# GStreamer/gst-plugins-rs

Hardware: AMD Instinct MI355X
Metric: 4K RGBA frames/sec through hsvfilter+colorlut at 1 GPU; % HBM roofline (higher is better)
Workload: dtype u8

## Files before the change

gst-plugins-rs_amd/csrc/colorlut_kernels.hip:

```cpp
#include "internal.hpp"
#include "hsv_device.hpp"
#include "exact_math.hpp"

#include <cmath>
#include <cstring>
#include <map>
#include <memory>
#include <mutex>
#include <vector>

namespace mi355 {

struct LutK {
  float scale[3];
  float offset[3];
  int size;
};


__device__ __forceinline__ uint32_t floor_idx(float x, uint32_t max_idx) {
  const float f = floorf(x);
  uint32_t i = (f > 0.0f) ? ((f >= 4294967040.0f) ? 0xffffffffu : (uint32_t)f) : 0u;
  return i < max_idx ? i : max_idx;
}
// ... 1337 lines not shown
  }
#undef MI355_ROWS
  return check_hip(ctx, hipGetLastError(), "colorlut rows kernel launch");
}


struct Rgba8Geom {
  size_t n_vec = 0;
  unsigned sw4 = 0, dw4 = 0;
  bool packed = false;
};
static bool rgba8_geom(const uint8_t *d_src, size_t src_pitch, int src_stride, const uint8_t *d_dst, size_t dst_pitch, int dst_stride, int n_frames,
                       int width, int height, Rgba8Geom *g) {
  const size_t row_bytes = (size_t)width * 4;
  if (((uintptr_t)d_src % 16 != 0) || ((uintptr_t)d_dst % 16 != 0)) return false;
  const bool packed = (size_t)src_stride == row_bytes && (size_t)dst_stride == row_bytes &&
                      (n_frames == 1 || (src_pitch == row_bytes * (size_t)height && dst_pitch == row_bytes * (size_t)height));
  const size_t total_bytes = row_bytes * (size_t)height * (size_t)n_frames;
  if (packed) {
    if (total_bytes % 16 != 0) return false;
    g->n_vec = total_bytes / 16;
    g->sw4 = g->dw4 = (unsigned)(row_bytes / 16);
    g->packed = true;
    return true;
  }
  if (width % 4 != 0 || width < 128 || (size_t)src_stride < row_bytes || (size_t)dst_stride < row_bytes || src_stride % 16 != 0 || dst_stride % 16 != 0) return false;
  if (n_frames != 1 && (src_pitch != (size_t)src_stride * (size_t)height || dst_pitch != (size_t)dst_stride * (size_t)height)) return false;
  g->n_vec = total_bytes / 16;
  g->sw4 = (unsigned)src_stride / 16;
  g->dw4 = (unsigned)dst_stride / 16;
  g->packed = false;
  return true;
}

static bool same_hs(const mi355_hsv_settings &a, const mi355_hsv_settings &b) { return std::memcmp(&a, &b, sizeof(a)) == 0; }

struct SharedTable {
  uint32_t *d = nullptr;
  hipEvent_t ready = nullptr;
  std::vector<hipEvent_t> released;
  int device = 0;
  ~SharedTable() {
    int cur = 0;
    (void)hipGetDevice(&cur);
    (void)hipSetDevice(device);
    if (ready) { (void)hipEventSynchronize(ready); (void)hipEventDestroy(ready); }
    for (hipEvent_t e : released) (void)hipEventDestroy(e);
    if (d) (void)hipFree(d);
    (void)hipSetDevice(cur);
  }
};
static std::mutex g_tables_mu;
static std::map<std::string, std::weak_ptr<SharedTable>> g_tables;

static void shared_table_release_locked(mi355_ctx *ctx, std::shared_ptr<void> *ref) {
  if (!*ref) return;
  if (ref->use_count() > 1) {
    SharedTable *sp = static_cast<SharedTable *>(ref->get());
    hipEvent_t e = nullptr;
    if (hipEventCreateWithFlags(&e, hipEventDisableTiming) == hipSuccess) {
      if (hipEventRecord(e, ctx->stream) == hipSuccess) sp->released.push_back(e);
      else { (void)hipEventDestroy(e); (void)hipStreamSynchronize(ctx->stream); }
    } else {
      (void)hipStreamSynchronize(ctx->stream);
    }
    (void)hipGetLastError();
  }
  ref->reset();
}
void shared_table_release(mi355_ctx *ctx, std::shared_ptr<void> *ref) {
  std::shared_ptr<void> last;
  {
    std::lock_guard<std::mutex> g(g_tables_mu);
    if (*ref && ref->use_count() == 1) last = std::move(*ref);
    else shared_table_release_locked(ctx, ref);
  }
}

template <class Build>
static int shared_table_acquire(mi355_ctx *ctx, const std::string &key, std::shared_ptr<void> *ref, uint32_t **out, Build &&build) {
  std::lock_guard<std::mutex> g(g_tables_mu);
  for (auto it = g_tables.begin(); it != g_tables.end();) it = it->second.expired() ? g_tables.erase(it) : std::next(it);
  const std::string full = std::string((const char *)&ctx->device, sizeof(ctx->device)) + key;
  if (auto sp = g_tables[full].lock()) {
    int rc = check_hip(ctx, hipStreamWaitEvent(ctx->stream, sp->ready, 0), "hipStreamWaitEvent(shared table)");
    if (rc) return rc;
    if (ref->get() != sp.get()) shared_table_release_locked(ctx, ref);
    *out = sp->d;
    *ref = sp;
    return MI355_OK;
  }
  std::shared_ptr<SharedTable> sp;
  if (*ref && ref->use_count() == 1) {
    sp = std::static_pointer_cast<SharedTable>(*ref);
    for (hipEvent_t e : sp->released) {
      int rc = check_hip(ctx, hipStreamWaitEvent(ctx->stream, e, 0), "hipStreamWaitEvent(released table)");
      if (rc) return rc;
    }
    for (hipEvent_t e : sp->released) (void)hipEventDestroy(e);
    sp->released.clear();
    for (auto it = g_tables.begin(); it != g_tables.end();) it = it->second.lock() == sp ? g_tables.erase(it) : std::next(it);
  } else {
    shared_table_release_locked(ctx, ref);
    sp = std::make_shared<SharedTable>();
    sp->device = ctx->device;
    int rc = check_hip(ctx, hipMalloc((void **)&sp->d, (size_t)kTableEntries * 4), "hipMalloc(memoised table)");
    if (rc) return rc;
    if ((rc = check_hip(ctx, hipEventCreateWithFlags(&sp->ready, hipEventDisableTiming), "hipEventCreate(shared table)"))) return rc;
  }
  int rc = build(sp->d);
  if (rc) { ref->reset(); return rc; }
  if ((rc = check_hip(ctx, hipEventRecord(sp->ready, ctx->stream), "hipEventRecord(shared table)"))) { ref->reset(); return rc; }
  g_tables[full] = sp;
  *out = sp->d;
  *ref = sp;
  return MI355_OK;
}

extern "C" int mi355_shared_table_count(void) {
  std::lock_guard<std::mutex> g(g_tables_mu);
  int n = 0;
  for (auto &kv : g_tables) n += kv.second.expired() ? 0 : 1;
  return n;
}

static int table_ensure(mi355_ctx *ctx, int which, int morton, const mi355_hsv_settings *hs) {
  LutDevice &L = ctx->lut;
  std::string key(which ? "F" : "L");
  key.push_back((char)('0' + morton));
  key += L.digest;
  if (which) key.append((const char *)hs, sizeof(*hs));
  if (L.table_ref[which] && L.table_key[which] == key) return MI355_OK;
  L.d_table[which] = nullptr;
  L.table_morton[which] = -1;
  L.table_key[which].clear();
  int rc = shared_table_acquire(ctx, key, &L.table_ref[which], &L.d_table[which], [&](uint32_t *tab) {
    uint8_t *t = (uint8_t *)tab;
    hipLaunchKernelGGL(table_domain_kernel, dim3(kTableEntries / 256), dim3(256), 0, ctx->stream, tab, morton);
    L.building_table = true;
    const char *serving = L.last_kernel;
    const int r = which == 0 ? launch_colorlut_compute(ctx, t, 0, 4096 * 4, t, 0, 4096 * 4, 1, 4096, 4096, MI355_FMT_RGBA)
                             : launch_hsv_colorlut_compute(ctx, t, 0, 4096 * 4, t, 0, 4096 * 4, 1, 4096, 4096, *hs, true);
    L.building_table = false;
    L.last_kernel = serving;
    return r;
  });
  if (rc) { L.table_ref[which].reset(); L.d_table[which] = nullptr; return rc; }
  L.table_key[which] = key;
  L.table_morton[which] = morton;
  if (which == 1) L.table_hs = *hs;
  return MI355_OK;
}

enum TableKernel { kTableGather = 0, kTableWindow = 1, kTableEither = 2 };
template <class Compute, class Ensure, class Table>
static int auto_launch(mi355_ctx *ctx, AutoPick &A, size_t n_vec, Compute &&compute, Ensure &&ensure, Table &&table);
static int launch_table_gather(mi355_ctx *ctx, const uint32_t *t, const uint8_t *d_src, uint8_t *d_dst, const Rgba8Geom &geo, int width, size_t rows, int morton);
static int launch_table_raw(mi355_ctx *ctx, const uint32_t *t, const uint8_t *d_src, uint8_t *d_dst, const Rgba8Geom &geo, int width, size_t rows, int morton,
                            TableKernel sub = kTableGather, int *last_sub = nullptr);
static int launch_table(mi355_ctx *ctx, int which, const uint8_t *d_src, uint8_t *d_dst, const Rgba8Geom &geo, int width, size_t rows, int morton,
                        const mi355_hsv_settings *hs, TableKernel sub = kTableGather) {
  int rc = table_ensure(ctx, which, morton, hs);
  if (rc) return rc;
  return launch_table_raw(ctx, ctx->lut.d_table[which], d_src, d_dst, geo, width, rows, morton, sub, &ctx->lut.last_sub[which]);
}

static int launch_table_raw(mi355_ctx *ctx, const uint32_t *t, const uint8_t *d_src, uint8_t *d_dst, const Rgba8Geom &geo, int width, size_t rows, int morton,
                            TableKernel sub, int *last_sub) {
  const bool window_ok = morton && sub != kTableGather && width % 4 == 0 && window_applicable(ctx, (unsigned)width / 4, geo.dw4, rows);
  const size_t src_bytes = (size_t)geo.sw4 * 16 * rows;
  const bool window = window_ok && (sub == kTableWindow || !recently_written(ctx->device, d_src, src_bytes));
  if (last_sub) *last_sub = window ? 1 : 0;
  int rc;
  if (window) {
    ctx->lut.last_kernel = "colorlut_window_kernel";
    rc = launch_window_table(ctx, t, d_src, d_dst, (unsigned)width / 4, geo.sw4, geo.dw4, rows);
  } else {
    rc = launch_table_gather(ctx, t, d_src, d_dst, geo, width, rows, morton);
  }
  return rc;
}

static int launch_table_gather(mi355_ctx *ctx, const uint32_t *t, const uint8_t *d_src, uint8_t *d_dst, const Rgba8Geom &geo, int width, size_t rows, int morton) {
  const size_t n_vec = geo.n_vec;
  ctx->lut.last_kernel = "colorlut_table_tiled_kernel";
  if (width % 4 == 0 && width >= 128 && rows < (1u << 30)) {
    const unsigned w4 = (unsigned)width / 4;
    const unsigned pad64 = (w4 + 63) / 64 * 64 - w4, pad32 = (w4 + 31) / 32 * 32 - w4;
    const unsigned tw4 = pad64 <= pad32 ? 64 : 32;
    const unsigned n_cols = (w4 + tw4 - 1) / tw4, rpb = 8 * (64 / tw4);
    const size_t n_tiles = (size_t)n_cols * ((rows + rpb - 1) / rpb);
    if (n_tiles < (1u << 31)) {
      const size_t grid = n_tiles;
#define MI355_LT(M, T) hipLaunchKernelGGL((colorlut_table_tiled_kernel<M, T>), dim3((unsigned)grid), dim3(256), 0, ctx->stream, (const uint4 *)d_src, \
                                          (uint4 *)d_dst, w4, geo.sw4, geo.dw4, (unsigned)rows, n_cols, t)
      if (morton && tw4 == 64) MI355_LT(true, 64);
      else if (morton) MI355_LT(true, 32);
      else if (tw4 == 64) MI355_LT(false, 64);
      else MI355_LT(false, 32);
#undef MI355_LT
      return check_hip(ctx, hipGetLastError(), "colorlut table kernel launch");
    }
  }
  if (!geo.packed) return set_error(ctx, MI355_ERR_INVALID_ARG, "colorlut: table kernel geometry");
  ctx->lut.last_kernel = "colorlut_table_kernel";
  size_t grid = (size_t)ctx->n_cu * 16;
  const size_t max_blocks = n_vec / 512 + 1;
  if (grid > max_blocks) grid = max_blocks;
  if (morton) hipLaunchKernelGGL((colorlut_table_kernel<true>), dim3((unsigned)grid), dim3(256), 0, ctx->stream, (const uint4 *)d_src, (uint4 *)d_dst, n_vec, t);
  else hipLaunchKernelGGL((colorlut_table_kernel<false>), dim3((unsigned)grid), dim3(256), 0, ctx->stream, (const uint4 *)d_src, (uint4 *)d_dst, n_vec, t);
  return check_hip(ctx, hipGetLastError(), "colorlut table kernel launch");
}

static void auto_harvest(AutoPick &A) {
  if (A.pending_kind < 0) return;
  if (hipEventQuery(A.ev1) != hipSuccess) {
    (void)hipGetLastError();
    return;
  }
  float ms = 0.0f;
  if (hipEventElapsedTime(&ms, A.ev0, A.ev1) != hipSuccess) { (void)hipGetLastError(); ms = 0.0f; }
  auto_complete(A, (double)ms);
}

template <class Compute, class Ensure, class Table>
static int auto_launch(mi355_ctx *ctx, AutoPick &A, size_t n_vec, Compute &&compute, Ensure &&ensure, Table &&table) {
  int rc;
  if (A.table_unavailable) return compute();
  if (!A.ev0) {
    if ((rc = check_hip(ctx, hipEventCreate(&A.ev0), "hipEventCreate"))) return rc;
    if ((rc = check_hip(ctx, hipEventCreate(&A.ev1), "hipEventCreate"))) return rc;
  }
  auto_harvest(A);
  const AutoDecision D = auto_decide(A, n_vec);
  if (D.kind == 1 && (rc = ensure())) {
    auto_give_up_table(A);
    (void)hipGetLastError();
    return compute();
  }
  if (D.measure && (rc = check_hip(ctx, hipEventRecord(A.ev0, ctx->stream), "hipEventRecord"))) return rc;
  if ((rc = D.kind ? table() : compute())) return rc;
  if (D.measure) {
    if ((rc = check_hip(ctx, hipEventRecord(A.ev1, ctx->stream), "hipEventRecord"))) return rc;
    auto_sampled(A, D, n_vec);
  }
  return MI355_OK;
}

constexpr size_t kAutoMinVec = 16384;
static bool table_variant(int v) { return v == 4 || v == 5 || v == 8 || v == 9; }
static TableKernel table_variant_kernel(int v) { return v == 8 ? kTableWindow : (v == 9 ? kTableEither : kTableGather); }

int launch_colorlut(mi355_ctx *ctx, const uint8_t *d_src, size_t src_pitch, int src_stride, uint8_t *d_dst,
                    size_t dst_pitch, int dst_stride, int n_frames, int width, int height, int format) {
  LutDevice &L = ctx->lut;
  if (!L.loaded) return set_error(ctx, MI355_ERR_NOT_CONFIGURED, "No LUT configured");
  if (n_frames <= 0 || width <= 0 || height <= 0) return MI355_OK;
  Rgba8Geom geo;
  const bool table_ok = format == MI355_FMT_RGBA && !ctx->force_generic &&
                        rgba8_geom(d_src, src_pitch, src_stride, d_dst, dst_pitch, dst_stride, n_frames, width, height, &geo);
  const size_t n_vec = geo.n_vec;
  const int v = ctx->lut_variant;
  auto compute = [&]() { return launch_colorlut_compute(ctx, d_src, src_pitch, src_stride, d_dst, dst_pitch, dst_stride, n_frames, width, height, format); };
  if (table_ok && table_variant(v))
    return launch_table(ctx, 0, d_src, d_dst, geo, width, (size_t)n_frames * height, v == 4 ? 0 : 1, nullptr, table_variant_kernel(v));
  if (!table_ok || v != 0 || n_vec < kAutoMinVec) return compute();
  return auto_launch(ctx, L.pick[0], n_vec, compute, [&]() { return table_ensure(ctx, 0, 1, nullptr); },
                     [&]() { return launch_table(ctx, 0, d_src, d_dst, geo, width, (size_t)n_frames * height, 1, nullptr, kTableEither); });
}

constexpr unsigned kStableCalls = 8;
int launch_hsv_colorlut(mi355_ctx *ctx, const uint8_t *d_src, size_t src_pitch, int src_stride, uint8_t *d_dst,
                        size_t dst_pitch, int dst_stride, int n_frames, int width, int height,
                        const mi355_hsv_settings &hs) {
  LutDevice &L = ctx->lut;
  if (!L.loaded) return set_error(ctx, MI355_ERR_NOT_CONFIGURED, "No LUT configured");
  if (n_frames <= 0 || width <= 0 || height <= 0) return MI355_OK;
  Rgba8Geom geo;
  const bool table_ok = !ctx->force_generic && rgba8_geom(d_src, src_pitch, src_stride, d_dst, dst_pitch, dst_stride, n_frames, width, height, &geo);
  const size_t n_vec = geo.n_vec;
  const int v = ctx->lut_variant;
  auto compute = [&]() { return launch_hsv_colorlut_compute(ctx, d_src, src_pitch, src_stride, d_dst, dst_pitch, dst_stride, n_frames, width, height, hs, false); };
  if (table_ok && table_variant(v))
    return launch_table(ctx, 1, d_src, d_dst, geo, width, (size_t)n_frames * height, v == 4 ? 0 : 1, &hs, table_variant_kernel(v));
  if (!table_ok || v != 0 || n_vec < kAutoMinVec) return compute();
  if (same_hs(hs, L.seen_hs)) { if (L.seen_stable < kStableCalls) L.seen_stable++; }
  else { L.seen_hs = hs; L.seen_stable = 0; }
  const bool have = L.table_ref[1] && L.table_morton[1] == 1 && same_hs(L.table_hs, hs);
  if (!have && L.seen_stable < kStableCalls) return compute();
  if (!have && L.pick[1].learn > 2) {
    L.pick[1].t_table = 0.0;
    L.pick[1].learn = 2;
  }
  return auto_launch(ctx, L.pick[1], n_vec, compute, [&]() { return table_ensure(ctx, 1, 1, &hs); },
                     [&]() { return launch_table(ctx, 1, d_src, d_dst, geo, width, (size_t)n_frames * height, 1, &hs, kTableEither); });
}

int colorlut_multi_table(mi355_ctx *ctx, const uint32_t **table_out) {
  LutDevice &L = ctx->lut;
  if (!L.loaded) return set_error(ctx, MI355_ERR_NOT_CONFIGURED, "No LUT configured");
  int rc = table_ensure(ctx, 0, 1, nullptr);
  if (rc) return rc;
  *table_out = L.d_table[0];
  return MI355_OK;
}

int colorlut_multi_fused_table(mi355_ctx *ctx, const mi355_hsv_settings *hs, const uint32_t **table_out) {
  LutDevice &L = ctx->lut;
  if (!L.loaded) return set_error(ctx, MI355_ERR_NOT_CONFIGURED, "No LUT configured");
  if (!hs) return set_error(ctx, MI355_ERR_INVALID_ARG, "null settings");
  int rc = table_ensure(ctx, 1, 1, hs);
  if (rc) return rc;
  *table_out = L.d_table[1];
  return MI355_OK;
}
int launch_colorlut_multi(mi355_ctx *ctx, hipStream_t stream, const uint32_t *table, uint8_t *const *srcs, uint8_t *const *dsts, int n_frames, int width,
                          int height, bool from_hbm) {
  if (n_frames < 1 || n_frames > kMultiFrames || width % 4 != 0 || width < 128 || height <= 0) return MI355_ERR_UNSUPPORTED;
  MultiFramePtrs s{}, d{};
  for (int f = 0; f < n_frames; f++) {
    if (!srcs[f] || !dsts[f] || (uintptr_t)srcs[f] % 16 != 0 || (uintptr_t)dsts[f] % 16 != 0) return MI355_ERR_UNSUPPORTED;
    s.p[f] = srcs[f];
    d.p[f] = dsts[f];
  }
  const unsigned w4 = (unsigned)width / 4;
  if (from_hbm && ctx->lut_variant == 0 && window_multi_applicable(ctx, w4, (size_t)height, n_frames)) {
    ctx->lut.last_kernel = "colorlut_window_kernel";
    return launch_window_table_multi(ctx, stream, table, srcs, dsts, n_frames, w4, (size_t)height);
  }
  ctx->lut.last_kernel = "colorlut_table_tiled_multi_kernel";
  const unsigned pad64 = (w4 + 63) / 64 * 64 - w4, pad32 = (w4 + 31) / 32 * 32 - w4;
  const unsigned tw4 = pad64 <= pad32 ? 64 : 32;
  const unsigned n_cols = (w4 + tw4 - 1) / tw4, rpb = 8 * (64 / tw4);
  const size_t tiles_per_frame = (size_t)n_cols * (((size_t)height + rpb - 1) / rpb);
  const size_t grid = tiles_per_frame * (size_t)n_frames;
  if (grid >= (1u << 31)) return MI355_ERR_UNSUPPORTED;
  if (tw4 == 64) hipLaunchKernelGGL((colorlut_table_tiled_multi_kernel<64>), dim3((unsigned)grid), dim3(256), 0, stream, s, d, w4, (unsigned)height, n_cols, (unsigned)tiles_per_frame, table);
  else hipLaunchKernelGGL((colorlut_table_tiled_multi_kernel<32>), dim3((unsigned)grid), dim3(256), 0, stream, s, d, w4, (unsigned)height, n_cols, (unsigned)tiles_per_frame, table);
  return check_hip(ctx, hipGetLastError(), "colorlut multi-frame table kernel launch");
}

void hsv_table_release(mi355_ctx *ctx) {
  HsvTable &T = ctx->hsv_table;
  shared_table_release(ctx, &T.table_ref);
  if (T.pick.ev0) (void)hipEventDestroy(T.pick.ev0);
  if (T.pick.ev1) (void)hipEventDestroy(T.pick.ev1);
  T = HsvTable{};
}

static int hsv_table_ensure(mi355_ctx *ctx, const PixFmt &fmt, const mi355_hsv_settings &hs) {
  HsvTable &T = ctx->hsv_table;
  if (T.valid && T.bgr == fmt.bgr && same_hs(T.hs, hs)) return MI355_OK;
  T.valid = false;
  T.d_table = nullptr;
  std::string key("H");
  key.push_back((char)('0' + fmt.bgr));
  key.append((const char *)&hs, sizeof(hs));
  int rc = shared_table_acquire(ctx, key, &T.table_ref, &T.d_table, [&](uint32_t *tab) {
    hipLaunchKernelGGL(table_domain_kernel, dim3(kTableEntries / 256), dim3(256), 0, ctx->stream, tab, 1);
    return launch_hsvfilter_compute(ctx, (uint8_t *)tab, 1, 0, 4096, 4096, 4096 * 4, fmt, hs);
  });
  if (rc) { T.table_ref.reset(); T.d_table = nullptr; return rc; }
  T.valid = true;
  T.bgr = fmt.bgr;
  T.hs = hs;
  return MI355_OK;
}

int launch_hsvfilter(mi355_ctx *ctx, uint8_t *d_data, int n_frames, size_t frame_pitch, int width, int height, int stride, const PixFmt &fmt,
                     const mi355_hsv_settings &hs) {
  if (n_frames <= 0 || width <= 0 || height <= 0) return MI355_OK;
  HsvTable &T = ctx->hsv_table;
  auto compute = [&]() { return launch_hsvfilter_compute(ctx, d_data, n_frames, frame_pitch, width, height, stride, fmt, hs); };
  Rgba8Geom geo;
  const bool candidate = ctx->hsv_table_mode == 1 || ctx->hsv_table_mode == 2 || (ctx->hsv_table_mode == 0 && hsv_variant_for(hs, false, true) < 0);
  const bool table_ok = candidate && !ctx->force_generic && fmt.pixel_stride == 4 && fmt.first == 0 &&
                        rgba8_geom(d_data, frame_pitch, stride, d_data, frame_pitch, stride, n_frames, width, height, &geo);
  const size_t n_vec = geo.n_vec;
  T.last_table = false;
  if (!table_ok) return compute();
  const size_t rows = (size_t)n_frames * height;
  if (ctx->hsv_table_mode == 2) {
    int rc = hsv_table_ensure(ctx, fmt, hs);
    T.last_table = true;
    return rc ? rc : launch_table_raw(ctx, T.d_table, d_data, d_data, geo, width, rows, 1, kTableEither, nullptr);
  }
  if (n_vec < kAutoMinVec) return compute();
  if (same_hs(hs, T.seen_hs) && fmt.bgr == T.seen_bgr) { if (T.seen_stable < kStableCalls) T.seen_stable++; }
  else { T.seen_hs = hs; T.seen_bgr = fmt.bgr; T.seen_stable = 0; }
  const bool have = T.valid && T.bgr == fmt.bgr && same_hs(T.hs, hs);
  if (!have && T.seen_stable < kStableCalls) return compute();
  if (!have && T.pick.learn > 2) {
    T.pick.t_table = 0.0;
    T.pick.learn = 2;
  }
  return auto_launch(ctx, T.pick, n_vec, compute, [&]() { return hsv_table_ensure(ctx, fmt, hs); },
                     [&]() { T.last_table = true; return launch_table_raw(ctx, T.d_table, d_data, d_data, geo, width, rows, 1, kTableEither, nullptr); });
}

}

extern "C" int mi355_selftest_brickwatch(int n_calls, const double *miss0, const double *slow0, const double *miss1, const double *slow1, int lag,
                                         int *level_out) {
  if (n_calls < 0 || !miss0 || !slow0 || !miss1 || !slow1 || !level_out || lag < 0) return MI355_ERR_INVALID_ARG;
  const bool shared1 = (lag >> 16) & 1;
  const int min_level = (lag >> 17) & 3;
  lag &= 0xffff;
  mi355::BrickWatch W;
  int level_since = -1, launches_since = 0, pend_level = -1, pend_ready = 0;
  double acc_m = 0, acc_s = 0, pend_m = 0, pend_s = 0;
  for (int i = 0; i < n_calls; i++) {
    if (pend_level >= 0 && i >= pend_ready) { const int l = pend_level; pend_level = -1; mi355::watch_snapshot(W, l, pend_m, pend_s, shared1); }
    const int level = mi355::watch_level(W, pend_level < 0, min_level);
    level_out[i] = level;
    if (level == 2) { level_since = 2; continue; }
    if (level != level_since) { level_since = level; launches_since = 0; acc_m = acc_s = 0; }
    acc_m += level ? miss1[i] : miss0[i];
    acc_s += level ? slow1[i] : slow0[i];
    launches_since++;
    if (pend_level < 0 && launches_since >= (W.probing == level ? 1 : (int)mi355::kWatchSnapEvery)) {
      pend_level = level; pend_m = acc_m / launches_since; pend_s = acc_s / launches_since; pend_ready = i + 1 + lag;
      launches_since = 0; acc_m = acc_s = 0;
    }
  }
  return MI355_OK;
}

extern "C" int mi355_selftest_autopick(int n_calls, const uint64_t *n_vec, const double *ms_compute, const double *ms_table, int lag,
                                       int *kind_out, int *measured_out) {
  if (n_calls < 0 || !n_vec || !ms_compute || !ms_table || !kind_out || lag < 0) return MI355_ERR_INVALID_ARG;
  mi355::AutoPolicy A;
  double pending_ms = 0.0;
  for (int i = 0; i < n_calls; i++) {
    const size_t nv = (size_t)n_vec[i];
    if (A.pending_kind >= 0 && A.calls - A.pending_call >= (unsigned)lag) mi355::auto_complete(A, pending_ms);
    const mi355::AutoDecision D = mi355::auto_decide(A, nv);
    kind_out[i] = D.kind;
    if (measured_out) measured_out[i] = D.measure ? 1 : 0;
    if (D.measure) {
      mi355::auto_sampled(A, D, nv);
      pending_ms = D.kind ? ms_table[i] : ms_compute[i];
    }
  }
  return MI355_OK;
}
```

gst-plugins-rs_amd/csrc/ctx.hip:

```cpp
#include "internal.hpp"
#include <mutex>

#include <cstdio>
#include <cstring>

namespace mi355 {

bool pixfmt_of(int format, PixFmt *out) {
  switch (format) {
    case MI355_FMT_RGBX: *out = {4, 0, 0, 0}; return true;
    case MI355_FMT_RGBA: *out = {4, 0, 0, 1}; return true;
    case MI355_FMT_XRGB: *out = {4, 1, 0, 0}; return true;
    case MI355_FMT_ARGB: *out = {4, 1, 0, 1}; return true;
    case MI355_FMT_BGRX: *out = {4, 0, 1, 0}; return true;
    case MI355_FMT_BGRA: *out = {4, 0, 1, 1}; return true;
    case MI355_FMT_XBGR: *out = {4, 1, 1, 0}; return true;
    case MI355_FMT_ABGR: *out = {4, 1, 1, 1}; return true;
    case MI355_FMT_RGB: *out = {3, 0, 0, 0}; return true;
    case MI355_FMT_BGR: *out = {3, 0, 1, 0}; return true;
    default: return false;
  }
}

int set_error(mi355_ctx *ctx, int status, const std::string &msg) {
// ... 1 lines not shown
  return status;
}

int check_hip(mi355_ctx *ctx, hipError_t e, const char *what) {
  if (e == hipSuccess) return MI355_OK;
  std::string msg = std::string(what) + ": " + hipGetErrorString(e);
  const int st = (e == hipErrorOutOfMemory) ? MI355_ERR_OUT_OF_MEMORY : MI355_ERR_HIP;
  return set_error(ctx, st, msg);
}

static int ensure_stage(mi355_ctx *ctx, int slot, size_t bytes) {
  if (ctx->d_stage_bytes[slot] >= bytes && ctx->d_stage[slot]) return MI355_OK;
  if (ctx->d_stage[slot]) (void)hipFree(ctx->d_stage[slot]);
  ctx->d_stage[slot] = nullptr;
  ctx->d_stage_bytes[slot] = 0;
  int rc = check_hip(ctx, hipMalloc(&ctx->d_stage[slot], bytes ? bytes : 16), "hipMalloc(staging)");
  if (rc) return rc;
  ctx->d_stage_bytes[slot] = bytes ? bytes : 16;
  return MI355_OK;
}

}

using namespace mi355;

template <typename F>
static int time_launches(mi355_ctx *ctx, int iters, float *ms_per_launch, F &&launch) {
  if (iters <= 0 || !ms_per_launch) return set_error(ctx, MI355_ERR_INVALID_ARG, "timing: bad iters/output");
  hipEvent_t e0, e1;
  int rc = check_hip(ctx, hipEventCreate(&e0), "hipEventCreate");
  if (rc) return rc;
  rc = check_hip(ctx, hipEventCreate(&e1), "hipEventCreate");
  if (rc) { (void)hipEventDestroy(e0); return rc; }
  rc = check_hip(ctx, hipEventRecord(e0, ctx->stream), "hipEventRecord");
  for (int i = 0; i < iters && rc == MI355_OK; i++) rc = launch();
  if (rc == MI355_OK) rc = check_hip(ctx, hipEventRecord(e1, ctx->stream), "hipEventRecord");
  if (rc == MI355_OK) rc = check_hip(ctx, hipEventSynchronize(e1), "hipEventSynchronize");
  float ms = 0.0f;
  if (rc == MI355_OK) rc = check_hip(ctx, hipEventElapsedTime(&ms, e0, e1), "hipEventElapsedTime");
  (void)hipEventDestroy(e0);
  (void)hipEventDestroy(e1);
  if (rc == MI355_OK) *ms_per_launch = ms / (float)iters;
  return rc;
}


#define REQUIRE_CTX(ctx) \
  do { if (!(ctx)) return MI355_ERR_INVALID_ARG; } while (0)
#define BIND_DEVICE(ctx)                                                                  \
  do { int rc__ = check_hip((ctx), hipSetDevice((ctx)->device), "hipSetDevice");          \
       if (rc__) return rc__; } while (0)

extern "C" {

int mi355_abi_version(void) { return MI355FX_ABI_VERSION; }

int mi355_device_count(void) {
  int n = 0;
  if (hipGetDeviceCount(&n) != hipSuccess) return 0;
  return n;
}

const char *mi355_status_string(int status) {
  switch (status) {
    case MI355_OK: return "ok";
    case MI355_ERR_INVALID_ARG: return "invalid argument";
    case MI355_ERR_NO_DEVICE: return "no usable gfx950 device";
    case MI355_ERR_HIP: return "HIP runtime error";
    case MI355_ERR_NOT_CONFIGURED: return "element not configured";
    case MI355_ERR_OUT_OF_MEMORY: return "out of device memory";
    case MI355_ERR_UNSUPPORTED: return "unsupported";
    case MI355_ERR_TIMEOUT: return "timeout";
    default: return "unknown status";
  }
}

}

namespace mi355 {
namespace {
struct Written { uintptr_t lo = 0, hi = 0; };
std::mutex g_written_mu;
Written g_written[16][2];
constexpr size_t kOnDieBytes = (size_t)320 << 20;
}

void note_written(int device, const void *p, size_t bytes) {
  if (device < 0 || device >= 16 || !p || !bytes) return;
  std::lock_guard<std::mutex> lk(g_written_mu);
  g_written[device][1] = g_written[device][0];
  g_written[device][0].lo = (uintptr_t)p;
  g_written[device][0].hi = (uintptr_t)p + bytes;
}

void forget_written(int device, const void *p, size_t bytes) {
  if (device < 0 || device >= 16 || !p || !bytes) return;
  std::lock_guard<std::mutex> lk(g_written_mu);
  for (Written &w : g_written[device])
    if (w.hi > w.lo && (uintptr_t)p < w.hi && (uintptr_t)p + bytes > w.lo) w = Written{};
}

bool recently_written(int device, const void *p, size_t bytes) {
  if (device < 0 || device >= 16 || !p || !bytes || bytes > kOnDieBytes) return false;
  std::lock_guard<std::mutex> lk(g_written_mu);
  for (const Written &w : g_written[device])
    if (w.hi > w.lo && (uintptr_t)p >= w.lo && (uintptr_t)p + bytes <= w.hi && w.hi - w.lo <= kOnDieBytes) return true;
  return false;
}
}

extern "C" {

mi355_ctx *mi355_ctx_create(int device, int *status) {
  int n = 0;
  hipError_t e = hipGetDeviceCount(&n);
  if (e != hipSuccess || n <= 0 || device < 0 || device >= n) {
    if (status) *status = MI355_ERR_NO_DEVICE;
    return nullptr;
  }
  if (hipSetDevice(device) != hipSuccess) {
    if (status) *status = MI355_ERR_NO_DEVICE;
    return nullptr;
  }
  hipDeviceProp_t prop;
  if (hipGetDeviceProperties(&prop, device) != hipSuccess) {
    if (status) *status = MI355_ERR_NO_DEVICE;
    return nullptr;
  }
  if (std::strncmp(prop.gcnArchName, "gfx950", 6) != 0) {
    std::fprintf(stderr, "mi355fx: device %d is %s, this library only carries gfx950 code\n", device, prop.gcnArchName);
    if (status) *status = MI355_ERR_NO_DEVICE;
    return nullptr;
  }
  mi355_ctx *ctx = new mi355_ctx();
  ctx->device = device;
  ctx->n_cu = prop.multiProcessorCount > 0 ? prop.multiProcessorCount : 256;
  if (hipStreamCreateWithFlags(&ctx->stream, hipStreamNonBlocking) != hipSuccess) {
    delete ctx;
    if (status) *status = MI355_ERR_HIP;
    return nullptr;
  }
  ctx->own_stream = true;
  if (status) *status = MI355_OK;
  return ctx;
}

void mi355_ctx_destroy(mi355_ctx *ctx) {
  if (!ctx) return;
  (void)hipSetDevice(ctx->device);
  (void)hipStreamSynchronize(ctx->stream);
  lut_release(ctx);
  hsv_table_release(ctx);
  window_release(ctx);
  loudnorm_release(ctx);
  loudnorm_batch_release(ctx);
  dssim_release(ctx);
  roundedcorners_release(ctx);
  colordetect_release(ctx);
  agingradio_release(ctx);
  mixer_release(ctx);
  yolodec_release(ctx);
  handdec_release(ctx);
  ebur128_release(ctx);
  hrtf_release(ctx);
  sofa_release(ctx);
  echo_release(ctx);
  if (ctx->host_copy_ev) (void)hipEventDestroy(ctx->host_copy_ev);
  for (int i = 0; i < 2; i++)
    if (ctx->d_stage[i]) (void)hipFree(ctx->d_stage[i]);
  if (ctx->own_stream && ctx->stream) (void)hipStreamDestroy(ctx->stream);
  delete ctx;
}

const char *mi355_ctx_last_error(const mi355_ctx *ctx) { return ctx ? ctx->last_error.c_str() : "null context"; }

void *mi355_ctx_stream(mi355_ctx *ctx) { return ctx ? (void *)ctx->stream : nullptr; }

int mi355_ctx_set_stream(mi355_ctx *ctx, void *hip_stream) {
  REQUIRE_CTX(ctx);
  BIND_DEVICE(ctx);
  if (ctx->own_stream && ctx->stream) {
    (void)hipStreamSynchronize(ctx->stream);
    (void)hipStreamDestroy(ctx->stream);
  }
  ctx->stream = (hipStream_t)hip_stream;
  ctx->own_stream = false;
  return MI355_OK;
}

int mi355_ctx_synchronize(mi355_ctx *ctx) {
  REQUIRE_CTX(ctx);
  BIND_DEVICE(ctx);
  return check_hip(ctx, hipStreamSynchronize(ctx->stream), "hipStreamSynchronize");
}

int mi355_ctx_set_flag(mi355_ctx *ctx, int flag, int value) {
  REQUIRE_CTX(ctx);
  if (flag == MI355_FLAG_FORCE_GENERIC) { ctx->force_generic = value != 0; return MI355_OK; }
  if (flag == MI355_FLAG_LUT_STAGGER && value >= 0 && value <= 4096) { ctx->lut_stagger = value; return MI355_OK; }
  if (flag == MI355_FLAG_LUT_VARIANT && value >= 0 && value <= 9) { ctx->lut_variant = value; return MI355_OK; }
  if (flag == MI355_FLAG_BRICK_TILES_PER_RUN && value >= 0 && value <= 4096) { ctx->brick_tiles_per_run = value; return MI355_OK; }
  if (flag == MI355_FLAG_BRICK_FOLD_AXIS && value >= 0 && value <= 2) { ctx->brick_fold_axis = value; return MI355_OK; }
  if (flag == MI355_FLAG_DSSIM_TRANSLUCENT && (value == 0 || value == 1)) { ctx->dssim_translucent = value; return MI355_OK; }
  if (flag == MI355_FLAG_DSSIM_FAST && (value == 0 || value == 1)) { ctx->dssim_fast = value; return MI355_OK; }
  if (flag == MI355_FLAG_BRICK_PRIO && value >= 0 && value <= 3) { ctx->brick_prio = value; return MI355_OK; }
  if (flag == MI355_FLAG_BRICK_SETS && (value == 0 || value == 32 || value == 48 || value == 64 || value == 512)) { ctx->brick_sets = value; return MI355_OK; }
  if (flag == MI355_FLAG_HSV_TABLE && value >= 0 && value <= 3) { ctx->hsv_table_mode = value; return MI355_OK; }
  if (flag == MI355_FLAG_FUSED_VARIANT && value >= 0 && value <= 1) { ctx->fused_variant = value; return MI355_OK; }
  if (flag == MI355_FLAG_HSV_BLOCKS_PER_CU && value >= 1 && value <= 4096) { ctx->hsv_blocks_per_cu = value; return MI355_OK; }
  if (flag == MI355_FLAG_HRTF_METHOD && value >= 0 && value <= 2) { ctx->hrtf_method = value; return MI355_OK; }
  if (flag == MI355_FLAG_BLOCKHASH_ANY_SIZE && (value == 0 || value == 1)) { ctx->blockhash_any_size = value; return MI355_OK; }
  if (flag == MI355_FLAG_HSV_NT && (value == 0 || value == 1)) { ctx->hsv_nt = value; return MI355_OK; }
  if (flag == MI355_FLAG_WINDOW_ORDER && (value == 0 || value == 1)) { ctx->window_order = value; return MI355_OK; }
  if (flag == MI355_FLAG_WINDOW_STATS && (value == 0 || value == 1)) { ctx->window_stats_on = value != 0; return MI355_OK; }
  if (flag == MI355_FLAG_WINDOW_MIN_STEPS && value >= 0 && value <= 4096) { ctx->window_min_steps = value; return MI355_OK; }
  return set_error(ctx, MI355_ERR_INVALID_ARG, "unknown flag");
}

void *mi355_device_alloc(mi355_ctx *ctx, size_t bytes) {
  if (!ctx) return nullptr;
  if (hipSetDevice(ctx->device) != hipSuccess) return nullptr;
  void *p = nullptr;
  if (check_hip(ctx, hipMalloc(&p, bytes ? bytes : 16), "hipMalloc")) return nullptr;
  return p;
}

int mi355_device_free(mi355_ctx *ctx, void *dptr) {
  REQUIRE_CTX(ctx);
  BIND_DEVICE(ctx);
  return check_hip(ctx, hipFree(dptr), "hipFree");
}

int mi355_memcpy_h2d(mi355_ctx *ctx, void *dptr, const void *host, size_t bytes) {
  REQUIRE_CTX(ctx);
  BIND_DEVICE(ctx);
  int rc = check_hip(ctx, hipMemcpyAsync(dptr, host, bytes, hipMemcpyHostToDevice, ctx->stream), "hipMemcpyAsync(H2D)");
  forget_written(ctx->device, dptr, bytes);
  __atomic_fetch_add(&ctx->n_h2d, 1ull, __ATOMIC_RELAXED);
  if (rc) return rc;
  return check_hip(ctx, hipStreamSynchronize(ctx->stream), "hipStreamSynchronize");
}

int mi355_memcpy_d2h(mi355_ctx *ctx, void *host, const void *dptr, size_t bytes) {
  REQUIRE_CTX(ctx);
  BIND_DEVICE(ctx);
  int rc = check_hip(ctx, hipMemcpyAsync(host, dptr, bytes, hipMemcpyDeviceToHost, ctx->stream), "hipMemcpyAsync(D2H)");
  __atomic_fetch_add(&ctx->n_d2h, 1ull, __ATOMIC_RELAXED);
  if (rc) return rc;
  return check_hip(ctx, hipStreamSynchronize(ctx->stream), "hipStreamSynchronize");
}


int mi355_hsvfilter_frames_device(mi355_ctx *ctx, uint8_t *d_data, int n_frames, size_t frame_pitch, int width,
                                  int height, int stride, int format, const mi355_hsv_settings *settings) {
  REQUIRE_CTX(ctx);
  PixFmt fmt;
  if (!settings || !pixfmt_of(format, &fmt)) return set_error(ctx, MI355_ERR_INVALID_ARG, "hsvfilter: bad settings/format");
  if (n_frames < 0 || width < 0 || height < 0 || stride < 0) return set_error(ctx, MI355_ERR_INVALID_ARG, "hsvfilter: negative size");
  if (n_frames == 0 || width == 0 || height == 0) return MI355_OK;
  if (!d_data) return set_error(ctx, MI355_ERR_INVALID_ARG, "hsvfilter: null data");
  if ((size_t)stride < (size_t)width * fmt.pixel_stride)
    return set_error(ctx, MI355_ERR_INVALID_ARG, "hsvfilter: stride smaller than width*pixel_stride");
  if (n_frames > 1 && frame_pitch < (size_t)(height - 1) * (size_t)stride + (size_t)width * fmt.pixel_stride)
    return set_error(ctx, MI355_ERR_INVALID_ARG, "hsvfilter: frame_pitch smaller than one frame (frames would overlap)");
  BIND_DEVICE(ctx);
  const int rc = launch_hsvfilter(ctx, d_data, n_frames, frame_pitch, width, height, stride, fmt, *settings);
  if (rc == MI355_OK) note_written(ctx->device, d_data, (size_t)(n_frames - 1) * frame_pitch + (size_t)stride * (size_t)height);
  return rc;
}

int mi355_hsvfilter_frame_ip(mi355_ctx *ctx, uint8_t *data, size_t data_len, int width, int stride, int format,
                             const mi355_hsv_settings *settings) {
  REQUIRE_CTX(ctx);
  PixFmt fmt;
  if (!settings || !pixfmt_of(format, &fmt)) return set_error(ctx, MI355_ERR_INVALID_ARG, "hsvfilter: bad settings/format");
  if (width < 0 || stride <= 0) return set_error(ctx, MI355_ERR_INVALID_ARG, "hsvfilter: bad width/stride");
  if (data_len % (size_t)fmt.pixel_stride != 0) return set_error(ctx, MI355_ERR_INVALID_ARG, "hsvfilter: plane length not a multiple of pixel stride");
  const size_t rows = data_len / (size_t)stride;
  if (rows == 0 || width == 0) return MI355_OK;
  if (!data) return set_error(ctx, MI355_ERR_INVALID_ARG, "hsvfilter: null data");
  if ((size_t)width * fmt.pixel_stride > (size_t)stride) return set_error(ctx, MI355_ERR_INVALID_ARG, "hsvfilter: width*pixel_stride exceeds stride");
  if (rows > 0x7fffffffu) return set_error(ctx, MI355_ERR_INVALID_ARG, "hsvfilter: too many rows");
  BIND_DEVICE(ctx);
  const size_t bytes = rows * (size_t)stride;
  int rc = ensure_stage(ctx, 0, bytes);
  if (rc) return rc;
  uint8_t *d = (uint8_t *)ctx->d_stage[0];
  rc = check_hip(ctx, hipMemcpyAsync(d, data, bytes, hipMemcpyHostToDevice, ctx->stream), "hipMemcpyAsync(H2D frame)");
  __atomic_fetch_add(&ctx->n_h2d, 1ull, __ATOMIC_RELAXED);
  if (rc) return rc;
  rc = launch_hsvfilter(ctx, d, 1, bytes, width, (int)rows, stride, fmt, *settings);
  if (rc) return rc;
  rc = check_hip(ctx, hipMemcpyAsync(data, d, bytes, hipMemcpyDeviceToHost, ctx->stream), "hipMemcpyAsync(D2H frame)");
  __atomic_fetch_add(&ctx->n_d2h, 1ull, __ATOMIC_RELAXED);
  if (rc) return rc;
  return check_hip(ctx, hipStreamSynchronize(ctx->stream), "hsvfilter: stream synchronize");
}


static bool detect_out_fmt(int fmt, int *alpha_first, int *bgr) {
  switch (fmt) {
    case MI355_FMT_RGBA: *alpha_first = 0; *bgr = 0; return true;
    case MI355_FMT_ARGB: *alpha_first = 1; *bgr = 0; return true;
    case MI355_FMT_BGRA: *alpha_first = 0; *bgr = 1; return true;
    case MI355_FMT_ABGR: *alpha_first = 1; *bgr = 1; return true;
    default: return false;
  }
}
static bool detect_in_fmt(int fmt, PixFmt *p) {
  switch (fmt) {
    case MI355_FMT_RGBX: case MI355_FMT_XRGB: case MI355_FMT_BGRX: case MI355_FMT_XBGR:
    case MI355_FMT_RGB: case MI355_FMT_BGR: return pixfmt_of(fmt, p);
    default: return false;
  }
}

}

namespace mi355 {
int hsvdetect_check_frames(const uint8_t *d_src, int src_stride, int src_format, const uint8_t *d_dst, int dst_stride, int dst_format, int n_frames,
                           int width, int height, const mi355_hsvdetect_settings *settings, PixFmt *sfmt, int *alpha_first, int *bgr, const char **why) {
  if (!settings || !detect_in_fmt(src_format, sfmt) || !detect_out_fmt(dst_format, alpha_first, bgr)) { *why = "hsvdetector: bad settings/format"; return MI355_ERR_INVALID_ARG; }
  if (n_frames < 0 || width < 0 || height < 0) { *why = "hsvdetector: negative size"; return MI355_ERR_INVALID_ARG; }
  if (n_frames == 0 || width == 0 || height == 0) return MI355_OK;
  if (!d_src || !d_dst) { *why = "hsvdetector: null data"; return MI355_ERR_INVALID_ARG; }
  if ((size_t)src_stride < (size_t)width * sfmt->pixel_stride || (size_t)dst_stride < (size_t)width * 4) {
    *why = "hsvdetector: line bytes exceed stride";
    return MI355_ERR_INVALID_ARG;
  }
  return MI355_OK;
}
}

extern "C" {

int mi355_hsvdetect_frames_device(mi355_ctx *ctx, const uint8_t *d_src, size_t src_pitch, int src_stride, int src_format,
                                  uint8_t *d_dst, size_t dst_pitch, int dst_stride, int dst_format, int n_frames,
                                  int width, int height, const mi355_hsvdetect_settings *settings) {
  REQUIRE_CTX(ctx);
  PixFmt sfmt;
  int af = 0, bgr = 0;
  const char *why = nullptr;
  const int bad = hsvdetect_check_frames(d_src, src_stride, src_format, d_dst, dst_stride, dst_format, n_frames, width, height, settings, &sfmt, &af, &bgr, &why);
  if (bad) return set_error(ctx, bad, why);
  if (n_frames == 0 || width == 0 || height == 0) return MI355_OK;
  BIND_DEVICE(ctx);
  const int rc = launch_hsvdetect(ctx, d_src, src_pitch, src_stride, sfmt, d_dst, dst_pitch, dst_stride, af, bgr, n_frames, width, height, *settings);
  if (rc == MI355_OK) note_written(ctx->device, d_dst, (size_t)(n_frames - 1) * dst_pitch + (size_t)dst_stride * (size_t)height);
  return rc;
}

int mi355_hsvdetect_frame(mi355_ctx *ctx, const uint8_t *src, size_t src_len, int src_stride, int src_format, uint8_t *dst,
                          size_t dst_len, int dst_stride, int dst_format, int width, const mi355_hsvdetect_settings *settings) {
  REQUIRE_CTX(ctx);
  PixFmt sfmt;
  int af = 0, bgr = 0;
  if (!settings || !detect_in_fmt(src_format, &sfmt) || !detect_out_fmt(dst_format, &af, &bgr))
    return set_error(ctx, MI355_ERR_INVALID_ARG, "hsvdetector: bad settings/format");
  if (width < 0 || src_stride <= 0 || dst_stride <= 0) return set_error(ctx, MI355_ERR_INVALID_ARG, "hsvdetector: bad width/stride");
  const size_t rows_in = src_len / (size_t)src_stride, rows_out = dst_len / (size_t)dst_stride;
  if (rows_in != rows_out) return set_error(ctx, MI355_ERR_INVALID_ARG, "hsvdetector: input/output row count mismatch");
  if (src_len % (size_t)sfmt.pixel_stride != 0) return set_error(ctx, MI355_ERR_INVALID_ARG, "hsvdetector: plane length not a multiple of pixel stride");
  if ((size_t)width * sfmt.pixel_stride > (size_t)src_stride || (size_t)width * 4 > (size_t)dst_stride)
    return set_error(ctx, MI355_ERR_INVALID_ARG, "hsvdetector: line bytes exceed stride");
  if (rows_in == 0 || width == 0) return MI355_OK;
  if (!src || !dst) return set_error(ctx, MI355_ERR_INVALID_ARG, "hsvdetector: null data");
  BIND_DEVICE(ctx);
  const size_t sb = rows_in * (size_t)src_stride, db = rows_out * (size_t)dst_stride;
  int rc = ensure_stage(ctx, 0, sb);
  if (rc) return rc;
  rc = ensure_stage(ctx, 1, db);
  if (rc) return rc;
  uint8_t *ds = (uint8_t *)ctx->d_stage[0], *dd = (uint8_t *)ctx->d_stage[1];
  rc = check_hip(ctx, hipMemcpyAsync(ds, src, sb, hipMemcpyHostToDevice, ctx->stream), "hipMemcpyAsync(H2D src)");
  __atomic_fetch_add(&ctx->n_h2d, 1ull, __ATOMIC_RELAXED);
  if (rc) return rc;
  rc = check_hip(ctx, hipMemcpyAsync(dd, dst, db, hipMemcpyHostToDevice, ctx->stream), "hipMemcpyAsync(H2D dst)");
  __atomic_fetch_add(&ctx->n_h2d, 1ull, __ATOMIC_RELAXED);
  if (rc) return rc;
  rc = launch_hsvdetect(ctx, ds, sb, src_stride, sfmt, dd, db, dst_stride, af, bgr, 1, width, (int)rows_in, *settings);
  if (rc) return rc;
  rc = check_hip(ctx, hipMemcpyAsync(dst, dd, db, hipMemcpyDeviceToHost, ctx->stream), "hipMemcpyAsync(D2H dst)");
  __atomic_fetch_add(&ctx->n_d2h, 1ull, __ATOMIC_RELAXED);
  if (rc) return rc;
  return check_hip(ctx, hipStreamSynchronize(ctx->stream), "hsvdetector: stream synchronize");
}


int mi355_colorlut_load(mi355_ctx *ctx, int is3d, size_t size, const float *table, const float domain_scale[3],
                        const float domain_offset[3]) {
  REQUIRE_CTX(ctx);
  if (!table || !domain_scale || !domain_offset) return set_error(ctx, MI355_ERR_INVALID_ARG, "colorlut: null LUT data");
  if (is3d ? (size < 2 || size > 256) : (size < 2 || size > 65536))
    return set_error(ctx, MI355_ERR_INVALID_ARG, "colorlut: LUT size out of range");
  BIND_DEVICE(ctx);
  int rc = check_hip(ctx, hipStreamSynchronize(ctx->stream), "colorlut: stream synchronize");
  if (rc) return rc;
  return lut_upload(ctx, is3d ? 1 : 0, size, table, domain_scale, domain_offset);
}

int mi355_colorlut_unload(mi355_ctx *ctx) {
  REQUIRE_CTX(ctx);
  BIND_DEVICE(ctx);
  (void)hipStreamSynchronize(ctx->stream);
  lut_release(ctx);
  return MI355_OK;
}

int mi355_colorlut_kernel_choice(mi355_ctx *ctx, int fused, int *table_in_use, double *ms_per_mpx_compute, double *ms_per_mpx_table) {
  REQUIRE_CTX(ctx);
  if (fused == 10 || fused == 11) {
    if (table_in_use) *table_in_use = ctx->lut.last_sub[fused - 10];
    if (ms_per_mpx_compute) *ms_per_mpx_compute = 0.0;
    if (ms_per_mpx_table) *ms_per_mpx_table = 0.0;
    return MI355_OK;
  }
  const AutoPick &A = fused == 2 ? ctx->hsv_table.pick : ctx->lut.pick[fused ? 1 : 0];
  if (table_in_use)
    *table_in_use = fused == 2 ? (ctx->hsv_table.last_table ? 1 : 0)
                               : (ctx->lut_variant == 4 || ctx->lut_variant == 5 || ctx->lut_variant == 8 || ctx->lut_variant == 9 || (ctx->lut_variant == 0 && A.t_table > 0.0 && A.table));
  if (ms_per_mpx_compute) *ms_per_mpx_compute = A.t_compute * 250000.0;
  if (ms_per_mpx_table) *ms_per_mpx_table = A.t_table * 250000.0;
  return MI355_OK;
}

const char *mi355_colorlut_last_kernel(mi355_ctx *ctx) {
  if (!ctx) return "";
  return ctx->lut.last_kernel ? ctx->lut.last_kernel : "";
}

int mi355_colorlut_brick_stats(mi355_ctx *ctx, uint64_t counters[2], double *last_miss_fraction, int *hostile, int reset) {
  REQUIRE_CTX(ctx);
  BIND_DEVICE(ctx);
  unsigned long long c[2] = {0, 0};
  int rc = brick_read_counters(ctx, ctx->lut.brick, c, reset != 0);
  if (rc) return rc;
  if (counters) { counters[0] = c[0]; counters[1] = c[1]; }
  if (last_miss_fraction) *last_miss_fraction = ctx->lut.brick.watch.last_miss;
  if (hostile) *hostile = ctx->lut.brick.watch.home;
  return MI355_OK;
}

int mi355_colorlut_window_stats(mi355_ctx *ctx, uint64_t counters[3], int reset) {
  REQUIRE_CTX(ctx);
  BIND_DEVICE(ctx);
  if (!counters) return set_error(ctx, MI355_ERR_INVALID_ARG, "null counters");
  unsigned long long c[3] = {0, 0, 0};
  int rc = window_read_counters(ctx, c, reset != 0);
  if (rc) return rc;
  for (int i = 0; i < 3; i++) counters[i] = c[i];
  return MI355_OK;
}

static int colorlut_bpp(int format) {
  if (format == MI355_FMT_RGBA) return 4;
  if (format == MI355_FMT_RGBA64_LE || format == MI355_FMT_RGBA64_BE) return 8;
  return 0;
}

int mi355_colorlut_frames_device(mi355_ctx *ctx, const uint8_t *d_src, size_t src_pitch, int src_stride, uint8_t *d_dst,
                                 size_t dst_pitch, int dst_stride, int n_frames, int width, int height, int format) {
  REQUIRE_CTX(ctx);
  const int bpp = colorlut_bpp(format);
  if (!bpp) return set_error(ctx, MI355_ERR_INVALID_ARG, "colorlut: format must be RGBA, RGBA64_LE or RGBA64_BE");
  if (!ctx->lut.loaded) return set_error(ctx, MI355_ERR_NOT_CONFIGURED, "No LUT configured");
  if (n_frames < 0 || width < 0 || height < 0) return set_error(ctx, MI355_ERR_INVALID_ARG, "colorlut: negative size");
  if (n_frames == 0 || width == 0 || height == 0) return MI355_OK;
  if (!d_src || !d_dst) return set_error(ctx, MI355_ERR_INVALID_ARG, "colorlut: null data");
  if ((size_t)src_stride < (size_t)width * bpp || (size_t)dst_stride < (size_t)width * bpp)
    return set_error(ctx, MI355_ERR_INVALID_ARG, "colorlut: stride smaller than row bytes");
  if (n_frames > 1 && (src_pitch < (size_t)(height - 1) * (size_t)src_stride + (size_t)width * bpp ||
                       dst_pitch < (size_t)(height - 1) * (size_t)dst_stride + (size_t)width * bpp))
    return set_error(ctx, MI355_ERR_INVALID_ARG, "colorlut: frame pitch smaller than one frame (frames would overlap)");
  BIND_DEVICE(ctx);
  const int rc = launch_colorlut(ctx, d_src, src_pitch, src_stride, d_dst, dst_pitch, dst_stride, n_frames, width, height, format);
  if (rc == MI355_OK) note_written(ctx->device, d_dst, (size_t)(n_frames - 1) * dst_pitch + (size_t)dst_stride * (size_t)height);
  return rc;
}

int mi355_hsv_colorlut_frames_device(mi355_ctx *ctx, const uint8_t *d_src, size_t src_pitch, int src_stride, uint8_t *d_dst,
                                     size_t dst_pitch, int dst_stride, int n_frames, int width, int height,
                                     const mi355_hsv_settings *settings) {
  REQUIRE_CTX(ctx);
  if (!settings) return set_error(ctx, MI355_ERR_INVALID_ARG, "hsv+colorlut: null settings");
  if (!ctx->lut.loaded) return set_error(ctx, MI355_ERR_NOT_CONFIGURED, "No LUT configured");
  if (n_frames < 0 || width < 0 || height < 0) return set_error(ctx, MI355_ERR_INVALID_ARG, "hsv+colorlut: negative size");
  if (n_frames == 0 || width == 0 || height == 0) return MI355_OK;
  if (!d_src || !d_dst) return set_error(ctx, MI355_ERR_INVALID_ARG, "hsv+colorlut: null data");
  if ((size_t)src_stride < (size_t)width * 4 || (size_t)dst_stride < (size_t)width * 4)
    return set_error(ctx, MI355_ERR_INVALID_ARG, "hsv+colorlut: stride smaller than row bytes");
  if (n_frames > 1 && (src_pitch < (size_t)(height - 1) * (size_t)src_stride + (size_t)width * 4 ||
                       dst_pitch < (size_t)(height - 1) * (size_t)dst_stride + (size_t)width * 4))
    return set_error(ctx, MI355_ERR_INVALID_ARG, "hsv+colorlut: frame pitch smaller than one frame (frames would overlap)");
  BIND_DEVICE(ctx);
  const int rc = launch_hsv_colorlut(ctx, d_src, src_pitch, src_stride, d_dst, dst_pitch, dst_stride, n_frames, width, height, *settings);
  if (rc == MI355_OK) note_written(ctx->device, d_dst, (size_t)(n_frames - 1) * dst_pitch + (size_t)dst_stride * (size_t)height);
  return rc;
}

int mi355_colorlut_frame(mi355_ctx *ctx, const uint8_t *src, int src_stride, uint8_t *dst, int dst_stride, int width,
                         int height, int format) {
  REQUIRE_CTX(ctx);
  const int bpp = colorlut_bpp(format);
  if (!bpp) return set_error(ctx, MI355_ERR_INVALID_ARG, "colorlut: format must be RGBA, RGBA64_LE or RGBA64_BE");
  if (!ctx->lut.loaded) return set_error(ctx, MI355_ERR_NOT_CONFIGURED, "No LUT configured");
  if (width < 0 || height < 0 || src_stride <= 0 || dst_stride <= 0) return set_error(ctx, MI355_ERR_INVALID_ARG, "colorlut: bad size/stride");
  if (width == 0 || height == 0) return MI355_OK;
  if (!src || !dst) return set_error(ctx, MI355_ERR_INVALID_ARG, "colorlut: null data");
  const size_t s_stride = bpp == 8 ? (size_t)(src_stride / 2) * 2 : (size_t)src_stride;
  const size_t d_stride = bpp == 8 ? (size_t)(dst_stride / 2) * 2 : (size_t)dst_stride;
  const size_t row_bytes = (size_t)width * bpp;
  if (row_bytes > s_stride || row_bytes > d_stride) return set_error(ctx, MI355_ERR_INVALID_ARG, "colorlut: row bytes exceed stride");
  BIND_DEVICE(ctx);
  const size_t packed = row_bytes * (size_t)height;
  int rc = ensure_stage(ctx, 0, packed);
  if (rc) return rc;
  rc = ensure_stage(ctx, 1, packed);
  if (rc) return rc;
  uint8_t *ds = (uint8_t *)ctx->d_stage[0], *dd = (uint8_t *)ctx->d_stage[1];
  rc = check_hip(ctx, hipMemcpy2DAsync(ds, row_bytes, src, s_stride, row_bytes, (size_t)height, hipMemcpyHostToDevice, ctx->stream),
                 "hipMemcpy2DAsync(H2D src)");
  if (rc) return rc;
  rc = launch_colorlut(ctx, ds, packed, (int)row_bytes, dd, packed, (int)row_bytes, 1, width, height, format);
  if (rc) return rc;
  rc = check_hip(ctx, hipMemcpy2DAsync(dst, d_stride, dd, row_bytes, row_bytes, (size_t)height, hipMemcpyDeviceToHost, ctx->stream),
                 "hipMemcpy2DAsync(D2H dst)");
  if (rc) return rc;
  return check_hip(ctx, hipStreamSynchronize(ctx->stream), "colorlut: stream synchronize");
}


int mi355_echo_setup(mi355_ctx *ctx, size_t ring_len) { return mi355_echo_setup_batch(ctx, 1, ring_len); }

int mi355_echo_setup_batch(mi355_ctx *ctx, int n_streams, size_t ring_len) {
  REQUIRE_CTX(ctx);
  BIND_DEVICE(ctx);
  return echo_setup(ctx, n_streams, ring_len);
}

int mi355_echo_reset(mi355_ctx *ctx) {
  REQUIRE_CTX(ctx);
  BIND_DEVICE(ctx);
  (void)hipStreamSynchronize(ctx->stream);
  echo_release(ctx);
  return MI355_OK;
}

int mi355_echo_process_batch_device(mi355_ctx *ctx, void *d_data, size_t stream_stride, size_t n, int is_f64, const size_t *delay_samples,
                                    const double *intensity, const double *feedback) {
  REQUIRE_CTX(ctx);
  if (!delay_samples || !intensity || !feedback) return set_error(ctx, MI355_ERR_INVALID_ARG, "rsaudioecho: null parameter array");
  if (n && !d_data) return set_error(ctx, MI355_ERR_INVALID_ARG, "rsaudioecho: null data");
  BIND_DEVICE(ctx);
  return launch_echo_batch(ctx, d_data, stream_stride, n, is_f64, delay_samples, intensity, feedback);
}

int mi355_echo_process_device(mi355_ctx *ctx, void *d_data, size_t n, int is_f64, size_t delay_samples, double intensity,
                              double feedback) {
  REQUIRE_CTX(ctx);
  if (n && !d_data) return set_error(ctx, MI355_ERR_INVALID_ARG, "rsaudioecho: null data");
  BIND_DEVICE(ctx);
  return launch_echo(ctx, d_data, n, is_f64, delay_samples, intensity, feedback);
}

static int echo_host(mi355_ctx *ctx, void *data, size_t n, int is_f64, size_t delay, double intensity, double feedback) {
  REQUIRE_CTX(ctx);
  if (n && !data) return set_error(ctx, MI355_ERR_INVALID_ARG, "rsaudioecho: null data");
  if (!ctx->echo.configured) return set_error(ctx, MI355_ERR_NOT_CONFIGURED, "rsaudioecho: not negotiated (setup not called)");
  BIND_DEVICE(ctx);
  const size_t bytes = n * (is_f64 ? sizeof(double) : sizeof(float));
  int rc = ensure_stage(ctx, 0, bytes);
  if (rc) return rc;
  if (n) {
    rc = check_hip(ctx, hipMemcpyAsync(ctx->d_stage[0], data, bytes, hipMemcpyHostToDevice, ctx->stream), "hipMemcpyAsync(H2D audio)");
    if (rc) return rc;
  }
  rc = launch_echo(ctx, ctx->d_stage[0], n, is_f64, delay, intensity, feedback);
  if (rc) return rc;
  if (n) {
    rc = check_hip(ctx, hipMemcpyAsync(data, ctx->d_stage[0], bytes, hipMemcpyDeviceToHost, ctx->stream), "hipMemcpyAsync(D2H audio)");
    if (rc) return rc;
  }
  return check_hip(ctx, hipStreamSynchronize(ctx->stream), "rsaudioecho: stream synchronize");
}

int mi355_echo_process_f32(mi355_ctx *ctx, float *data, size_t n, size_t delay_samples, double intensity, double feedback) {
  return echo_host(ctx, data, n, 0, delay_samples, intensity, feedback);
}
int mi355_echo_process_f64(mi355_ctx *ctx, double *data, size_t n, size_t delay_samples, double intensity, double feedback) {
  return echo_host(ctx, data, n, 1, delay_samples, intensity, feedback);
}

int mi355_echo_get_state(mi355_ctx *ctx, double *ring_out, size_t ring_len, size_t *pos_out) {
  return mi355_echo_get_state_batch(ctx, 0, ring_out, ring_len, pos_out);
}

int mi355_echo_get_state_batch(mi355_ctx *ctx, int stream, double *ring_out, size_t ring_len, size_t *pos_out) {
  REQUIRE_CTX(ctx);
  if (!ctx->echo.configured) return set_error(ctx, MI355_ERR_NOT_CONFIGURED, "rsaudioecho: not negotiated (setup not called)");
  if (stream < 0 || stream >= ctx->echo.n_streams) return set_error(ctx, MI355_ERR_INVALID_ARG, "rsaudioecho: no such stream in the batch");
  BIND_DEVICE(ctx);
  if (pos_out) *pos_out = ctx->echo.pos;
  if (ring_out) {
// ... 453 lines not shown
```

gst-plugins-rs_amd/csrc/group.hip:

```cpp
#include "internal.hpp"

#include <chrono>
#include <condition_variable>
#include <algorithm>
#include <cstring>
#include <deque>
#include <mutex>
#include <unordered_map>
#include <vector>

using namespace mi355;

namespace {

struct Desc {
  mi355_ctx *ctx;
  uint8_t *src, *dst;
  int width, height, stride, format;
  mi355_hsv_settings hs;
  const uint32_t *table;
  std::shared_ptr<void> table_ref;
  bool batchable;
  bool fused;
  uint64_t ticket;
// ... 826 lines not shown
        both.insert(both.end(), frames.begin(), frames.end());
        unsigned long long *d_hashes = (unsigned long long *)(g->d_hash_sums[lane] + (size_t)2 * kCmpMaxBatch * 64);
        rc = blockhash_enqueue(a, both.data(), 2 * n, first.stride, first.width, first.height, fmt.pixel_stride, g->d_hash_sums[lane], d_hashes);
        if (!rc && hipMemcpyAsync(block, d_hashes, (size_t)2 * n * 8, hipMemcpyDeviceToHost, a->stream) != hipSuccess) rc = MI355_ERR_HIP;
      }
      if (!rc && hipEventRecord(done, a->stream) != hipSuccess) rc = MI355_ERR_HIP;
      if (rc) {
        (void)hipGetLastError();
        if (done) g->events.push_back(done);
        if (block) g->cmp_blocks.push_back(block);
        g->last_error = a->last_error.empty() ? "group: compare launch failed" : a->last_error;
        if (g->cmp_results.size() > 65536) g->cmp_results.clear();
        for (const CmpDesc &d : take) g->cmp_results[d.ticket] = CmpResult{rc, 0.0, {0, 0}};
        if (!first_rc) first_rc = rc;
        continue;
      }
      CmpBatch b{g->next_cmp_seq++, {}, first.algo, first.width, first.height, lane, done, 0, block};
      for (const CmpDesc &d : take) { b.tickets.push_back(d.ticket); g->cmp_where[d.ticket] = b.seq; reached |= until != 0 && d.ticket == until; }
      g->cmp_batches.push_back(std::move(b));
    }
    for (const CmpDesc &d : all)
      if (d.ready) g->events.push_back(d.ready);
    g->n_cmp_pairs += (uint64_t)total;
    g->n_cmp_batches++;
    if ((uint64_t)total > g->n_cmp_largest) g->n_cmp_largest = (uint64_t)total;
  }
  g->cv.notify_all();
  return first_rc;
}

void cmp_retire_done(mi355_group *g) {
  for (CmpBatch &b : g->cmp_batches) {
    if (b.collected) continue;
    if (hipEventQuery(b.done) != hipSuccess) { (void)hipGetLastError(); continue; }
    cmp_collect(g, b);
  }
  cmp_retire(g);
}

int cmp_wait_unlocking(mi355_group *g, std::unique_lock<std::mutex> &lk, uint64_t ticket) {
  auto it = g->cmp_where.find(ticket);
  if (it == g->cmp_where.end()) return MI355_OK;
  const uint64_t seq = it->second;
  const Waited w = wait_seq_unlocking(g->cmp_batches, seq, lk);
  if (w == Waited::kNothing) return MI355_OK;
  if (w == Waited::kFailed) return fail(g, MI355_ERR_HIP, "hipEventSynchronize(group compare batch)");
  int lane = -1;
  for (const CmpBatch &b : g->cmp_batches)
    if (b.seq == seq) lane = b.lane;
  for (CmpBatch &b : g->cmp_batches)
    if (b.lane == lane && b.seq <= seq) cmp_collect(g, b);
  cmp_retire(g);
  return MI355_OK;
}


template <class F>
void for_each_set_queue(mi355_group *g, F &&f) {
  f(g->cd);
  f(g->hd);
  f(g->yd);
  f(g->hn);
}

int refuse_set_queue_ticket(mi355_group *g, uint64_t ticket) {
  std::string owner;
  for_each_set_queue(g, [&](auto &q) {
    if (owner.empty() && q.owns(ticket)) owner = q.foreign_refusal();
  });
  return owner.empty() ? MI355_OK : fail(g, MI355_ERR_INVALID_ARG, owner);
}

}

extern "C" {

mi355_group *mi355_group_create(int device, int max_batch, int *status) {
  if (max_batch < 0 || max_batch > kMultiFrames) { if (status) *status = MI355_ERR_INVALID_ARG; return nullptr; }
  if (hipSetDevice(device) != hipSuccess) { (void)hipGetLastError(); if (status) *status = MI355_ERR_NO_DEVICE; return nullptr; }
  mi355_group *g = new mi355_group();
  g->device = device;
  g->max_batch = max_batch ? max_batch : 8;
  if (hipStreamCreateWithFlags(&g->stream, hipStreamNonBlocking) != hipSuccess) {
    (void)hipGetLastError();
    delete g;
    if (status) *status = MI355_ERR_HIP;
    return nullptr;
  }
  if (status) *status = MI355_OK;
  return g;
}

void mi355_group_destroy(mi355_group *g) {
  if (!g) return;
  (void)hipSetDevice(g->device);
  {
    Locked L(g);
    (void)flush_locked(g);
    (void)wait_all_unlocking(g, L.lk);
  }
  (void)hipStreamSynchronize(g->stream);
  if (g->actx) {
    {
      Locked L(g);
      (void)cmp_flush_locked(g);
    }
    for (int l = 0; l < kCmpMaxLanes; l++)
      if (g->alane[l]) (void)hipStreamSynchronize(g->alane[l]->stream);
    for (CmpBatch &b : g->cmp_batches) { (void)hipEventDestroy(b.done); (void)hipHostFree(b.h_block); }
    g->cmp_batches.clear();
    for (void *b : g->cmp_blocks) (void)hipHostFree(b);
    for (int l = 0; l < kCmpMaxLanes; l++) {
      if (g->d_hash_sums[l]) (void)hipFree(g->d_hash_sums[l]);
      if (g->alane[l]) mi355_ctx_destroy(g->alane[l]);
    }
  }
  for_each_set_queue(g, [&](auto &q) { q.destroy(g); });
  for (Batch &b : g->batches) (void)hipEventDestroy(b.done);
  for (Desc &d : g->pending)
    if (d.ready) (void)hipEventDestroy(d.ready);
  g->pending.clear();
  g->batches.clear();
  g->dead_refs.clear();
  for (hipEvent_t e : g->events) (void)hipEventDestroy(e);
  (void)hipStreamDestroy(g->stream);
  delete g;
}

const char *mi355_group_last_error(mi355_group *g) { return g ? g->last_error.c_str() : "null group"; }

static int submit_frame(mi355_group *g, mi355_ctx *ctx, uint8_t *d_src, uint8_t *d_dst, int width, int height, int stride, int format,
                        const mi355_hsv_settings *settings, uint64_t *ticket, bool fused) {
  if (!g) return MI355_ERR_INVALID_ARG;
  Locked L(g);
  PixFmt fmt;
  if (!ctx || !d_src || !d_dst || !settings || width <= 0 || height <= 0 || !pixfmt_of(format, &fmt) || (size_t)stride < (size_t)width * fmt.pixel_stride)
    return fail(g, MI355_ERR_INVALID_ARG, "group: bad frame");
  if (format != MI355_FMT_RGBA) return fail(g, MI355_ERR_INVALID_ARG, "group: hsvfilter ! colorlut takes RGBA frames only");
  if (ctx->device != g->device) return fail(g, MI355_ERR_INVALID_ARG, "group: context of another device");
  if (!ctx->lut.loaded) return fail(g, MI355_ERR_NOT_CONFIGURED, "No LUT configured");
  if (hipSetDevice(g->device) != hipSuccess) { (void)hipGetLastError(); return fail(g, MI355_ERR_HIP, "hipSetDevice"); }
  Desc d{};
  d.ctx = ctx; d.src = d_src; d.dst = d_dst; d.width = width; d.height = height; d.stride = stride; d.format = format; d.hs = *settings;
  d.fused = fused;
  retire_done(g);
  bool settled = true;
  if (fused) {
    if (std::memcmp(&ctx->group_fused_hs, settings, sizeof(*settings)) == 0) { if (ctx->group_fused_stable < 1000000u) ctx->group_fused_stable++; }
    else { ctx->group_fused_hs = *settings; ctx->group_fused_stable = 1; }
    settled = ctx->group_fused_stable >= 8u;
  }
  const uint8_t *one[1] = {d_src};
  d.batchable = settled && format == MI355_FMT_RGBA && (fused || d_src != d_dst) && hsvfilter_multi_applicable(one, 1, width, height, stride, fmt) && width % 4 == 0 &&
                width >= 128 && (uintptr_t)d_dst % 16 == 0 && ctx->lut_variant == 0 && ctx->hsv_table_mode != 2 && (!fused || ctx->lut.is3d);
  if (d.batchable && (fused ? colorlut_multi_fused_table(ctx, settings, &d.table) : colorlut_multi_table(ctx, &d.table)) != MI355_OK) {
    (void)hipGetLastError();
    d.batchable = false;
    d.table = nullptr;
  }
  if (d.batchable) d.table_ref = ctx->lut.table_ref[fused ? 1 : 0];
  if (int rc = record_ready(g, ctx, &d.ready)) return rc;
  d.ticket = g->next_ticket++;
  if (ticket) *ticket = d.ticket;
  g->pending.push_back(d);
  if ((int)g->pending.size() >= g->max_batch) (void)flush_locked(g, g->pending.front().ticket);
  return MI355_OK;
}

int mi355_group_submit_chain(mi355_group *g, mi355_ctx *ctx, uint8_t *d_src, uint8_t *d_dst, int width, int height, int stride, int format,
                             const mi355_hsv_settings *settings, uint64_t *ticket) {
  return submit_frame(g, ctx, d_src, d_dst, width, height, stride, format, settings, ticket, false);
}

int mi355_group_submit_fused(mi355_group *g, mi355_ctx *ctx, uint8_t *d_src, uint8_t *d_dst, int width, int height, int stride, int format,
                             const mi355_hsv_settings *settings, uint64_t *ticket) {
  return submit_frame(g, ctx, d_src, d_dst, width, height, stride, format, settings, ticket, true);
}

int mi355_group_flush(mi355_group *g) {
  if (!g) return MI355_ERR_INVALID_ARG;
  Locked L(g);
  if (hipSetDevice(g->device) != hipSuccess) { (void)hipGetLastError(); return fail(g, MI355_ERR_HIP, "hipSetDevice"); }
  const int rc = flush_locked(g);
  const int rc2 = g->actx ? cmp_flush_locked(g) : MI355_OK;
  int first = rc ? rc : rc2;
  for_each_set_queue(g, [&](auto &q) {
    const int r = q.kind.set_up() ? q.flush_locked(g) : MI355_OK;
    if (!first) first = r;
  });
  return first;
}


int mi355_group_set_rendezvous(mi355_group *g, int expected_streams, unsigned linger_us) {
  if (!g || expected_streams < 0) return MI355_ERR_INVALID_ARG;
  Locked L(g);
  g->expected_streams = expected_streams;
  g->linger_us = linger_us;
  return MI355_OK;
}

int mi355_group_set_compare_lanes(mi355_group *g, int lanes) {
  if (!g || lanes < 1 || lanes > kCmpMaxLanes) return MI355_ERR_INVALID_ARG;
  Locked L(g);
  if (g->actx) return fail(g, MI355_ERR_INVALID_ARG, "group: the compare queue's streams exist already (set the lanes before the first submit_compare)");
  g->n_lanes = lanes;
  return MI355_OK;
}

int mi355_group_submit_compare(mi355_group *g, mi355_ctx *ctx, const uint8_t *d_ref, const uint8_t *d_frame, int stride, int width, int height, int format,
                               int algo, uint64_t *ticket) {
  if (!g) return MI355_ERR_INVALID_ARG;
  Locked L(g);
  PixFmt fmt;
  if (!ctx || !d_ref || !d_frame || width <= 0 || height <= 0 || !pixfmt_of(format, &fmt) || (format != MI355_FMT_RGB && format != MI355_FMT_RGBA) ||
      (size_t)stride < (size_t)width * fmt.pixel_stride)
    return fail(g, MI355_ERR_INVALID_ARG, "group: bad frame pair (videocompare's engines take packed RGB / RGBA)");
  if (algo != MI355_HASH_DSSIM && algo != MI355_HASH_BLOCKHASH)
    return fail(g, MI355_ERR_UNSUPPORTED, "group: pairs are batched for hash-algorithm dssim and blockhash; the resize hashes go through their context");
  if (algo == MI355_HASH_BLOCKHASH && (width % 8 != 0 || height % 8 != 0))
    return fail(g, MI355_ERR_UNSUPPORTED, "group: blockhash batches take frames of 8 x 8 whole blocks (the any-size path goes through its context)");
  if (ctx->device != g->device) return fail(g, MI355_ERR_INVALID_ARG, "group: context of another device");
  if (hipSetDevice(g->device) != hipSuccess) { (void)hipGetLastError(); return fail(g, MI355_ERR_HIP, "hipSetDevice"); }
  if (!g->actx) {
    int st = MI355_OK;
    for (int l = 0; l < g->n_lanes && !st; l++) {
      g->alane[l] = mi355_ctx_create(g->device, &st);
      if (!g->alane[l] && !st) st = MI355_ERR_HIP;
      if (!st && hipMalloc((void **)&g->d_hash_sums[l], (size_t)2 * kCmpMaxBatch * (64 * 4 + 8)) != hipSuccess) { (void)hipGetLastError(); st = MI355_ERR_OUT_OF_MEMORY; }
    }
    if (st) {
      for (int l = 0; l < kCmpMaxLanes; l++) {
        if (g->d_hash_sums[l]) (void)hipFree(g->d_hash_sums[l]);
        if (g->alane[l]) mi355_ctx_destroy(g->alane[l]);
        g->d_hash_sums[l] = nullptr; g->alane[l] = nullptr;
      }
      return fail(g, st, "group: no contexts for the compare queue");
    }
    g->actx = g->alane[0];
  }
  cmp_retire_done(g);
  CmpDesc d{};
  d.ctx = ctx; d.ref = d_ref; d.frame = d_frame; d.width = width; d.height = height; d.stride = stride; d.format = format; d.algo = algo;
  d.translucent = ctx->dssim_translucent;
  d.fast = ctx->dssim_fast;
  if (int rc = record_ready(g, ctx, &d.ready)) return rc;
  d.ticket = g->next_ticket++;
  if (ticket) *ticket = d.ticket;
  g->cmp_pending.push_back(d);
  const int full = g->expected_streams > 0 && g->expected_streams < kCmpMaxBatch ? g->expected_streams : kCmpMaxBatch;
  if ((int)g->cmp_pending.size() >= full) (void)cmp_flush_locked(g);
  return MI355_OK;
}

int mi355_group_wait_compare(mi355_group *g, uint64_t ticket, double *distance, uint64_t hashes[2]) {
  if (!g) return MI355_ERR_INVALID_ARG;
  Locked L(g);
  std::unique_lock<std::mutex> &lk = L.lk;
  if (ticket == 0 || ticket >= g->next_ticket) return fail(g, MI355_ERR_INVALID_ARG, "group: unknown ticket");
  if (int rc = refuse_set_queue_ticket(g, ticket)) return rc;
  if (hipSetDevice(g->device) != hipSuccess) { (void)hipGetLastError(); return fail(g, MI355_ERR_HIP, "hipSetDevice"); }
  auto is_pending = [&]() { for (const CmpDesc &d : g->cmp_pending) if (d.ticket == ticket) return true; return false; };
  if (is_pending()) {
    if (g->expected_streams > 0 && g->linger_us > 0) {
      const auto deadline = std::chrono::steady_clock::now() + std::chrono::microseconds(g->linger_us);
      while (is_pending() && (int)g->cmp_pending.size() < g->expected_streams) {
        if (g->cv.wait_until(lk, deadline) == std::cv_status::timeout) break;
      }
    }
    if (is_pending()) (void)cmp_flush_locked(g, ticket);
  }
  int rc = cmp_wait_unlocking(g, lk, ticket);
  if (rc) return rc;
  auto r = g->cmp_results.find(ticket);
  if (r == g->cmp_results.end()) return fail(g, MI355_ERR_INVALID_ARG, "group: this pair's result has been collected already (or the ticket is not a pair's)");
  const CmpResult res = r->second;
  g->cmp_results.erase(r);
  if (res.status) return fail(g, res.status, "group: the launch that carried this pair failed");
  if (distance) *distance = res.distance;
  if (hashes) { hashes[0] = res.hashes[0]; hashes[1] = res.hashes[1]; }
  return MI355_OK;
}

int mi355_group_compare_stats(mi355_group *g, uint64_t stats[3]) {
  if (!g || !stats) return MI355_ERR_INVALID_ARG;
  std::lock_guard<std::mutex> lk(g->mu);
  stats[0] = g->n_cmp_pairs;
  stats[1] = g->n_cmp_batches;
  stats[2] = g->n_cmp_largest;
  return MI355_OK;
}


int mi355_group_set_colordetect_rendezvous(mi355_group *g, int expected_streams, unsigned linger_us) {
  if (!g || expected_streams < 0) return MI355_ERR_INVALID_ARG;
  Locked L(g);
  g->cd.set_rendezvous(expected_streams, linger_us);
  return MI355_OK;
}

int mi355_group_submit_colordetect(mi355_group *g, mi355_ctx *ctx, const uint8_t *d_data, size_t data_len, int format, int quality, int max_colors,
                                   uint64_t *ticket) {
  if (!g) return MI355_ERR_INVALID_ARG;
  Locked L(g);
  if (!ctx || !ticket) return fail(g, MI355_ERR_INVALID_ARG, "group: null context or ticket");
  const char *why = nullptr;
  int rc = colordetect_check_frame(data_len, format, quality, max_colors, &why);
// ... 334 lines not shown
```

gst-plugins-rs_amd/csrc/internal.hpp:

```cpp
#pragma once
#include <hip/hip_runtime.h>
#include <cstddef>
#include <cstdint>
#include <memory>
#include <string>
#include <vector>
#include "../../include/mi355fx.h"

#include "autopick.hpp"
#include "colorlut_brick.hpp"
#include "colorlut_window.hpp"

namespace mi355 {

struct AutoPick : AutoPolicy {
  hipEvent_t ev0 = nullptr, ev1 = nullptr;
};

struct LutDevice {
  int is3d = 0;
  int size = 0;
  float scale[3] = {1, 1, 1};
  float offset[3] = {0, 0, 0};
  float *d_cells = nullptr;
  float *d_planar = nullptr;
  uint32_t *d_axis = nullptr;
  size_t planar_plane_floats = 0;
  int lds_Sy = 0, lds_Sz = 0;
  size_t lds_bytes = 0;
  bool lds_all_resident = false;
  bool lds_ok = false;
  uint32_t *d_table[2] = {nullptr, nullptr};
  std::shared_ptr<void> table_ref[2];
  std::string table_key[2];
  std::string digest;
  int table_morton[2] = {-1, -1};
  mi355_hsv_settings table_hs{};
  mi355_hsv_settings seen_hs{};
  unsigned seen_stable = 0;
  AutoPick pick[2];
  int last_sub[2] = {0, 0};
  BrickLut brick;
  bool building_table = false;
  const char *last_kernel = "";
  bool loaded = false;
};

struct HsvTable {
  uint32_t *d_table = nullptr;
  std::shared_ptr<void> table_ref;
  bool valid = false;
  int bgr = 0;
  mi355_hsv_settings hs{};
  mi355_hsv_settings seen_hs{};
  int seen_bgr = 0;
  unsigned seen_stable = 0;
  bool last_table = false;
  AutoPick pick;
};

struct EchoDevice {
  double *d_ring = nullptr;
  size_t ring_len = 0;
  size_t pos = 0;
  int n_streams = 1;
  void *d_par = nullptr, *h_par = nullptr;
  hipEvent_t par_ev = nullptr;
  bool configured = false;
};

}

struct mi355_dssim_image;

struct mi355_ctx {
  int device = 0;
  hipStream_t stream = nullptr;
  bool own_stream = false;
  int n_cu = 256;
  void *d_stage[2] = {nullptr, nullptr};
  size_t d_stage_bytes[2] = {0, 0};
  mi355::LutDevice lut;
  mi355::EchoDevice echo;
  void *ebur128 = nullptr;
  void *hrtf = nullptr;
  void *sofa = nullptr;
  void *loudnorm = nullptr;
  void *loudnorm_batch = nullptr;
  void *dssim_cache = nullptr;
  void *rounded = nullptr;
  void *colordetect = nullptr;
  void *agingradio = nullptr;
  void *mixer = nullptr;
  void *yolodec = nullptr;
  void *handdec = nullptr;
  unsigned long long n_h2d = 0, n_d2h = 0;
  bool force_generic = false;
  int fused_variant = 0;
  int lut_variant = 0;
  int hsv_table_mode = 0;
  mi355::HsvTable hsv_table;
  int lut_stagger = 0;
  int brick_tiles_per_run = 0;
  int brick_fold_axis = 2;
  hipEvent_t host_copy_ev = nullptr;
  int dssim_translucent = 0;
  int dssim_fast = 0;
  int brick_prio = 3;
  int brick_sets = 0;
  int hrtf_method = 0;
  int window_min_steps = mi355::kWindowMinStepsPerBlock;
  int window_order = 1;
  bool window_stats_on = false;
  unsigned long long *d_window_counters = nullptr;
  int blockhash_any_size = 0;
  int hsv_nt = 0;
  mi355_hsv_settings group_fused_hs{};
  unsigned group_fused_stable = 0;
  int hsv_blocks_per_cu = 64;
  std::string last_error;
};

namespace mi355 {

constexpr int kMultiFrames = 16;
struct MultiFramePtrs { uint8_t *p[kMultiFrames]; };

struct PixFmt {
  int pixel_stride;
  int first;
  int bgr;
  int has_alpha;
};
bool pixfmt_of(int format, PixFmt *out);

int set_error(mi355_ctx *ctx, int status, const std::string &msg);
void note_written(int device, const void *p, size_t bytes);
bool recently_written(int device, const void *p, size_t bytes);
void forget_written(int device, const void *p, size_t bytes);
int check_hip(mi355_ctx *ctx, hipError_t e, const char *what);

int launch_hsvfilter(mi355_ctx *ctx, uint8_t *d_data, int n_frames, size_t frame_pitch, int width,
                     int height, int stride, const PixFmt &fmt, const mi355_hsv_settings &s);
int launch_hsvfilter_compute(mi355_ctx *ctx, uint8_t *d_data, int n_frames, size_t frame_pitch, int width,
                     int height, int stride, const PixFmt &fmt, const mi355_hsv_settings &s);
void hsv_table_release(mi355_ctx *ctx);
bool hsvfilter_multi_applicable(const uint8_t *const *frames, int n_frames, int width, int height, int stride, const PixFmt &fmt);
int launch_hsvfilter_multi(mi355_ctx *ctx, hipStream_t stream, uint8_t *const *frames, int n_frames, int width, int height, const PixFmt &fmt,
                           const mi355_hsv_settings &s);
int colorlut_multi_table(mi355_ctx *ctx, const uint32_t **table_out);
int colorlut_multi_fused_table(mi355_ctx *ctx, const mi355_hsv_settings *hs, const uint32_t **table_out);
int launch_colorlut_multi(mi355_ctx *ctx, hipStream_t stream, const uint32_t *table, uint8_t *const *srcs, uint8_t *const *dsts, int n_frames, int width,
                          int height, bool from_hbm = false);
int launch_hsvdetect(mi355_ctx *ctx, const uint8_t *d_src, size_t src_pitch, int src_stride,
                     const PixFmt &sfmt, uint8_t *d_dst, size_t dst_pitch, int dst_stride,
                     int dst_alpha_first, int dst_bgr, int n_frames, int width, int height,
                     const mi355_hsvdetect_settings &s);
int launch_colorlut(mi355_ctx *ctx, const uint8_t *d_src, size_t src_pitch, int src_stride,
                    uint8_t *d_dst, size_t dst_pitch, int dst_stride, int n_frames, int width,
                    int height, int format);
int launch_hsv_colorlut(mi355_ctx *ctx, const uint8_t *d_src, size_t src_pitch, int src_stride,
                        uint8_t *d_dst, size_t dst_pitch, int dst_stride, int n_frames, int width,
                        int height, const mi355_hsv_settings &hs);
int lut_upload(mi355_ctx *ctx, int is3d, size_t size, const float *table, const float scale[3],
               const float offset[3]);
void lut_release(mi355_ctx *ctx);
int echo_setup(mi355_ctx *ctx, int n_streams, size_t ring_len);
void echo_release(mi355_ctx *ctx);
int launch_echo_batch(mi355_ctx *ctx, void *d_data, size_t stream_stride, size_t n, int is_f64, const size_t *delay, const double *intensity,
                      const double *feedback);
int launch_echo(mi355_ctx *ctx, void *d_data, size_t n, int is_f64, size_t delay, double intensity,
                double feedback);
int ebur128_setup(mi355_ctx *ctx, unsigned channels, unsigned rate, unsigned mode, const int *channel_class);
int ebur128_setup_batch(mi355_ctx *ctx, unsigned n_streams, unsigned channels, unsigned rate, unsigned mode, const int *channel_class);
int ebur128_add_frames_batch(mi355_ctx *ctx, const void *data, size_t frames, int fmt, int device_data);
int ebur128_query_batch(mi355_ctx *ctx, int what, double *out);
int ebur128_peak_batch(mi355_ctx *ctx, int true_peak, double *out);
int ebur128_reset(mi355_ctx *ctx);
int ebur128_reset_stream(mi355_ctx *ctx, unsigned stream);
int ebur128_add_frames_streams(mi355_ctx *ctx, const void *data, size_t slot_elems, const size_t *frames_per, int fmt, int device_data);
void ebur128_release(mi355_ctx *ctx);
int launch_blockhash(mi355_ctx *ctx, const uint8_t *d_frames, size_t frame_pitch, int stride, int n_frames, int width, int height,
                     int channels, unsigned long long *hashes);
int launch_imghash(mi355_ctx *ctx, const uint8_t *d_frames, size_t frame_pitch, int stride, int n_frames, int width, int height, int channels,
                   int algo, unsigned long long *hashes);
int loudnorm_setup(mi355_ctx *ctx, unsigned channels, double loudness_target, double loudness_range_target, double max_true_peak, double offset_db);
int loudnorm_push(mi355_ctx *ctx, const double *data, size_t frames, double *out, size_t out_cap_frames, size_t *out_frames);
int loudnorm_drain(mi355_ctx *ctx, double *out, size_t out_cap_frames, size_t *out_frames, int *eos);
void loudnorm_release(mi355_ctx *ctx);
int loudnorm_setup_batch(mi355_ctx *ctx, unsigned n_streams, unsigned channels, double loudness_target, double loudness_range_target, double max_true_peak, double offset_db);
size_t loudnorm_batch_frame_size(mi355_ctx *ctx);
size_t loudnorm_member_frame_size(mi355_ctx *ctx, unsigned stream);
int loudnorm_member_frame_type(mi355_ctx *ctx, unsigned stream);
int loudnorm_process_members(mi355_ctx *ctx, const unsigned char *members, const double *data, size_t stream_stride, size_t frames, double *out, size_t out_stride,
                             size_t out_cap_frames, size_t *out_frames, int device_data, int final_frame);
int loudnorm_process_batch(mi355_ctx *ctx, const double *data, size_t stream_stride, size_t frames, double *out, size_t out_stride, size_t out_cap_frames,
                           size_t *out_frames, int device_data, int final_frame);
void loudnorm_batch_release(mi355_ctx *ctx);
int dssim_create_image(mi355_ctx *ctx, const uint8_t *d_frame, int stride, int width, int height, int channels, mi355_dssim_image **out);
void dssim_free_image(mi355_ctx *ctx, mi355_dssim_image *img);
int dssim_compare(mi355_ctx *ctx, const mi355_dssim_image *a, const mi355_dssim_image *b, double *out);
int dssim_compare_frames(mi355_ctx *ctx, const mi355_dssim_image *a, const uint8_t *const *d_frames, int n_frames, int stride, int width, int height,
                         int channels, double *out);
int dssim_compare_pairs_enqueue(mi355_ctx *ctx, const uint8_t *const *d_refs, const uint8_t *const *d_frames, int n_pairs, int stride, int width, int height,
                                int channels, double *h_slots);
void dssim_scores_from_slots(int width, int height, const double *h_slots, int n_pairs, double *out);
int dssim_compare_pairs(mi355_ctx *ctx, const uint8_t *const *d_refs, const uint8_t *const *d_frames, int n_pairs, int stride, int width, int height,
                        int channels, double *out, int map_scale, float *map_out);
struct DssimFastJob { const uint8_t *u8[2]; const float4 *lin[2]; int stride, channels, pattern, w, h; float *map; double *partial; };
struct DssimFastJobs { DssimFastJob job[3]; unsigned first[4]; const float *lut; };
constexpr int kDssimFastTw = 32, kDssimFastTh = 16;
int dssim_fast_enqueue(mi355_ctx *ctx, const DssimFastJobs &J);
constexpr int kDssimSlotDoubles = 15;
int blockhash_enqueue(mi355_ctx *ctx, const uint8_t *const *d_frames, int n, int stride, int width, int height, int channels, uint32_t *d_sums,
                      unsigned long long *d_hashes);
int dssim_cbrt_selftest(mi355_ctx *ctx, uint32_t lo_bits, uint32_t hi_bits, uint64_t *mismatches);
void dssim_release(mi355_ctx *ctx);
void roundedcorners_release(mi355_ctx *ctx);
void colordetect_release(mi355_ctx *ctx);
constexpr int kCdSetMax = MI355_COLORDETECT_SET_MAX;
struct CdFrame { const uint8_t *data; size_t data_len; int format, quality, max_colors; };
struct CdSetScratch;
int colordetect_check_frame(size_t data_len, int format, int quality, int max_colors, const char **why);
int colordetect_plan(int n_cu, int n_jobs, const uint64_t *n_samples, uint32_t *first_block, uint32_t *blocks, uint64_t *samples_per_block, uint32_t *total_blocks);
CdSetScratch *colordetect_set_scratch_new(hipStream_t stream, int *status, std::string *err);
void colordetect_set_scratch_free(CdSetScratch *S);
size_t colordetect_set_block_bytes();
int colordetect_launch_set(CdSetScratch *S, hipStream_t stream, int n_cu, const CdFrame *frames, int n, void *h_block, int *kernel_launches, std::string *err);
void colordetect_set_result(const void *h_block, int i, uint8_t palette_rgb[255 * 3], int *n_colors);
constexpr int kHdSetMax = MI355_HSVDETECT_SET_MAX;
struct HdFrame {
  const uint8_t *src;
  uint8_t *dst;
  int src_stride, dst_stride, width, height;
  PixFmt sfmt;
  int dst_alpha_first, dst_bgr;
  mi355_hsvdetect_settings s;
  int force_generic;
};
int hsvdetect_check_frames(const uint8_t *d_src, int src_stride, int src_format, const uint8_t *d_dst, int dst_stride, int dst_format, int n_frames,
                           int width, int height, const mi355_hsvdetect_settings *settings, PixFmt *sfmt, int *alpha_first, int *bgr, const char **why);
int hsvdetect_plan(int n_cu, int blocks_per_cu, unsigned units_per_block, int n_jobs, const uint64_t *units, uint32_t *first_block, uint32_t *blocks,
                   uint32_t *total_blocks);
int hsvdetect_launch_set(hipStream_t stream, int n_cu, const HdFrame *frames, int n, int *kernel_launches, std::string *err);

enum { kAgingClick = 1, kAgingNoise = 2, kAgingQuant = 4, kAgingCubic = 8 };
struct AgingJob {
  void *data;
  double *state;
  unsigned long long frames, k0;
  unsigned long long seed, p_int;
  double alpha, factor, ampl, dist;
  unsigned channels, passes;
  int is_f64, flags;
};
int agingradio_setup_filter(unsigned rate, unsigned lowpass_freq, double *alpha);
void agingradio_settings_to_job(const mi355_agingradio_settings &s, AgingJob *J);
int launch_agingradio_jobs(hipStream_t stream, int n_cu, const AgingJob *h_jobs, const AgingJob *d_jobs, unsigned n_jobs, std::string *err);
void agingradio_release(mi355_ctx *ctx);
struct MixerCall {
  unsigned n_inputs, n_out_channels;
  const uint16_t *bits;
  const mi355_mixer_segment *segs;
  unsigned n_segs;
  const mi355_mixer_output *outs;
  unsigned n_outs;
  size_t frames;
// ... 108 lines not shown
```

gst-plugins-rs_amd/mi355fx/__init__.py:

```python
import ctypes as C
import os

import numpy as np

_HERE = os.path.dirname(os.path.abspath(__file__))
PKG_ROOT = os.path.dirname(_HERE)
LIB_PATH = os.environ.get("MI355FX_LIB") or os.path.join(PKG_ROOT, "libmi355fx.so")
HEADER_PATH = os.path.join(os.path.dirname(PKG_ROOT), "include", "mi355fx.h")

FMT = {"RGBx": 0, "xRGB": 1, "BGRx": 2, "xBGR": 3, "RGBA": 4, "ARGB": 5, "BGRA": 6, "ABGR": 7,
       "RGB": 8, "BGR": 9, "RGBA64_LE": 10, "RGBA64_BE": 11}
FMT_LAYOUT = {"RGBx": (4, 0, 0), "RGBA": (4, 0, 0), "RGB": (3, 0, 0), "xRGB": (4, 1, 0), "ARGB": (4, 1, 0),
              "BGRx": (4, 0, 1), "BGRA": (4, 0, 1), "BGR": (3, 0, 1), "xBGR": (4, 1, 1), "ABGR": (4, 1, 1)}

OK, ERR_INVALID_ARG, ERR_NO_DEVICE, ERR_HIP, ERR_NOT_CONFIGURED, ERR_OOM, ERR_UNSUPPORTED, ERR_TIMEOUT = 0, -1, -2, -3, -4, -5, -6, -7
FLAG_FORCE_GENERIC = 1
FLAG_HSV_BLOCKS_PER_CU = 2
FLAG_FUSED_VARIANT = 3
FLAG_LUT_VARIANT = 4
FLAG_LUT_STAGGER = 5
FLAG_HSV_TABLE = 6
FLAG_BRICK_TILES_PER_RUN = 7
FLAG_BRICK_SETS = 8
FLAG_BRICK_PRIO = 9
# ... 34 lines not shown
    _fields_ = [("data", C.c_void_p), ("format", C.c_uint32), ("channel_offset", C.c_uint32), ("n_channels", C.c_uint32)]


def mixer_tables(segments, outputs):
    fmt = {np.dtype(np.float32): 0, np.dtype(np.int16): 1}
    segs = (MixerSegment * max(len(segments), 1))()
    for k, (inp, data, off) in enumerate(segments):
        if isinstance(data, np.ndarray):
            assert data.ndim == 1 and data.flags.c_contiguous
            segs[k] = MixerSegment(data.ctypes.data if data.size else None, inp, fmt[data.dtype], off, data.size)
        else:
            segs[k] = MixerSegment(data[0], inp, data[1], off, data[2])
    outs = (MixerOutput * max(len(outputs), 1))()
    for k, (data, off, nch) in enumerate(outputs):
        if isinstance(data, np.ndarray):
            assert data.flags.c_contiguous
            outs[k] = MixerOutput(data.ctypes.data if data.size else None, fmt[data.dtype], off, nch)
        else:
            outs[k] = MixerOutput(data[0], data[1], off, nch)
    return segs, outs


class YoloParams(C.Structure):
    _fields_ = [("box_confidence_threshold", C.c_float), ("class_confidence_threshold", C.c_float), ("iou_threshold", C.c_float)]


YOLO_LAYOUT = {"V8": 0, "X": 1}
YOLO_X_HEAD = 2
YOLO_DET = np.dtype([("xmin", "<f4"), ("ymin", "<f4"), ("xmax", "<f4"), ("ymax", "<f4"), ("x", "<i4"), ("y", "<i4"), ("width", "<i4"),
                     ("height", "<i4"), ("class_id", "<u4"), ("confidence", "<f4"), ("candidate", "<u4"), ("reserved", "<u4")])


def _yolo_params(params):
    if isinstance(params, YoloParams) or (len(params) == 3 and not hasattr(params[0], "__len__") and not isinstance(params[0], YoloParams)):
        params = [params]
    arr = (YoloParams * max(len(params), 1))()
    for k, q in enumerate(params):
        arr[k] = q if isinstance(q, YoloParams) else YoloParams(*[float(v) for v in q])
    return arr, len(params)


YOLOX_LEVELS_MAX = 8


class YoloxLevel(C.Structure):
    _fields_ = [("reg", C.c_void_p), ("obj", C.c_void_p), ("cls", C.c_void_p), ("reg_pitch_bytes", C.c_size_t), ("obj_pitch_bytes", C.c_size_t),
                ("cls_pitch_bytes", C.c_size_t), ("h", C.c_uint32), ("w", C.c_uint32), ("stride", C.c_uint32), ("reserved", C.c_uint32)]


def _yolox_levels(levels):
    arr = (YoloxLevel * max(len(levels), 1))()
    for k, q in enumerate(levels):
        arr[k] = q if isinstance(q, YoloxLevel) else YoloxLevel(*q)
    return arr


def yolox_candidates(levels):
    return sum((q.h * q.w) if isinstance(q, YoloxLevel) else (q[6] * q[7]) for q in levels)


class HandParams(C.Structure):
    _fields_ = [("confidence_threshold", C.c_float), ("nms_iou_threshold", C.c_float), ("max_hands", C.c_uint32), ("frame_width", C.c_int32),
                ("frame_height", C.c_int32)]


HAND_MAX = 10
HANDDEC_SET_MAX = 32
KP_VISIBILITY = {"UNKNOWN": 0, "VISIBLE": 1, "OCCLUDED": 2}
HAND_DET = np.dtype([("xmin", "<f4"), ("ymin", "<f4"), ("xmax", "<f4"), ("ymax", "<f4"), ("rotation", "<f4"), ("rotation_od", "<f4"), ("confidence", "<f4"),
                     ("index", "<u4"), ("x", "<i4"), ("y", "<i4"), ("width", "<i4"), ("height", "<i4"), ("has_od", "<u4"), ("reserved", "<u4", (3,))])
HAND_KP = np.dtype([("count", "<u4"), ("positions", "<i4", (42,)), ("confidences", "<f4", (21,)), ("visibilities", "u1", (21,)), ("reserved", "u1", (11,))])


def _hand_params(params):
    if isinstance(params, HandParams) or not (hasattr(params[0], "__len__") or isinstance(params[0], HandParams)):
        params = [params]
    arr = (HandParams * max(len(params), 1))()
    for k, q in enumerate(params):
        if isinstance(q, HandParams):
            arr[k] = q
        else:
            frame = tuple(q[3:5]) if len(q) >= 5 and q[3] is not None else (0, 0)
            arr[k] = HandParams(float(q[0]), float(q[1]), int(q[2]), int(frame[0]), int(frame[1]))
    return arr, len(params)


class HsvDetectSettings(C.Structure):
    _fields_ = [("hue_ref", C.c_float), ("hue_var", C.c_float), ("saturation_ref", C.c_float),
                ("saturation_var", C.c_float), ("value_ref", C.c_float), ("value_var", C.c_float)]


class Mi355Error(RuntimeError):
    def __init__(self, status, message):
        super().__init__("mi355fx status %d: %s" % (status, message))
        self.status = status


_lib = None


def load_library():
    global _lib
    if _lib is not None:
        return _lib
    if not os.path.exists(LIB_PATH):
        raise ImportError("libmi355fx.so not built: run `make -C %s` (or __graft_entry__.build())" % PKG_ROOT)
    L = C.CDLL(LIB_PATH)
    vp, sz, i, u8p = C.c_void_p, C.c_size_t, C.c_int, C.c_void_p
    f32p = C.POINTER(C.c_float)
    sig = {
        "mi355_abi_version": (i, []),
        "mi355_device_count": (i, []),
        "mi355_ctx_create": (vp, [i, C.POINTER(i)]),
        "mi355_ctx_destroy": (None, [vp]),
        "mi355_ctx_last_error": (C.c_char_p, [vp]),
        "mi355_status_string": (C.c_char_p, [i]),
        "mi355_ctx_stream": (vp, [vp]),
        "mi355_ctx_set_stream": (i, [vp, vp]),
        "mi355_ctx_synchronize": (i, [vp]),
        "mi355_ctx_set_flag": (i, [vp, i, i]),
        "mi355_device_alloc": (vp, [vp, sz]),
        "mi355_device_free": (i, [vp, vp]),
        "mi355_memcpy_h2d": (i, [vp, vp, vp, sz]),
        "mi355_memcpy_d2h": (i, [vp, vp, vp, sz]),
        "mi355_hsv_colorlut_chain_batches_device": (i, [vp, vp, vp, i, i, sz, i, i, i, i, C.POINTER(HsvSettings), i]),
        "mi355_buf_alloc": (vp, [vp, sz]),
        "mi355_buf_ref": (vp, [vp]),
        "mi355_buf_unref": (None, [vp]),
        "mi355_buf_size": (sz, [vp]),
        "mi355_buf_device_ptr": (vp, [vp, vp, i]),
        "mi355_buf_commit": (i, [vp, vp]),
        "mi355_buf_map_host": (vp, [vp, i]),
        "mi355_buf_unmap_host": (i, [vp]),
        "mi355_buf_state": (i, [vp]),
        "mi355_ctx_transfer_counts": (i, [vp, C.POINTER(C.c_uint64), C.POINTER(C.c_uint64)]),
        "mi355_roundedcorners_set_mask": (i, [vp, u8p, i, i, i]),
        "mi355_roundedcorners_mask_device": (i, [vp, C.POINTER(vp), C.POINTER(sz), C.POINTER(i)]),
        "mi355_roundedcorners_append_device": (i, [vp, u8p, sz, sz, i]),
        "mi355_colordetect_frame": (i, [vp, u8p, sz, i, i, i, u8p, C.POINTER(C.c_int)]),
        "mi355_colordetect_frames_device": (i, [vp, vp, sz, sz, i, i, i, i, u8p, C.POINTER(C.c_int)]),
        "mi355_colordetect_histogram_device": (i, [vp, vp, sz, i, i, C.POINTER(C.c_uint32), C.POINTER(C.c_int)]),
        "mi355_hsvfilter_frame_ip": (i, [vp, u8p, sz, i, i, i, C.POINTER(HsvSettings)]),
        "mi355_hsvfilter_frames_device": (i, [vp, u8p, i, sz, i, i, i, i, C.POINTER(HsvSettings)]),
        "mi355_hsvdetect_frame": (i, [vp, u8p, sz, i, i, u8p, sz, i, i, i, C.POINTER(HsvDetectSettings)]),
        "mi355_hsvdetect_frames_device": (i, [vp, u8p, sz, i, i, u8p, sz, i, i, i, i, i, C.POINTER(HsvDetectSettings)]),
        "mi355_colorlut_load": (i, [vp, i, sz, f32p, f32p, f32p]),
        "mi355_colorlut_unload": (i, [vp]),
        "mi355_selftest_autopick": (i, [i, C.POINTER(C.c_uint64), C.POINTER(C.c_double), C.POINTER(C.c_double), i, C.POINTER(C.c_int), C.POINTER(C.c_int)]),
        "mi355_colorlut_kernel_choice": (i, [vp, i, C.POINTER(C.c_int), C.POINTER(C.c_double), C.POINTER(C.c_double)]),
        "mi355_shared_table_count": (i, []),
        "mi355_colorlut_last_kernel": (C.c_char_p, [vp]),
        "mi355_colorlut_brick_stats": (i, [vp, C.POINTER(C.c_uint64), C.POINTER(C.c_double), C.POINTER(C.c_int), i]),
        "mi355_colorlut_window_stats": (i, [vp, C.POINTER(C.c_uint64), i]),
        "mi355_selftest_brickwatch": (i, [i, C.POINTER(C.c_double), C.POINTER(C.c_double), C.POINTER(C.c_double), C.POINTER(C.c_double), i, C.POINTER(C.c_int)]),
        "mi355_colorlut_frame": (i, [vp, u8p, i, u8p, i, i, i, i]),
        "mi355_colorlut_frames_device": (i, [vp, u8p, sz, i, u8p, sz, i, i, i, i, i]),
        "mi355_hsv_colorlut_frames_device": (i, [vp, u8p, sz, i, u8p, sz, i, i, i, i, C.POINTER(HsvSettings)]),
        "mi355_echo_setup": (i, [vp, sz]),
        "mi355_echo_reset": (i, [vp]),
        "mi355_echo_process_f32": (i, [vp, vp, sz, sz, C.c_double, C.c_double]),
        "mi355_echo_process_f64": (i, [vp, vp, sz, sz, C.c_double, C.c_double]),
        "mi355_echo_process_device": (i, [vp, vp, sz, i, sz, C.c_double, C.c_double]),
        "mi355_echo_get_state": (i, [vp, vp, sz, C.POINTER(sz)]),
        "mi355_echo_setup_batch": (i, [vp, i, sz]),
        "mi355_echo_process_batch_device": (i, [vp, vp, sz, sz, i, vp, vp, vp]),
        "mi355_echo_get_state_batch": (i, [vp, i, vp, sz, C.POINTER(sz)]),
        "mi355_ebur128_setup": (i, [vp, C.c_uint, C.c_uint, C.c_uint, C.POINTER(C.c_int)]),
        "mi355_ebur128_setup_batch": (i, [vp, C.c_uint, C.c_uint, C.c_uint, C.c_uint, C.POINTER(C.c_int)]),
        "mi355_ebur128_add_frames_batch": (i, [vp, vp, sz, i]),
        "mi355_ebur128_add_frames_batch_device": (i, [vp, vp, sz, i]),
        "mi355_ebur128_loudness_batch": (i, [vp, i, C.POINTER(C.c_double)]),
        "mi355_ebur128_peak_batch": (i, [vp, i, C.POINTER(C.c_double)]),
        "mi355_ebur128_reset": (i, [vp]),
        "mi355_ebur128_teardown": (i, [vp]),
        "mi355_ebur128_add_frames": (i, [vp, vp, sz, i]),
        "mi355_ebur128_add_frames_planar": (i, [vp, C.POINTER(vp), sz, i]),
        "mi355_ebur128_loudness_momentary": (i, [vp, C.POINTER(C.c_double)]),
        "mi355_ebur128_loudness_shortterm": (i, [vp, C.POINTER(C.c_double)]),
        "mi355_ebur128_loudness_global": (i, [vp, C.POINTER(C.c_double)]),
        "mi355_ebur128_relative_threshold": (i, [vp, C.POINTER(C.c_double)]),
        "mi355_ebur128_loudness_range": (i, [vp, C.POINTER(C.c_double)]),
        "mi355_ebur128_sample_peak": (i, [vp, C.c_uint, C.POINTER(C.c_double)]),
        "mi355_ebur128_true_peak": (i, [vp, C.c_uint, C.POINTER(C.c_double)]),
        "mi355_loudnorm_setup": (i, [vp, C.c_uint, C.c_double, C.c_double, C.c_double, C.c_double]),
        "mi355_loudnorm_push": (i, [vp, vp, sz, vp, sz, C.POINTER(sz)]),
        "mi355_loudnorm_drain": (i, [vp, vp, sz, C.POINTER(sz), C.POINTER(i)]),
        "mi355_loudnorm_teardown": (i, [vp]),
        "mi355_loudnorm_setup_batch": (i, [vp, C.c_uint, C.c_uint, C.c_double, C.c_double, C.c_double, C.c_double]),
        "mi355_loudnorm_batch_frame_size": (sz, [vp]),
        "mi355_loudnorm_process_batch": (i, [vp, vp, sz, sz, vp, sz, sz, C.POINTER(sz), i, i]),
        "mi355_host_alloc": (vp, [vp, sz]),
        "mi355_host_free": (i, [vp, vp]),
        "mi355_pipe_create": (vp, [vp, i, sz]),
        "mi355_pipe_destroy": (None, [vp]),
        "mi355_pipe_submit_hsvfilter": (i, [vp, u8p, sz, i, i, i, C.POINTER(HsvSettings), C.POINTER(C.c_uint64)]),
        "mi355_pipe_submit_colorlut": (i, [vp, u8p, i, u8p, i, i, i, i, C.POINTER(C.c_uint64)]),
        "mi355_pipe_submit_hsv_colorlut": (i, [vp, u8p, i, u8p, i, i, i, C.POINTER(HsvSettings), C.POINTER(C.c_uint64)]),
        "mi355_pipe_wait": (i, [vp, C.c_uint64]),
        "mi355_pipe_wait_all": (i, [vp]),
        "mi355_videocompare_hash_frame": (i, [vp, u8p, i, i, i, i, i, C.POINTER(C.c_uint64)]),
        "mi355_videocompare_hash_frames_device": (i, [vp, u8p, sz, i, i, i, i, i, i, C.POINTER(C.c_uint64)]),
        "mi355_videocompare_distance": (C.c_double, [i, C.c_uint64, C.c_uint64]),
        "mi355_dssim_create_image": (i, [vp, u8p, i, i, i, i, C.POINTER(vp)]),
        "mi355_dssim_create_image_device": (i, [vp, u8p, i, i, i, i, C.POINTER(vp)]),
        "mi355_dssim_free_image": (None, [vp, vp]),
        "mi355_dssim_compare": (i, [vp, vp, vp, C.POINTER(C.c_double)]),
        "mi355_dssim_compare_frames": (i, [vp, vp, C.POINTER(vp), i, i, i, i, i, C.POINTER(C.c_double)]),
        "mi355_dssim_compare_frames_device": (i, [vp, vp, C.POINTER(vp), i, i, i, i, i, C.POINTER(C.c_double)]),
        "mi355_issue_streams_round": (i, [C.POINTER(vp), i, C.POINTER(vp), C.POINTER(vp), i, i, i, i, C.POINTER(HsvSettings)]),
        "mi355_group_create": (vp, [i, i, C.POINTER(C.c_int)]),
        "mi355_group_destroy": (None, [vp]),
        "mi355_group_last_error": (C.c_char_p, [vp]),
        "mi355_group_submit_chain": (i, [vp, vp, u8p, u8p, i, i, i, i, C.POINTER(HsvSettings), C.POINTER(C.c_uint64)]),
        "mi355_group_submit_fused": (i, [vp, vp, u8p, u8p, i, i, i, i, C.POINTER(HsvSettings), C.POINTER(C.c_uint64)]),
        "mi355_group_flush": (i, [vp]),
        "mi355_pipe_set_group": (i, [vp, vp]),
        "mi355_group_wait": (i, [vp, C.c_uint64]),
        "mi355_group_order_after": (i, [vp, vp, C.c_uint64]),
        "mi355_group_wait_all": (i, [vp]),
        "mi355_group_stats": (i, [vp, C.POINTER(C.c_uint64)]),
        "mi355_group_set_rendezvous": (i, [vp, i, C.c_uint]),
        "mi355_group_set_compare_lanes": (i, [vp, i]),
        "mi355_group_submit_compare": (i, [vp, vp, u8p, u8p, i, i, i, i, i, C.POINTER(C.c_uint64)]),
        "mi355_group_wait_compare": (i, [vp, C.c_uint64, C.POINTER(C.c_double), C.POINTER(C.c_uint64)]),
        "mi355_group_compare_stats": (i, [vp, C.POINTER(C.c_uint64)]),
        "mi355_group_set_colordetect_rendezvous": (i, [vp, i, C.c_uint]),
        "mi355_group_submit_colordetect": (i, [vp, vp, vp, sz, i, i, i, C.POINTER(C.c_uint64)]),
        "mi355_group_wait_colordetect": (i, [vp, C.c_uint64, u8p, C.POINTER(C.c_int)]),
        "mi355_group_colordetect_stats": (i, [vp, C.POINTER(C.c_uint64)]),
        "mi355_selftest_colordetect_plan": (i, [i, i, C.POINTER(C.c_uint64), C.POINTER(C.c_uint32), C.POINTER(C.c_uint32), C.POINTER(C.c_uint64),
                                                C.POINTER(C.c_uint32)]),
        "mi355_group_set_hsvdetect_rendezvous": (i, [vp, i, C.c_uint]),
        "mi355_group_submit_hsvdetect": (i, [vp, vp, u8p, i, i, u8p, i, i, i, i, C.POINTER(HsvDetectSettings), C.POINTER(C.c_uint64)]),
        "mi355_group_wait_hsvdetect": (i, [vp, C.c_uint64]),
        "mi355_group_hsvdetect_stats": (i, [vp, C.POINTER(C.c_uint64)]),
        "mi355_selftest_hsvdetect_plan": (i, [i, i, C.c_uint, i, C.POINTER(C.c_uint64), C.POINTER(C.c_uint32), C.POINTER(C.c_uint32),
                                              C.POINTER(C.c_uint32)]),
        "mi355_agroup_create_echo": (vp, [i, i, sz, C.POINTER(C.c_int)]),
        "mi355_agroup_create_ebur128": (vp, [i, i, C.c_uint, C.c_uint, C.c_uint, C.POINTER(C.c_int), C.POINTER(C.c_int)]),
        "mi355_agroup_create_loudnorm": (vp, [i, i, C.c_uint, C.c_double, C.c_double, C.c_double, C.c_double, C.POINTER(C.c_int)]),
        "mi355_agroup_destroy": (None, [vp]),
        "mi355_agroup_last_error": (C.c_char_p, [vp]),
        "mi355_agroup_set_linger": (i, [vp, C.c_uint, C.c_uint]),
        "mi355_agroup_detach": (i, [vp, i]),
        "mi355_agroup_submit_echo": (i, [vp, i, vp, sz, i, sz, C.c_double, C.c_double, i, C.POINTER(C.c_uint64)]),
        "mi355_agroup_submit_ebur128": (i, [vp, i, vp, sz, i, i, C.POINTER(C.c_uint64)]),
        "mi355_agroup_ebur128_reset": (i, [vp, i]),
        "mi355_agroup_submit_loudnorm": (i, [vp, i, vp, sz, vp, sz, i, i, C.POINTER(C.c_uint64)]),
        "mi355_agroup_loudnorm_frame_size": (sz, [vp, i]),
        "mi355_agroup_wait": (i, [vp, C.c_uint64, C.POINTER(sz)]),
        "mi355_agroup_ebur128_loudness": (i, [vp, i, i, C.POINTER(C.c_double)]),
        "mi355_agroup_ebur128_peak": (i, [vp, i, i, C.c_uint, C.POINTER(C.c_double)]),
        "mi355_agroup_echo_get_state": (i, [vp, i, vp, sz, C.POINTER(sz)]),
        "mi355_agroup_stats": (i, [vp, C.POINTER(C.c_uint64)]),
        "mi355_agroup_loudnorm_push": (i, [vp, i, vp, sz, vp, sz, C.POINTER(sz)]),
        "mi355_agroup_loudnorm_drain": (i, [vp, i, vp, sz, C.POINTER(sz), C.POINTER(C.c_int)]),
        "mi355_agroup_shared_echo": (vp, [i, i, sz, C.POINTER(C.c_int), C.POINTER(C.c_int)]),
        "mi355_agingradio_setup": (i, [vp, C.c_uint, C.c_uint, C.c_uint, C.c_uint64]),
        "mi355_agingradio_process": (i, [vp, vp, sz, i, C.POINTER(AgingRadioSettings)]),
        "mi355_agingradio_process_device": (i, [vp, vp, sz, i, C.POINTER(AgingRadioSettings)]),
        "mi355_agingradio_get_state": (i, [vp, C.POINTER(C.c_double), C.c_uint, C.POINTER(C.c_uint64)]),
        "mi355_agingradio_reset": (i, [vp]),
        "mi355_agroup_create_agingradio": (vp, [i, i, C.POINTER(C.c_int)]),
        "mi355_agroup_shared_agingradio": (vp, [i, i, C.POINTER(C.c_int), C.POINTER(C.c_int)]),
        "mi355_agroup_agingradio_setup": (i, [vp, i, C.c_uint, C.c_uint, C.c_uint, C.c_uint64]),
        "mi355_agroup_submit_agingradio": (i, [vp, i, vp, sz, i, C.POINTER(AgingRadioSettings), i, C.POINTER(C.c_uint64)]),
        "mi355_agroup_agingradio_get_state": (i, [vp, i, C.POINTER(C.c_double), C.c_uint, C.POINTER(C.c_uint64)]),
        "mi355_mixer_setup": (i, [vp, C.c_uint, C.c_uint, vp]),
        "mi355_mixer_setup_minus1": (i, [vp, C.c_uint]),
        "mi355_mixer_process": (i, [vp, C.POINTER(MixerSegment), C.c_uint, C.POINTER(MixerOutput), C.c_uint, sz]),
        "mi355_mixer_process_device": (i, [vp, C.POINTER(MixerSegment), C.c_uint, C.POINTER(MixerOutput), C.c_uint, sz]),
        "mi355_mixer_reset": (i, [vp]),
        "mi355_yolodec_tensor": (i, [vp, vp, i, C.c_uint32, C.c_uint32, C.POINTER(YoloParams), vp, C.c_uint32, C.POINTER(C.c_uint32)]),
        "mi355_yolodec_tensors_device": (i, [vp, vp, sz, i, i, C.c_uint32, C.c_uint32, C.POINTER(YoloParams), vp, C.c_uint32, C.POINTER(C.c_uint32)]),
        "mi355_selftest_yolodec_check": (i, [sz, i, i, C.c_uint32, C.c_uint32]),
        "mi355_yolox_head_decode_device": (i, [vp, C.POINTER(YoloxLevel), i, i, C.c_uint32, vp, sz]),
        "mi355_yolox_head_dets_device": (i, [vp, C.POINTER(YoloxLevel), i, i, C.c_uint32, C.POINTER(YoloParams), vp, C.c_uint32, C.POINTER(C.c_uint32)]),
        "mi355_yolox_head_dets": (i, [vp, C.POINTER(YoloxLevel), i, C.c_uint32, C.POINTER(YoloParams), vp, C.c_uint32, C.POINTER(C.c_uint32)]),
        "mi355_yolox_input_frames_device": (i, [vp, vp, sz, sz, i, C.c_uint32, C.c_uint32, vp, sz]),
        "mi355_selftest_yolox_head_check": (i, [C.POINTER(YoloxLevel), i, i, C.c_uint32, sz]),
        "mi355_handdec_palm_tensor": (i, [vp, vp, C.c_uint32, C.POINTER(HandParams), vp, C.POINTER(C.c_uint32)]),
        "mi355_handdec_palm_tensors_device": (i, [vp, vp, sz, i, C.c_uint32, C.POINTER(HandParams), vp, C.POINTER(C.c_uint32)]),
        "mi355_handdec_landmarks_tensor": (i, [vp, vp, C.c_uint32, C.c_uint32, vp, C.c_uint32, C.POINTER(HandParams), vp, vp, C.POINTER(C.c_uint32)]),
        "mi355_handdec_landmarks_tensors_device": (i, [vp, vp, sz, i, C.c_uint32, C.c_uint32, vp, sz, C.c_uint32, C.POINTER(HandParams), vp, vp,
                                                       C.POINTER(C.c_uint32)]),
        "mi355_selftest_handdec_check": (i, [i, sz, i, C.c_uint32, C.c_uint32, sz, C.c_uint32, C.c_uint32, C.c_int32, C.c_int32]),
        "mi355_group_set_yolodec_rendezvous": (i, [vp, i, C.c_uint]),
        "mi355_group_submit_yolodec": (i, [vp, vp, vp, i, C.c_uint32, C.c_uint32, C.POINTER(YoloParams), C.c_uint32, C.POINTER(C.c_uint64)]),
        "mi355_group_wait_yolodec": (i, [vp, C.c_uint64, vp, C.POINTER(C.c_uint32)]),
        "mi355_group_yolodec_stats": (i, [vp, C.POINTER(C.c_uint64)]),
        "mi355_selftest_yolodec_set_plan": (i, [i, C.POINTER(C.c_int)] + [C.POINTER(C.c_uint32)] * 5 + [C.POINTER(C.c_uint64)] * 4),
        "mi355_group_submit_yolox_head": (i, [vp, vp, C.POINTER(YoloxLevel), i, C.c_uint32, C.POINTER(YoloParams), C.c_uint32, C.POINTER(C.c_uint64)]),
        "mi355_group_yolox_head_stats": (i, [vp, C.POINTER(C.c_uint64)]),
        "mi355_selftest_yolox_head_set_plan": (i, [i, C.POINTER(C.c_int)] + [C.POINTER(C.c_uint32)] * 3 + [C.POINTER(C.c_int)] + [C.POINTER(C.c_uint32)] * 5 +
                                               [C.POINTER(C.c_uint64)] * 3 + [C.POINTER(C.c_uint32), C.POINTER(C.c_uint64)]),
        "mi355_group_set_handdec_rendezvous": (i, [vp, i, C.c_uint]),
        "mi355_group_submit_handdec_palm": (i, [vp, vp, vp, C.c_uint32, C.POINTER(HandParams), C.POINTER(C.c_uint64)]),
        "mi355_group_submit_handdec_landmarks": (i, [vp, vp, vp, C.c_uint32, C.c_uint32, vp, C.c_uint32, C.POINTER(HandParams), C.POINTER(C.c_uint64)]),
        "mi355_group_wait_handdec": (i, [vp, C.c_uint64, vp, vp, C.POINTER(C.c_uint32)]),
        "mi355_group_handdec_stats": (i, [vp, C.POINTER(C.c_uint64)]),
        "mi355_selftest_handdec_set_plan": (i, [i, C.POINTER(C.c_int)] + [C.POINTER(C.c_uint32)] * 3 + [C.POINTER(C.c_uint64)]),
        "mi355_selftest_mixer_plan": (i, [i] + [C.POINTER(C.c_uint32)] * 4 + [C.POINTER(C.c_uint64)] + [C.POINTER(C.c_uint32)] * 4 + [C.c_uint32]
                                      + [C.POINTER(C.c_uint32)] * 3),
        "mi355_agroup_create_mixer": (vp, [i, i, C.POINTER(C.c_int)]),
        "mi355_agroup_shared_mixer": (vp, [i, i, C.POINTER(C.c_int), C.POINTER(C.c_int)]),
        "mi355_agroup_mixer_setup": (i, [vp, i, C.c_uint, C.c_uint, vp]),
# ... 678 lines not shown
        st = C.c_int(0)
        self.h = self.L.mi355_ctx_create(device, C.byref(st))
        if not self.h:
            raise Mi355Error(st.value, self.L.mi355_status_string(st.value).decode())
        self.device = device

    def close(self):
        if getattr(self, "h", None):
            self.L.mi355_ctx_destroy(self.h)
            self.h = None

    def __del__(self):
        try:
            self.close()
        except Exception:
            pass

    def __enter__(self):
        return self

    def __exit__(self, *a):
        self.close()

    def _ck(self, rc):
        if rc != 0:
            raise Mi355Error(rc, self.L.mi355_ctx_last_error(self.h).decode("utf-8", "replace"))

    @property
    def stream(self):
        return self.L.mi355_ctx_stream(self.h)

    def set_stream(self, hip_stream):
        self._ck(self.L.mi355_ctx_set_stream(self.h, hip_stream))

    def synchronize(self):
        self._ck(self.L.mi355_ctx_synchronize(self.h))

    def set_flag(self, flag, value):
        self._ck(self.L.mi355_ctx_set_flag(self.h, flag, int(value)))

    def alloc(self, nbytes):
        p = self.L.mi355_device_alloc(self.h, nbytes)
        if not p:
            raise Mi355Error(ERR_OOM, self.L.mi355_ctx_last_error(self.h).decode())
        return p

    def free(self, dptr):
        self._ck(self.L.mi355_device_free(self.h, dptr))

    def h2d(self, dptr, arr):
        arr = np.ascontiguousarray(arr)
        self._ck(self.L.mi355_memcpy_h2d(self.h, dptr, arr.ctypes.data, arr.nbytes))

    def d2h(self, arr, dptr):
        assert arr.flags.c_contiguous
        self._ck(self.L.mi355_memcpy_d2h(self.h, arr.ctypes.data, dptr, arr.nbytes))

    def chain_batches_device(self, src_ptrs, dst_ptrs, n_frames, frame_pitch, stride, width, height, fmt, settings, lanes=1):
        key = (tuple(src_ptrs), tuple(dst_ptrs))
        arr = self._chain_arrays.get(key) if hasattr(self, "_chain_arrays") else None
        if arr is None:
            if not hasattr(self, "_chain_arrays"):
                self._chain_arrays = {}
            n = len(src_ptrs)
            arr = self._chain_arrays[key] = ((C.c_void_p * n)(*src_ptrs), (C.c_void_p * n)(*dst_ptrs))
        hs = HsvSettings(*[float(v) for v in settings])
        self._ck(self.L.mi355_hsv_colorlut_chain_batches_device(self.h, arr[0], arr[1], len(src_ptrs), n_frames, frame_pitch, stride, width, height,
                                                                FMT[fmt], C.byref(hs), lanes))

    def buf_alloc(self, nbytes):
        b = self.L.mi355_buf_alloc(self.h, nbytes)
        if not b:
            raise Mi355Error(ERR_OOM, self.L.mi355_ctx_last_error(self.h).decode())
        return DeviceBuffer(self, b)

    def transfer_counts(self):
        a, b = C.c_uint64(0), C.c_uint64(0)
        self._ck(self.L.mi355_ctx_transfer_counts(self.h, C.byref(a), C.byref(b)))
        return int(a.value), int(b.value)

    def roundedcorners_set_mask(self, mask, width, height, stride):
        if mask is None:
            self._ck(self.L.mi355_roundedcorners_set_mask(self.h, None, 0, 0, 0))
        else:
            mask = np.ascontiguousarray(mask, dtype=np.uint8)
            assert mask.size >= stride * ((height + 1) & ~1)
            self._ck(self.L.mi355_roundedcorners_set_mask(self.h, mask.ctypes.data, width, height, stride))

    def roundedcorners_mask_device(self):
        p, n, st = C.c_void_p(), C.c_size_t(0), C.c_int(0)
        self._ck(self.L.mi355_roundedcorners_mask_device(self.h, C.byref(p), C.byref(n), C.byref(st)))
        return p.value, int(n.value), int(st.value)

    def roundedcorners_append_device(self, d_frames, frame_pitch, alpha_offset, n_frames):
        self._ck(self.L.mi355_roundedcorners_append_device(self.h, d_frames, frame_pitch, alpha_offset, n_frames))

    def hsvfilter_frame_ip(self, data, width, stride, fmt, settings, data_len=None):
        s = HsvSettings(*[float(v) for v in settings])
        n = data.nbytes if data_len is None else data_len
        self._ck(self.L.mi355_hsvfilter_frame_ip(self.h, _ptr(data), n, width, stride, FMT[fmt], C.byref(s)))
        return data

    def hsvfilter_frames_device(self, dptr, n_frames, frame_pitch, width, height, stride, fmt, settings):
        s = HsvSettings(*[float(v) for v in settings])
        self._ck(self.L.mi355_hsvfilter_frames_device(self.h, dptr, n_frames, frame_pitch, width, height, stride, FMT[fmt], C.byref(s)))

    def time_hsvfilter_device(self, dptr, n_frames, frame_pitch, width, height, stride, fmt, settings, iters):
        s = HsvSettings(*[float(v) for v in settings])
        ms = C.c_float(0)
        self._ck(self.L.mi355_time_hsvfilter_device(self.h, dptr, n_frames, frame_pitch, width, height, stride, FMT[fmt], C.byref(s), iters, C.byref(ms)))
        return ms.value

    def hsvdetect_frame(self, src, src_stride, src_fmt, dst, dst_stride, dst_fmt, width, settings):
        s = HsvDetectSettings(*[float(v) for v in settings])
        self._ck(self.L.mi355_hsvdetect_frame(self.h, _ptr(src), src.nbytes, src_stride, FMT[src_fmt], _ptr(dst), dst.nbytes,
                                              dst_stride, FMT[dst_fmt], width, C.byref(s)))
        return dst

    def hsvdetect_frames_device(self, d_src, src_pitch, src_stride, src_fmt, d_dst, dst_pitch, dst_stride, dst_fmt, n_frames, width, height, settings):
        s = None if settings is None else C.byref(HsvDetectSettings(*[float(v) for v in settings]))
        self._ck(self.L.mi355_hsvdetect_frames_device(self.h, d_src, src_pitch, src_stride, FMT[src_fmt], d_dst, dst_pitch, dst_stride, FMT[dst_fmt],
                                                      n_frames, width, height, s))

    def colorlut_load(self, is3d, size, table, scale=(1.0, 1.0, 1.0), offset=(0.0, 0.0, 0.0)):
        t = np.ascontiguousarray(table, dtype=np.float32).ravel()
        assert t.size == (4 * size ** 3 if is3d else 3 * size), "table size mismatch"
        sc = np.ascontiguousarray(scale, dtype=np.float32)
        of = np.ascontiguousarray(offset, dtype=np.float32)
        fp = C.POINTER(C.c_float)
        self._ck(self.L.mi355_colorlut_load(self.h, int(is3d), size, t.ctypes.data_as(fp), sc.ctypes.data_as(fp), of.ctypes.data_as(fp)))

    def colorlut_unload(self):
        self._ck(self.L.mi355_colorlut_unload(self.h))

    def colorlut_kernel_choice(self, fused=False):
        k, a, b = C.c_int(0), C.c_double(0), C.c_double(0)
        self._ck(self.L.mi355_colorlut_kernel_choice(self.h, int(fused), C.byref(k), C.byref(a), C.byref(b)))
        return bool(k.value), a.value, b.value

    def colorlut_kernel_name(self):
        return (self.L.mi355_colorlut_last_kernel(self.h) or b"").decode()

    def colorlut_brick_stats(self, reset=False):
        c = (C.c_uint64 * 2)()
        f, h = C.c_double(0), C.c_int(0)
        self._ck(self.L.mi355_colorlut_brick_stats(self.h, c, C.byref(f), C.byref(h), int(reset)))
        return int(c[0]), int(c[1]), f.value, int(h.value)

    def colorlut_window_stats(self, reset=False):
        c = (C.c_uint64 * 3)()
        self._ck(self.L.mi355_colorlut_window_stats(self.h, c, int(reset)))
        return int(c[0]), int(c[1]), int(c[2])

    def colorlut_frame(self, src, src_stride, dst, dst_stride, width, height, fmt="RGBA"):
        self._ck(self.L.mi355_colorlut_frame(self.h, _ptr(src), src_stride, _ptr(dst), dst_stride, width, height, FMT[fmt]))
        return dst

    def colorlut_frames_device(self, d_src, src_pitch, src_stride, d_dst, dst_pitch, dst_stride, n_frames, width, height, fmt="RGBA"):
        self._ck(self.L.mi355_colorlut_frames_device(self.h, d_src, src_pitch, src_stride, d_dst, dst_pitch, dst_stride, n_frames, width, height, FMT[fmt]))

    def time_colorlut_device(self, d_src, src_pitch, src_stride, d_dst, dst_pitch, dst_stride, n_frames, width, height, fmt, iters):
        ms = C.c_float(0)
        self._ck(self.L.mi355_time_colorlut_device(self.h, d_src, src_pitch, src_stride, d_dst, dst_pitch, dst_stride, n_frames, width, height, FMT[fmt], iters, C.byref(ms)))
        return ms.value

    def hsv_colorlut_frames_device(self, d_src, src_pitch, src_stride, d_dst, dst_pitch, dst_stride, n_frames, width, height, settings):
        s = HsvSettings(*[float(v) for v in settings])
        self._ck(self.L.mi355_hsv_colorlut_frames_device(self.h, d_src, src_pitch, src_stride, d_dst, dst_pitch, dst_stride, n_frames, width, height, C.byref(s)))

    def time_hsv_colorlut_device(self, d_src, src_pitch, src_stride, d_dst, dst_pitch, dst_stride, n_frames, width, height, settings, iters):
        s = HsvSettings(*[float(v) for v in settings])
        ms = C.c_float(0)
        self._ck(self.L.mi355_time_hsv_colorlut_device(self.h, d_src, src_pitch, src_stride, d_dst, dst_pitch, dst_stride, n_frames, width, height, C.byref(s), iters, C.byref(ms)))
        return ms.value

    def loudnorm_setup(self, channels, loudness_target=-24.0, loudness_range_target=7.0, max_true_peak=-2.0, offset=0.0):
        self._ck(self.L.mi355_loudnorm_setup(self.h, channels, loudness_target, loudness_range_target, max_true_peak, offset))
        self._ln_channels = channels

    def loudnorm_push(self, data):
        a = np.ascontiguousarray(data, dtype=np.float64).reshape(-1)
        frames = a.size // self._ln_channels
        cap = (frames // 19200 + 32) * 19200
        out = np.zeros(cap * self._ln_channels, np.float64)
        n = C.c_size_t(0)
        self._ck(self.L.mi355_loudnorm_push(self.h, a.ctypes.data, frames, out.ctypes.data, cap, C.byref(n)))
        return out[: n.value * self._ln_channels]

    def loudnorm_drain(self):
        cap = 31 * 19200 + 3 * 192000
        out = np.zeros(cap * self._ln_channels, np.float64)
        n, eos = C.c_size_t(0), C.c_int(0)
        self._ck(self.L.mi355_loudnorm_drain(self.h, out.ctypes.data, cap, C.byref(n), C.byref(eos)))
        return None if eos.value else out[: n.value * self._ln_channels]

    def loudnorm_teardown(self):
        self._ck(self.L.mi355_loudnorm_teardown(self.h))

    def loudnorm_setup_batch(self, n_streams, channels, loudness_target=-24.0, loudness_range_target=7.0, max_true_peak=-2.0, offset=0.0):
        self._ck(self.L.mi355_loudnorm_setup_batch(self.h, n_streams, channels, loudness_target, loudness_range_target, max_true_peak, offset))
        self._lnb = (n_streams, channels)

    def loudnorm_batch_frame_size(self):
        return int(self.L.mi355_loudnorm_batch_frame_size(self.h))

    def loudnorm_process_batch(self, data, final=False):
        S, ch = self._lnb
        a = np.ascontiguousarray(data, dtype=np.float64).reshape(S, -1)
        frames = a.shape[1] // ch
        cap = 31 * 19200 if final else max(frames, 19200)
        out = np.zeros((S, cap * ch), np.float64)
        n = C.c_size_t(0)
        self._ck(self.L.mi355_loudnorm_process_batch(self.h, a.ctypes.data if a.size else None, a.shape[1], frames, out.ctypes.data, cap * ch, cap, C.byref(n), int(final), 0))
        return out[:, : n.value * ch]

    def loudnorm_process_batch_device(self, d_in, stream_stride, frames, d_out, out_stride, cap_frames, final=False):
        n = C.c_size_t(0)
        self._ck(self.L.mi355_loudnorm_process_batch(self.h, d_in, stream_stride, frames, d_out, out_stride, cap_frames, C.byref(n), int(final), 1))
        return n.value

    def host_array(self, nbytes):
        p = self.L.mi355_host_alloc(self.h, nbytes)
        if not p:
            raise Mi355Error(ERR_OOM, self.L.mi355_ctx_last_error(self.h).decode("utf-8", "replace"))
        arr = np.ctypeslib.as_array((C.c_uint8 * nbytes).from_address(p))
        self._pinned = getattr(self, "_pinned", {})
        self._pinned[arr.ctypes.data] = p
        return arr

    def host_free(self, arr):
        p = self._pinned.pop(arr.ctypes.data)
        self._ck(self.L.mi355_host_free(self.h, p))

    def pipe_create(self, depth, max_frame_bytes):
        p = self.L.mi355_pipe_create(self.h, depth, max_frame_bytes)
        if not p:
            raise Mi355Error(ERR_INVALID_ARG, self.L.mi355_ctx_last_error(self.h).decode("utf-8", "replace"))
        return p

    def pipe_destroy(self, pipe):
        self.L.mi355_pipe_destroy(pipe)

    def pipe_submit_hsvfilter(self, pipe, data, width, stride, fmt, settings):
        s = HsvSettings(*[float(v) for v in settings])
        t = C.c_uint64(0)
        self._ck(self.L.mi355_pipe_submit_hsvfilter(pipe, _ptr(data), data.nbytes, width, stride, FMT[fmt], C.byref(s), C.byref(t)))
        return t.value

    def pipe_submit_colorlut(self, pipe, src, src_stride, dst, dst_stride, width, height, fmt="RGBA"):
        t = C.c_uint64(0)
        self._ck(self.L.mi355_pipe_submit_colorlut(pipe, _ptr(src), src_stride, _ptr(dst), dst_stride, width, height, FMT[fmt], C.byref(t)))
        return t.value

    def pipe_submit_hsv_colorlut(self, pipe, src, src_stride, dst, dst_stride, width, height, settings):
        s = HsvSettings(*[float(v) for v in settings])
        t = C.c_uint64(0)
        self._ck(self.L.mi355_pipe_submit_hsv_colorlut(pipe, _ptr(src), src_stride, _ptr(dst), dst_stride, width, height, C.byref(s), C.byref(t)))
        return t.value

    def pipe_set_group(self, pipe, group):
        self._ck(self.L.mi355_pipe_set_group(pipe, group.h if group is not None else None))

    def pipe_wait(self, pipe, ticket):
        self._ck(self.L.mi355_pipe_wait(pipe, ticket))

    def pipe_wait_all(self, pipe):
        self._ck(self.L.mi355_pipe_wait_all(pipe))

    COLORDETECT_FORMATS = ("RGB", "RGBA", "ARGB", "BGR", "BGRA")

    def colordetect_frame(self, data, fmt, quality=10, max_colors=2):
        a = np.ascontiguousarray(data, dtype=np.uint8).reshape(-1)
        pal = np.zeros(255 * 3, np.uint8)
        n = C.c_int(0)
        self._ck(self.L.mi355_colordetect_frame(self.h, a.ctypes.data, a.nbytes, FMT[fmt], quality, max_colors, pal.ctypes.data, C.byref(n)))
        return [tuple(int(x) for x in pal[3 * k:3 * k + 3]) for k in range(n.value)]

    def colordetect_frames_device(self, d_frames, frame_pitch, data_len, n_frames, fmt, quality=10, max_colors=2):
        pal = np.zeros(max(n_frames, 1) * 255 * 3, np.uint8)
        n = (C.c_int * max(n_frames, 1))()
        self._ck(self.L.mi355_colordetect_frames_device(self.h, d_frames, frame_pitch, data_len, n_frames, FMT[fmt], quality, max_colors,
                                                        pal.ctypes.data, n))
        return [[tuple(int(x) for x in pal[(f * 255 + k) * 3:(f * 255 + k) * 3 + 3]) for k in range(n[f])] for f in range(n_frames)]

    def colordetect_histogram_device(self, d_data, data_len, fmt, quality=10):
        hist = np.zeros(32768, np.uint32)
        box = (C.c_int * 6)()
        self._ck(self.L.mi355_colordetect_histogram_device(self.h, d_data, data_len, FMT[fmt], quality,
                                                           hist.ctypes.data_as(C.POINTER(C.c_uint32)), box))
        b = tuple(box[k] for k in range(6))
        return hist, (None if b[0] < 0 else b)

    HASH_ALGO = {"mean": 0, "gradient": 1, "vertgradient": 2, "doublegradient": 3, "blockhash": 4, "dssim": 5}

    def videocompare_hash_frame(self, frame, stride, width, height, fmt="RGBA", algo="blockhash"):
        h = C.c_uint64(0)
        self._ck(self.L.mi355_videocompare_hash_frame(self.h, _ptr(frame), stride, width, height, FMT[fmt], self.HASH_ALGO[algo], C.byref(h)))
        return h.value

    def videocompare_hash_frames_device(self, d_frames, frame_pitch, stride, n_frames, width, height, fmt="RGBA", algo="blockhash"):
        hs = (C.c_uint64 * max(n_frames, 1))()
        self._ck(self.L.mi355_videocompare_hash_frames_device(self.h, d_frames, frame_pitch, stride, n_frames, width, height, FMT[fmt],
                                                              self.HASH_ALGO[algo], hs))
        return [hs[k] for k in range(n_frames)]

    def videocompare_distance(self, a, b, algo="blockhash"):
# ... 420 lines not shown
```

include/mi355fx.h:

```cpp
#ifndef MI355FX_H
#define MI355FX_H

#include <stddef.h>
#include <stdint.h>

#ifdef __cplusplus
extern "C" {
#endif

#define MI355FX_ABI_VERSION 1

typedef enum mi355_status {
  MI355_OK = 0,
  MI355_ERR_INVALID_ARG = -1,
  MI355_ERR_NO_DEVICE = -2,
  MI355_ERR_HIP = -3,
  MI355_ERR_NOT_CONFIGURED = -4,
  MI355_ERR_OUT_OF_MEMORY = -5,
  MI355_ERR_UNSUPPORTED = -6,
  MI355_ERR_TIMEOUT = -7
} mi355_status;

typedef enum mi355_video_format {
  MI355_FMT_RGBX = 0,
  MI355_FMT_XRGB = 1,
  MI355_FMT_BGRX = 2,
  MI355_FMT_XBGR = 3,
  MI355_FMT_RGBA = 4,
  MI355_FMT_ARGB = 5,
  MI355_FMT_BGRA = 6,
  MI355_FMT_ABGR = 7,
  MI355_FMT_RGB = 8,
  MI355_FMT_BGR = 9,
  MI355_FMT_RGBA64_LE = 10,
  MI355_FMT_RGBA64_BE = 11
} mi355_video_format;

typedef struct mi355_ctx mi355_ctx;


int mi355_abi_version(void);
int mi355_device_count(void);
mi355_ctx *mi355_ctx_create(int device, int *status);
void mi355_ctx_destroy(mi355_ctx *ctx);
const char *mi355_ctx_last_error(const mi355_ctx *ctx);
const char *mi355_status_string(int status);
void *mi355_ctx_stream(mi355_ctx *ctx);
int mi355_ctx_set_stream(mi355_ctx *ctx, void *hip_stream);
int mi355_ctx_synchronize(mi355_ctx *ctx);

typedef enum mi355_flag {
  MI355_FLAG_FORCE_GENERIC = 1,
  MI355_FLAG_HSV_BLOCKS_PER_CU = 2,
  MI355_FLAG_LUT_VARIANT = 4,
  MI355_FLAG_HSV_TABLE = 6,
  MI355_FLAG_LUT_STAGGER = 5,
  MI355_FLAG_FUSED_VARIANT = 3,
  MI355_FLAG_BRICK_TILES_PER_RUN = 7,
  MI355_FLAG_DSSIM_TRANSLUCENT = 11,
  MI355_FLAG_DSSIM_FAST = 19,
  MI355_FLAG_BRICK_FOLD_AXIS = 10,
  MI355_FLAG_BRICK_PRIO = 9,
  MI355_FLAG_HRTF_METHOD = 12,
  MI355_FLAG_BLOCKHASH_ANY_SIZE = 15,
  MI355_FLAG_HSV_NT = 14,
  MI355_FLAG_WINDOW_ORDER = 17,
  MI355_FLAG_WINDOW_STATS = 18,
  MI355_FLAG_WINDOW_MIN_STEPS = 13,
  MI355_FLAG_BRICK_SETS = 8
} mi355_flag;
int mi355_ctx_set_flag(mi355_ctx *ctx, int flag, int value);

void *mi355_device_alloc(mi355_ctx *ctx, size_t bytes);
int mi355_device_free(mi355_ctx *ctx, void *dptr);
int mi355_memcpy_h2d(mi355_ctx *ctx, void *dptr, const void *host, size_t bytes);
int mi355_memcpy_d2h(mi355_ctx *ctx, void *host, const void *dptr, size_t bytes);

typedef struct mi355_hsv_settings {
  float hue_shift;
  float saturation_mul;
  float saturation_off;
  float value_mul;
  float value_off;
} mi355_hsv_settings;

int mi355_hsvfilter_frame_ip(mi355_ctx *ctx, uint8_t *data, size_t data_len, int width, int stride,
                             int format, const mi355_hsv_settings *settings);
int mi355_hsvfilter_frames_device(mi355_ctx *ctx, uint8_t *d_data, int n_frames, size_t frame_pitch,
                                  int width, int height, int stride, int format,
                                  const mi355_hsv_settings *settings);

typedef struct mi355_hsvdetect_settings {
  float hue_ref, hue_var;
  float saturation_ref, saturation_var;
  float value_ref, value_var;
} mi355_hsvdetect_settings;

int mi355_hsvdetect_frame(mi355_ctx *ctx, const uint8_t *src, size_t src_len, int src_stride,
                          int src_format, uint8_t *dst, size_t dst_len, int dst_stride,
                          int dst_format, int width, const mi355_hsvdetect_settings *settings);
int mi355_hsvdetect_frames_device(mi355_ctx *ctx, const uint8_t *d_src, size_t src_pitch,
                                  int src_stride, int src_format, uint8_t *d_dst, size_t dst_pitch,
                                  int dst_stride, int dst_format, int n_frames, int width,
                                  int height, const mi355_hsvdetect_settings *settings);

int mi355_colorlut_load(mi355_ctx *ctx, int is3d, size_t size, const float *table,
                        const float domain_scale[3], const float domain_offset[3]);
int mi355_colorlut_unload(mi355_ctx *ctx);
int mi355_colorlut_kernel_choice(mi355_ctx *ctx, int fused, int *table_in_use, double *ms_per_mpx_compute, double *ms_per_mpx_table);
int mi355_shared_table_count(void);
const char *mi355_colorlut_last_kernel(mi355_ctx *ctx);
int mi355_colorlut_brick_stats(mi355_ctx *ctx, uint64_t counters[2], double *last_miss_fraction, int *level, int reset);
int mi355_colorlut_window_stats(mi355_ctx *ctx, uint64_t counters[3], int reset);
int mi355_selftest_brickwatch(int n_calls, const double *miss0, const double *slow0, const double *miss1, const double *slow1, int lag,
                              int *level_out);
int mi355_selftest_autopick(int n_calls, const uint64_t *n_vec, const double *ms_compute, const double *ms_table, int lag,
                            int *kind_out, int *measured_out);
int mi355_colorlut_frame(mi355_ctx *ctx, const uint8_t *src, int src_stride, uint8_t *dst,
                         int dst_stride, int width, int height, int format);
int mi355_colorlut_frames_device(mi355_ctx *ctx, const uint8_t *d_src, size_t src_pitch,
                                 int src_stride, uint8_t *d_dst, size_t dst_pitch, int dst_stride,
                                 int n_frames, int width, int height, int format);

int mi355_issue_streams_round(mi355_ctx *const *ctxs, int n_streams, uint8_t *const *d_src, uint8_t *const *d_dst,
                              int width, int height, int stride, int format, const mi355_hsv_settings *settings);

typedef struct mi355_group mi355_group;
mi355_group *mi355_group_create(int device, int max_batch, int *status);
void mi355_group_destroy(mi355_group *group);
const char *mi355_group_last_error(mi355_group *group);
int mi355_group_submit_chain(mi355_group *group, mi355_ctx *ctx, uint8_t *d_src, uint8_t *d_dst, int width, int height,
                             int stride, int format, const mi355_hsv_settings *settings, uint64_t *ticket);
int mi355_group_submit_fused(mi355_group *group, mi355_ctx *ctx, uint8_t *d_src, uint8_t *d_dst, int width, int height,
                             int stride, int format, const mi355_hsv_settings *settings, uint64_t *ticket);
int mi355_group_flush(mi355_group *group);
int mi355_group_order_after(mi355_group *group, mi355_ctx *ctx, uint64_t ticket);
int mi355_group_wait(mi355_group *group, uint64_t ticket);
int mi355_group_wait_all(mi355_group *group);
int mi355_group_stats(mi355_group *group, uint64_t stats[3]);
int mi355_group_submit_round(mi355_group *group, mi355_ctx *const *ctxs, int n_streams, uint8_t *const *d_src,
                             uint8_t *const *d_dst, int width, int height, int stride, int format,
                             const mi355_hsv_settings *settings);
int mi355_group_submit_round_fused(mi355_group *group, mi355_ctx *const *ctxs, int n_streams, uint8_t *const *d_src,
                                   uint8_t *const *d_dst, int width, int height, int stride, int format,
                                   const mi355_hsv_settings *settings);

int mi355_group_set_rendezvous(mi355_group *group, int expected_streams, unsigned linger_us);
int mi355_group_set_compare_lanes(mi355_group *group, int lanes);
int mi355_group_submit_compare(mi355_group *group, mi355_ctx *ctx, const uint8_t *d_ref, const uint8_t *d_frame, int stride, int width, int height,
                               int format, int algo, uint64_t *ticket);
int mi355_group_wait_compare(mi355_group *group, uint64_t ticket, double *distance, uint64_t hashes[2]);
int mi355_group_compare_stats(mi355_group *group, uint64_t stats[3]);

#define MI355_COLORDETECT_SET_MAX 32
int mi355_group_set_colordetect_rendezvous(mi355_group *group, int expected_streams, unsigned linger_us);
int mi355_group_submit_colordetect(mi355_group *group, mi355_ctx *ctx, const uint8_t *d_data, size_t data_len, int format, int quality,
                                   int max_colors, uint64_t *ticket);
int mi355_group_wait_colordetect(mi355_group *group, uint64_t ticket, uint8_t palette_rgb[255 * 3], int *n_colors);
int mi355_group_colordetect_stats(mi355_group *group, uint64_t stats[4]);
int mi355_selftest_colordetect_plan(int n_cu, int n_jobs, const uint64_t *n_samples, uint32_t *first_block, uint32_t *blocks,
                                    uint64_t *samples_per_block, uint32_t *total_blocks);

#define MI355_HSVDETECT_SET_MAX 32
int mi355_group_set_hsvdetect_rendezvous(mi355_group *group, int expected_streams, unsigned linger_us);
int mi355_group_submit_hsvdetect(mi355_group *group, mi355_ctx *ctx, const uint8_t *d_src, int src_stride, int src_format,
                                 uint8_t *d_dst, int dst_stride, int dst_format, int width, int height,
                                 const mi355_hsvdetect_settings *settings, uint64_t *ticket);
int mi355_group_wait_hsvdetect(mi355_group *group, uint64_t ticket);
int mi355_group_hsvdetect_stats(mi355_group *group, uint64_t stats[4]);
int mi355_selftest_hsvdetect_plan(int n_cu, int blocks_per_cu, unsigned units_per_block, int n_jobs, const uint64_t *units,
                                  uint32_t *first_block, uint32_t *blocks, uint32_t *total_blocks);

typedef struct mi355_agroup mi355_agroup;
mi355_agroup *mi355_agroup_create_echo(int device, int n_members, size_t ring_len, int *status);
mi355_agroup *mi355_agroup_create_ebur128(int device, int n_members, unsigned channels, unsigned rate, unsigned mode, const int *channel_class,
                                          int *status);
mi355_agroup *mi355_agroup_create_loudnorm(int device, int n_members, unsigned channels, double loudness_target, double loudness_range_target,
                                           double max_true_peak, double offset, int *status);
void mi355_agroup_destroy(mi355_agroup *group);
const char *mi355_agroup_last_error(mi355_agroup *group);
int mi355_agroup_set_linger(mi355_agroup *group, unsigned linger_us, unsigned timeout_ms);
int mi355_agroup_detach(mi355_agroup *group, int member);
int mi355_agroup_submit_echo(mi355_agroup *group, int member, void *data, size_t n, int is_f64, size_t delay_samples, double intensity,
                             double feedback, int device_data, uint64_t *ticket);
int mi355_agroup_submit_ebur128(mi355_agroup *group, int member, const void *data, size_t frames, int sample_format, int device_data,
                                uint64_t *ticket);
int mi355_agroup_ebur128_reset(mi355_agroup *group, int member);
int mi355_agroup_submit_loudnorm(mi355_agroup *group, int member, const double *data, size_t frames, double *out, size_t out_capacity_frames,
                                 int final_frame, int device_data, uint64_t *ticket);
size_t mi355_agroup_loudnorm_frame_size(mi355_agroup *group, int member);
int mi355_agroup_loudnorm_push(mi355_agroup *group, int member, const double *data, size_t frames, double *out, size_t out_capacity_frames,
                               size_t *out_frames);
int mi355_agroup_loudnorm_drain(mi355_agroup *group, int member, double *out, size_t out_capacity_frames, size_t *out_frames, int *eos);
int mi355_agroup_wait(mi355_agroup *group, uint64_t ticket, size_t *out_frames);
int mi355_agroup_ebur128_loudness(mi355_agroup *group, int member, int what, double *out);
int mi355_agroup_ebur128_peak(mi355_agroup *group, int member, int true_peak, unsigned channel, double *out);
int mi355_agroup_echo_get_state(mi355_agroup *group, int member, double *ring_out, size_t ring_len, size_t *pos_out);
int mi355_agroup_stats(mi355_agroup *group, uint64_t stats[3]);
mi355_agroup *mi355_agroup_shared_echo(int device, int n_members, size_t ring_len, int *member, int *status);
mi355_agroup *mi355_agroup_shared_ebur128(int device, int n_members, unsigned channels, unsigned rate, unsigned mode, const int *channel_class,
                                          int *member, int *status);
mi355_agroup *mi355_agroup_shared_loudnorm(int device, int n_members, unsigned channels, double loudness_target, double loudness_range_target,
                                           double max_true_peak, double offset, int *member, int *status);
void mi355_agroup_release(mi355_agroup *group, int member);
mi355_group *mi355_group_shared(int device, int *status);
void mi355_group_release(mi355_group *group);

int mi355_hsv_colorlut_frames_device(mi355_ctx *ctx, const uint8_t *d_src, size_t src_pitch,
                                     int src_stride, uint8_t *d_dst, size_t dst_pitch, int dst_stride,
                                     int n_frames, int width, int height,
                                     const mi355_hsv_settings *settings);

int mi355_echo_setup(mi355_ctx *ctx, size_t ring_len);
int mi355_echo_reset(mi355_ctx *ctx);
int mi355_echo_process_f32(mi355_ctx *ctx, float *data, size_t n, size_t delay_samples,
                           double intensity, double feedback);
int mi355_echo_process_f64(mi355_ctx *ctx, double *data, size_t n, size_t delay_samples,
                           double intensity, double feedback);
int mi355_echo_process_device(mi355_ctx *ctx, void *d_data, size_t n, int is_f64,
                              size_t delay_samples, double intensity, double feedback);
int mi355_echo_get_state(mi355_ctx *ctx, double *ring_out, size_t ring_len, size_t *pos_out);
int mi355_echo_setup_batch(mi355_ctx *ctx, int n_streams, size_t ring_len);
int mi355_echo_process_batch_device(mi355_ctx *ctx, void *d_data, size_t stream_stride, size_t n, int is_f64,
                                    const size_t *delay_samples, const double *intensity, const double *feedback);
int mi355_echo_get_state_batch(mi355_ctx *ctx, int stream, double *ring_out, size_t ring_len, size_t *pos_out);

typedef enum mi355_ebur128_mode {
  MI355_EBUR128_MOMENTARY = 1, MI355_EBUR128_SHORT_TERM = 2, MI355_EBUR128_GLOBAL = 4,
  MI355_EBUR128_LOUDNESS_RANGE = 8, MI355_EBUR128_SAMPLE_PEAK = 16, MI355_EBUR128_TRUE_PEAK = 32
} mi355_ebur128_mode;
int mi355_ebur128_setup(mi355_ctx *ctx, unsigned channels, unsigned rate, unsigned mode, const int *channel_class);
int mi355_ebur128_setup_batch(mi355_ctx *ctx, unsigned n_streams, unsigned channels, unsigned rate, unsigned mode, const int *channel_class);
int mi355_ebur128_add_frames_batch(mi355_ctx *ctx, const void *data, size_t frames, int sample_format);
int mi355_ebur128_add_frames_batch_device(mi355_ctx *ctx, const void *d_data, size_t frames, int sample_format);
int mi355_ebur128_loudness_batch(mi355_ctx *ctx, int what, double *out);
int mi355_ebur128_peak_batch(mi355_ctx *ctx, int true_peak, double *out);
int mi355_ebur128_reset(mi355_ctx *ctx);
int mi355_ebur128_teardown(mi355_ctx *ctx);
int mi355_ebur128_add_frames(mi355_ctx *ctx, const void *data, size_t frames, int sample_format);
int mi355_ebur128_add_frames_planar(mi355_ctx *ctx, const void *const *planes, size_t frames, int sample_format);
int mi355_ebur128_loudness_momentary(mi355_ctx *ctx, double *out);
int mi355_ebur128_loudness_shortterm(mi355_ctx *ctx, double *out);
int mi355_ebur128_loudness_global(mi355_ctx *ctx, double *out);
int mi355_ebur128_relative_threshold(mi355_ctx *ctx, double *out);
int mi355_ebur128_loudness_range(mi355_ctx *ctx, double *out);
int mi355_ebur128_sample_peak(mi355_ctx *ctx, unsigned channel, double *out);
int mi355_ebur128_true_peak(mi355_ctx *ctx, unsigned channel, double *out);

int mi355_loudnorm_setup(mi355_ctx *ctx, unsigned channels, double loudness_target,
                         double loudness_range_target, double max_true_peak, double offset);
int mi355_loudnorm_push(mi355_ctx *ctx, const double *data, size_t frames, double *out,
                        size_t out_capacity_frames, size_t *out_frames);
int mi355_loudnorm_drain(mi355_ctx *ctx, double *out, size_t out_capacity_frames, size_t *out_frames,
                         int *eos);
int mi355_loudnorm_teardown(mi355_ctx *ctx);
int mi355_loudnorm_setup_batch(mi355_ctx *ctx, unsigned n_streams, unsigned channels, double loudness_target,
                               double loudness_range_target, double max_true_peak, double offset);
size_t mi355_loudnorm_batch_frame_size(mi355_ctx *ctx);
int mi355_loudnorm_process_batch(mi355_ctx *ctx, const double *data, size_t stream_stride, size_t frames,
                                 double *out, size_t out_stream_stride, size_t out_capacity_frames,
                                 size_t *out_frames, int final_frame, int device_data);

typedef enum mi355_hash_algo {
  MI355_HASH_MEAN = 0, MI355_HASH_GRADIENT = 1, MI355_HASH_VERTGRADIENT = 2, MI355_HASH_DOUBLEGRADIENT = 3,
  MI355_HASH_BLOCKHASH = 4, MI355_HASH_DSSIM = 5
} mi355_hash_algo;
// ... 286 lines not shown
```

Measured before the change: 45150.

## Add bounding-box LUT kernel that stages per-tile table bricks in LDS

Adds a colorlut box kernel: each wave loads a tile of pixels, reduces the min/max RGB bounding box, copies just the covering 4x4x4 table bricks into LDS, and then does its lookups from LDS rather than gathering from the global table. Tiles whose box exceeds the brick capacity fall back to global gathers and bump a counter. A watcher samples that fallback share, leaves the box path when it is high and re-probes it with exponential backoff. The fused hsv+colorlut auto path now uses the watched box kernel, which adds periodic counter snapshots, memsets and event traffic.

```diff
diff --git a/gst-plugins-rs_amd/csrc/boxwatch.hpp b/gst-plugins-rs_amd/csrc/boxwatch.hpp
--- /dev/null
+++ b/gst-plugins-rs_amd/csrc/boxwatch.hpp
@@ -0,0 +1,49 @@
+#pragma once
+
+namespace mi355 {
+
+struct BoxWatch {
+  bool on_box = true;
+  bool probing = false;
+  unsigned retry_in = 0;
+  unsigned period = 0;
+  double last_share = 0.0;
+};
+
+constexpr unsigned kBoxWatchSnapEvery = 16;
+constexpr unsigned kBoxWatchPeriodMin = 64, kBoxWatchPeriodMax = 1024;
+constexpr double kBoxShareLeave = 0.30, kBoxShareReturn = 0.20;
+
+inline bool boxwatch_next(BoxWatch &W, bool can_probe) {
+  if (W.on_box) return true;
+  if (W.probing) return false;
+  if (W.retry_in > 0) { W.retry_in--; return false; }
+  if (!can_probe) return false;
+  W.probing = true;
+  return true;
+}
+
+inline void boxwatch_snapshot(BoxWatch &W, double share, bool probe) {
+  W.last_share = share;
+  if (probe) {
+    if (!W.probing) return;
+    W.probing = false;
+    if (share < kBoxShareReturn) {
+      W.on_box = true;
+      W.period = 0;
+      W.retry_in = 0;
+    } else {
+      W.period = W.period ? (W.period * 2 > kBoxWatchPeriodMax ? kBoxWatchPeriodMax : W.period * 2) : kBoxWatchPeriodMin;
+      W.retry_in = W.period;
+    }
+    return;
+  }
+  if (!W.on_box) return;
+  if (share > kBoxShareLeave) {
+    W.on_box = false;
+    W.period = kBoxWatchPeriodMin;
+    W.retry_in = W.period;
+  }
+}
+
+}
diff --git a/gst-plugins-rs_amd/csrc/colorlut_box.hip b/gst-plugins-rs_amd/csrc/colorlut_box.hip
--- /dev/null
+++ b/gst-plugins-rs_amd/csrc/colorlut_box.hip
@@ -0,0 +1,335 @@
+#include "internal.hpp"
+#include "colorlut_box.hpp"
+#include <type_traits>
+
+namespace mi355 {
+
+namespace {
+
+typedef uint32_t u4_t __attribute__((ext_vector_type(4)));
+typedef uint32_t u2_t __attribute__((ext_vector_type(2)));
+typedef unsigned short us2_t __attribute__((ext_vector_type(2)));
+
+constexpr unsigned box_lds_bytes(unsigned cap) { return (256 + 4 * cap * 64) * 4; }
+constexpr unsigned box_waves_per_simd(unsigned cap) { return 160 * 1024 / box_lds_bytes(cap); }
+constexpr int kBoxCounterSlots = 64, kBoxCounterStride = 32;
+
+__device__ __forceinline__ uint32_t box_spread3(uint32_t v) {
+  v &= 0x000000ffu;
+  v = (v | (v << 8)) & 0x0000f00fu;
+  v = (v | (v << 4)) & 0x000c30c3u;
+  v = (v | (v << 2)) & 0x00249249u;
+  return v;
+}
+__device__ __forceinline__ uint32_t pk_min(uint32_t a, uint32_t b) {
+  return __builtin_bit_cast(uint32_t, __builtin_elementwise_min(__builtin_bit_cast(us2_t, a), __builtin_bit_cast(us2_t, b)));
+}
+__device__ __forceinline__ uint32_t pk_max(uint32_t a, uint32_t b) {
+  return __builtin_bit_cast(uint32_t, __builtin_elementwise_max(__builtin_bit_cast(us2_t, a), __builtin_bit_cast(us2_t, b)));
+}
+__device__ __forceinline__ unsigned uni(unsigned v) { return (unsigned)__builtin_amdgcn_readfirstlane((int)v); }
+
+}
+
+template <bool MULTI, unsigned CAP, unsigned ROWS>
+__global__ __launch_bounds__(256, box_waves_per_simd(CAP)) void colorlut_box_kernel(const u4_t *__restrict__ src, u4_t *__restrict__ dst, unsigned w4, unsigned sw4, unsigned dw4, unsigned rows,
+                                                            unsigned src_bytes, unsigned dst_bytes, unsigned n_cols, unsigned tiles_per_frame, const uint32_t *__restrict__ table,
+                                                            unsigned *__restrict__ fallbacks, MultiFramePtrs srcs, MultiFramePtrs dsts) {
+  static_assert(CAP % 16 == 0 && CAP >= 16 && CAP <= 64 && ROWS % 8 == 0, "whole groups of four wave loads; the gather path's strip fits the box; wave loads in pairs");
+  constexpr int kBoxLoads = ROWS / 4;
+  constexpr unsigned kBoxWaveWords = CAP * 64;
+  extern __shared__ uint32_t box_lds[];
+  uint32_t *s_spread = box_lds;
+  s_spread[threadIdx.x] = box_spread3(threadIdx.x);
+  __syncthreads();
+  const unsigned wave = uni(threadIdx.x >> 6), lane = threadIdx.x & 63;
+  uint32_t *x = box_lds + 256 + wave * kBoxWaveWords;
+  unsigned t = blockIdx.x;
+  if (MULTI) {
+    const unsigned frame = t / tiles_per_frame;
+    t -= frame * tiles_per_frame;
+    src = (const u4_t *)srcs.p[frame];
+    dst = (u4_t *)dsts.p[frame];
+  }
+  const unsigned tx = t % n_cols, ty = t / n_cols;
+  const unsigned col0 = tx * kBoxTileW4 + wave * 16u;
+  if (col0 >= w4) return;
+  const unsigned g = lane & 15u, sub = lane >> 4;
+  const unsigned col = col0 + g, row0 = ty * ROWS + sub;
+  const unsigned cc = col < w4 ? col : w4 - 1u;
+  const __amdgpu_buffer_rsrc_t srs = __builtin_amdgcn_make_buffer_rsrc((void *)src, 0, (int)src_bytes, 0x00020000);
+  u4_t P[kBoxLoads];
+  if ((ty + 1u) * ROWS <= rows) {
+    const uint32_t o = (row0 * sw4 + cc) << 4;
+#pragma unroll
+    for (int k = 0; k < kBoxLoads; k++) P[k] = __builtin_amdgcn_raw_buffer_load_b128(srs, (int)o, (int)(k * 64u * sw4), 2 );
+  } else {
+#pragma unroll
+    for (int k = 0; k < kBoxLoads; k++) {
+      const unsigned r = row0 + 4u * k, cr = r < rows ? r : rows - 1u;
+      P[k] = __builtin_amdgcn_raw_buffer_load_b128(srs, (int)((cr * sw4 + cc) << 4), 0, 2 );
+    }
+  }
+  auto wave_sync = [] {
+    __builtin_amdgcn_fence(__ATOMIC_ACQ_REL, "wavefront");
+    __builtin_amdgcn_wave_barrier();
+  };
+
+  uint32_t lo_rb = 0x00ff00ffu, lo_g = 0x00ff00ffu, hi_rb = 0u, hi_g = 0u;
+#pragma unroll
+  for (int k = 0; k < kBoxLoads; k++) {
+    const uint32_t px[4] = {P[k].x, P[k].y, P[k].z, P[k].w};
+#pragma unroll
+    for (int c = 0; c < 4; c++) {
+      const uint32_t rb = px[c] & 0x00ff00ffu, ga = (px[c] >> 8) & 0x00ff00ffu;
+      lo_rb = pk_min(lo_rb, rb);
+      hi_rb = pk_max(hi_rb, rb);
+      lo_g = pk_min(lo_g, ga);
+      hi_g = pk_max(hi_g, ga);
+    }
+  }
+#pragma unroll
+  for (int o = 32; o > 0; o >>= 1) {
+    lo_rb = pk_min(lo_rb, (uint32_t)__shfl_xor((int)lo_rb, o));
+    hi_rb = pk_max(hi_rb, (uint32_t)__shfl_xor((int)hi_rb, o));
+    lo_g = pk_min(lo_g, (uint32_t)__shfl_xor((int)lo_g, o));
+    hi_g = pk_max(hi_g, (uint32_t)__shfl_xor((int)hi_g, o));
+  }
+  lo_rb = uni(lo_rb); hi_rb = uni(hi_rb); lo_g = uni(lo_g); hi_g = uni(hi_g);
+  const unsigned r0 = lo_rb & 0xfcu, g0 = lo_g & 0xfcu, b0 = (lo_rb >> 16) & 0xfcu;
+  const unsigned nr = (((hi_rb & 0xffu) | 3u) - r0 + 1u) >> 2, ng = (((hi_g & 0xffu) | 3u) - g0 + 1u) >> 2, nb = ((((hi_rb >> 16) & 0xffu) | 3u) - b0 + 1u) >> 2;
+  const unsigned nbricks = nr * ng * nb;
+
+  if (nbricks <= CAP) {
+    const unsigned R = 4u * nr, RG = R * 4u * ng, nrg = nr * ng;
+    const unsigned m_r = (65536u + nr - 1u) / nr, m_rg = (65536u + nrg - 1u) / nrg;
+    const unsigned lane_e = 2u * ((g >> 1) & 1u) + R * 2u * ((g >> 2) & 1u) + RG * (2u * (g >> 3) + (g & 1u));
+    const __amdgpu_buffer_rsrc_t trs = __builtin_amdgcn_make_buffer_rsrc((void *)table, 0, 1 << 26, 0x00020000);
+    auto copy = [&](auto ngroups) {
+      constexpr int NL = 4 * decltype(ngroups)::value;
+      u4_t v[NL];
+      uint32_t e0[NL];
+#pragma unroll
+      for (int it = 0; it < NL; it++) {
+        const unsigned n_ = 4u * it + sub, ok = n_ < nbricks, n = ok ? n_ : 0u;
+        const unsigned k = (n * m_rg) >> 16, rem = n - k * nrg, j = (rem * m_r) >> 16, i = rem - j * nr;
+        const uint32_t slot = s_spread[r0 + 4u * i] | (s_spread[g0 + 4u * j] << 1) | (s_spread[b0 + 4u * k] << 2);
+        e0[it] = ok ? lane_e + 4u * i + R * 4u * j + RG * 4u * k : 0xffffffffu;
+        v[it] = __builtin_amdgcn_raw_buffer_load_b128(trs, ok ? (int)(slot * 4u + g * 16u) : (int)0x80000000u, 0, 0);
+      }
+#pragma unroll
+      for (int it = 0; it < NL; it++)
+        if (e0[it] != 0xffffffffu) {
+          const u2_t a = {v[it].x, v[it].y}, b = {v[it].z, v[it].w};
+          *(u2_t *)(x + e0[it]) = a;
+          *(u2_t *)(x + e0[it] + R) = b;
+        }
+    };
+    if (nbricks <= 16u) copy(std::integral_constant<int, 1>{});
+    else if (CAP <= 32u || nbricks <= 32u) copy(std::integral_constant<int, 2>{});
+    else copy(std::integral_constant<int, (CAP > 32u ? 4 : 2)>{});
+    wave_sync();
+    const uint32_t base = 0u - (r0 + R * g0 + RG * b0);
+#pragma unroll
+    for (int k = 0; k < kBoxLoads; k++) {
+      const uint32_t px[4] = {P[k].x, P[k].y, P[k].z, P[k].w};
+      uint32_t o[4];
+#pragma unroll
+      for (int c = 0; c < 4; c++) o[c] = x[(px[c] & 0xffu) + base + ((px[c] >> 8) & 0xffu) * R + ((px[c] >> 16) & 0xffu) * RG];
+      P[k].x = (o[0] & 0x00ffffffu) | (px[0] & 0xff000000u);
+      P[k].y = (o[1] & 0x00ffffffu) | (px[1] & 0xff000000u);
+      P[k].z = (o[2] & 0x00ffffffu) | (px[2] & 0xff000000u);
+      P[k].w = (o[3] & 0x00ffffffu) | (px[3] & 0xff000000u);
+    }
+  } else {
+    if (lane == 0) atomicAdd(fallbacks + (blockIdx.x % kBoxCounterSlots) * kBoxCounterStride, 1u);
+    auto index = [&](uint32_t p) -> uint32_t { return s_spread[p & 0xffu] | (s_spread[(p >> 8) & 0xffu] << 1) | (s_spread[(p >> 16) & 0xffu] << 2); };
+#pragma unroll
+    for (int k = 0; k < kBoxLoads; k += 2) {
+      *(u4_t *)(x + lane * 4) = P[k];
+      *(u4_t *)(x + 256 + lane * 4) = P[k + 1];
+      wave_sync();
+      uint32_t px[8], o[8];
+#pragma unroll
+      for (int j = 0; j < 8; j++) px[j] = x[j * 64 + lane];
+#pragma unroll
+      for (int j = 0; j < 8; j++) o[j] = table[index(px[j])];
+#pragma unroll
+      for (int j = 0; j < 8; j++) x[j * 64 + lane] = (o[j] & 0x00ffffffu) | (px[j] & 0xff000000u);
+      wave_sync();
+      P[k] = *(u4_t *)(x + lane * 4);
+      P[k + 1] = *(u4_t *)(x + 256 + lane * 4);
+      wave_sync();
+    }
+  }
+
+  const __amdgpu_buffer_rsrc_t drs = __builtin_amdgcn_make_buffer_rsrc(dst, 0, (int)dst_bytes, 0x00020000);
+#pragma unroll
+  for (int k = 0; k < kBoxLoads; k++) {
+    const unsigned r = row0 + 4u * k;
+    const uint32_t off = col < w4 && r < rows ? (r * dw4 + col) << 4 : 0x80000000u;
+    __builtin_amdgcn_raw_buffer_store_b128(P[k], drs, (int)off, 0, 2 );
+  }
+}
+
+constexpr unsigned kBoxSmallCap = 32, kBoxSmallRows = 32;
+static unsigned box_tile_rows(bool small) { return small ? kBoxSmallRows : kBoxTileRows; }
+
+bool box_applicable(unsigned w4, unsigned sw4, unsigned dw4, size_t rows) {
+  if (w4 < 32 || rows == 0 || rows >= (1u << 30)) return false;
+  if (rows * dw4 * 16 >= (1ull << 31) || rows * sw4 * 16 >= (1ull << 31)) return false;
+  const size_t tiles = (size_t)((w4 + kBoxTileW4 - 1) / kBoxTileW4) * ((rows + kBoxSmallRows - 1) / kBoxSmallRows);
+  return tiles < (1u << 31);
+}
+
+bool box_multi_applicable(unsigned w4, size_t frame_rows, int n_frames) {
+  return n_frames >= 1 && n_frames <= kMultiFrames && box_applicable(w4, w4, w4, frame_rows) &&
+         (size_t)((w4 + kBoxTileW4 - 1) / kBoxTileW4) * ((frame_rows + kBoxSmallRows - 1) / kBoxSmallRows) * (size_t)n_frames < (1u << 31);
+}
+
+constexpr size_t kBoxCounterBytes = (size_t)kBoxCounterSlots * kBoxCounterStride * sizeof(unsigned);
+
+static int box_counters_ensure(mi355_ctx *ctx, unsigned **d_counters, hipStream_t stream) {
+  if (*d_counters) return MI355_OK;
+  int rc;
+  if ((rc = check_hip(ctx, hipMalloc((void **)d_counters, kBoxCounterBytes), "hipMalloc(box counters)"))) return rc;
+  return check_hip(ctx, hipMemsetAsync(*d_counters, 0, kBoxCounterBytes, stream), "hipMemsetAsync(box counters)");
+}
+
+static int box_launch(mi355_ctx *ctx, const uint32_t *table, const uint8_t *d_src, uint8_t *d_dst, unsigned w4, unsigned sw4, unsigned dw4, size_t rows, unsigned *d_counters,
+                      bool small) {
+  const unsigned n_cols = (w4 + kBoxTileW4 - 1) / kBoxTileW4, n_rows = (unsigned)((rows + box_tile_rows(small) - 1) / box_tile_rows(small));
+#define MI355_BOX(CAP, ROWS) hipLaunchKernelGGL((colorlut_box_kernel<false, CAP, ROWS>), dim3(n_cols * n_rows), dim3(256), box_lds_bytes(CAP), ctx->stream, (const u4_t *)d_src, \
+                                                (u4_t *)d_dst, w4, sw4, dw4, (unsigned)rows, (unsigned)(rows * sw4 * 16), (unsigned)(rows * dw4 * 16), n_cols, n_cols * n_rows, table, \
+                                                d_counters, MultiFramePtrs{}, MultiFramePtrs{})
+  if (small) MI355_BOX(kBoxSmallCap, kBoxSmallRows);
+  else MI355_BOX(kBoxCapBricks, kBoxTileRows);
+#undef MI355_BOX
+  return check_hip(ctx, hipGetLastError(), "colorlut box kernel launch");
+}
+static unsigned long long box_wave_count(unsigned w4, size_t rows, bool small) {
+  return (unsigned long long)((w4 + 15) / 16) * ((rows + box_tile_rows(small) - 1) / box_tile_rows(small));
+}
+
+int launch_box_table(mi355_ctx *ctx, const uint32_t *table, const uint8_t *d_src, uint8_t *d_dst, unsigned w4, unsigned sw4, unsigned dw4, size_t rows, bool small) {
+  int rc;
+  if ((rc = box_counters_ensure(ctx, &ctx->d_box_counters, ctx->stream))) return rc;
+  ctx->box_waves += box_wave_count(w4, rows, small);
+  return box_launch(ctx, table, d_src, d_dst, w4, sw4, dw4, rows, ctx->d_box_counters, small);
+}
+
+static void box_harvest(BoxWatchState &S) {
+  if (!S.pending) return;
+  if (hipEventQuery(S.ev) != hipSuccess) { (void)hipGetLastError(); return; }
+  S.pending = false;
+  unsigned long long fallbacks = 0;
+  for (int i = 0; i < kBoxCounterSlots; i++) fallbacks += S.h_counters[i * kBoxCounterStride];
+  const bool was_on_box = S.w.on_box;
+  if (S.waves_snapshot) boxwatch_snapshot(S.w, (double)fallbacks / (double)S.waves_snapshot, S.probe_snapshot);
+  if (was_on_box && !S.w.on_box) S.stale = true;
+}
+
+bool box_watch_choose(mi355_ctx *ctx) {
+  BoxWatchState &S = ctx->box_watch;
+  box_harvest(S);
+  return boxwatch_next(S.w, !S.pending);
+}
+
+int launch_box_table_watched(mi355_ctx *ctx, const uint32_t *table, const uint8_t *d_src, uint8_t *d_dst, unsigned w4, unsigned sw4, unsigned dw4, size_t rows) {
+  BoxWatchState &S = ctx->box_watch;
+  int rc;
+  if (!S.ev) {
+    if ((rc = check_hip(ctx, hipHostMalloc((void **)&S.h_counters, kBoxCounterBytes), "hipHostMalloc(box watch)"))) return rc;
+    if ((rc = check_hip(ctx, hipEventCreateWithFlags(&S.ev, hipEventDisableTiming), "hipEventCreate(box watch)"))) return rc;
+  }
+  if ((rc = box_counters_ensure(ctx, &S.d_counters, ctx->stream))) return rc;
+  if (S.stale) {
+    if ((rc = check_hip(ctx, hipMemsetAsync(S.d_counters, 0, kBoxCounterBytes, ctx->stream), "box watch counters reset"))) return rc;
+    S.stale = false;
+    S.waves_since = 0;
+    S.launches_since = 0;
+  }
+  if ((rc = box_launch(ctx, table, d_src, d_dst, w4, sw4, dw4, rows, S.d_counters, true))) return rc;
+  S.waves_since += box_wave_count(w4, rows, true);
+  const unsigned need = S.w.probing ? 1u : kBoxWatchSnapEvery;
+  if (++S.launches_since < need || S.pending) return MI355_OK;
+  if ((rc = check_hip(ctx, hipMemcpyAsync(S.h_counters, S.d_counters, kBoxCounterBytes, hipMemcpyDeviceToHost, ctx->stream), "box watch snapshot"))) return rc;
+  if ((rc = check_hip(ctx, hipMemsetAsync(S.d_counters, 0, kBoxCounterBytes, ctx->stream), "box watch counters reset"))) return rc;
+  if ((rc = check_hip(ctx, hipEventRecord(S.ev, ctx->stream), "hipEventRecord(box watch)"))) return rc;
+  S.pending = true;
+  S.probe_snapshot = S.w.probing;
+  S.waves_snapshot = S.waves_since;
+  S.waves_since = 0;
+  S.launches_since = 0;
+  return MI355_OK;
+}
+
+int launch_box_table_multi(mi355_ctx *ctx, hipStream_t stream, const uint32_t *table, uint8_t *const *srcs, uint8_t *const *dsts, int n_frames, unsigned w4,
+                           size_t frame_rows, bool small) {
+  int rc;
+  if ((rc = box_counters_ensure(ctx, &ctx->d_box_counters, stream))) return rc;
+  MultiFramePtrs s{}, d{};
+  for (int f = 0; f < kMultiFrames; f++) { s.p[f] = srcs[f < n_frames ? f : 0]; d.p[f] = dsts[f < n_frames ? f : 0]; }
+  const unsigned n_cols = (w4 + kBoxTileW4 - 1) / kBoxTileW4, n_rows = (unsigned)((frame_rows + box_tile_rows(small) - 1) / box_tile_rows(small));
+  ctx->box_waves += box_wave_count(w4, frame_rows, small) * (unsigned)n_frames;
+#define MI355_BOX(CAP, ROWS) hipLaunchKernelGGL((colorlut_box_kernel<true, CAP, ROWS>), dim3(n_cols * n_rows * (unsigned)n_frames), dim3(256), box_lds_bytes(CAP), stream, \
+                                                (const u4_t *)nullptr, (u4_t *)nullptr, w4, w4, w4, (unsigned)frame_rows, (unsigned)(frame_rows * w4 * 16),                      \
+                                                (unsigned)(frame_rows * w4 * 16), n_cols, n_cols * n_rows, table, ctx->d_box_counters, s, d)
+  if (small) MI355_BOX(kBoxSmallCap, kBoxSmallRows);
+  else MI355_BOX(kBoxCapBricks, kBoxTileRows);
+#undef MI355_BOX
+  return check_hip(ctx, hipGetLastError(), "colorlut box kernel launch (multi-frame)");
+}
+
+int box_read_counters(mi355_ctx *ctx, unsigned long long out[2], bool reset) {
+  out[0] = ctx->box_waves;
+  out[1] = 0;
+  if (reset) ctx->box_waves = 0;
+  if (!ctx->d_box_counters) return MI355_OK;
+  unsigned h[kBoxCounterSlots * kBoxCounterStride];
+  int rc;
+  if ((rc = check_hip(ctx, hipMemcpyAsync(h, ctx->d_box_counters, sizeof(h), hipMemcpyDeviceToHost, ctx->stream), "hipMemcpyAsync(box counters)"))) return rc;
+  if (reset && (rc = check_hip(ctx, hipMemsetAsync(ctx->d_box_counters, 0, sizeof(h), ctx->stream), "hipMemsetAsync(box counters)"))) return rc;
+  if ((rc = check_hip(ctx, hipStreamSynchronize(ctx->stream), "hipStreamSynchronize"))) return rc;
+  for (int i = 0; i < kBoxCounterSlots; i++) out[1] += h[i * kBoxCounterStride];
+  return MI355_OK;
+}
+
+void box_release(mi355_ctx *ctx) {
+  BoxWatchState &S = ctx->box_watch;
+  if (ctx->d_box_counters) (void)hipFree(ctx->d_box_counters);
+  if (S.d_counters) (void)hipFree(S.d_counters);
+  if (S.h_counters) (void)hipHostFree(S.h_counters);
+  if (S.ev) (void)hipEventDestroy(S.ev);
+  ctx->d_box_counters = nullptr;
+  S = BoxWatchState{};
+}
+
+}
+
+extern "C" int mi355_selftest_boxwatch(int n_calls, const double *share, int lag, int *box_out) {
+  if (n_calls < 0 || !share || !box_out) return MI355_ERR_INVALID_ARG;
+  mi355::BoxWatch W;
+  bool pend = false, pend_probe = false;
+  int pend_ready = 0;
+  unsigned launches_since = 0;
+  double acc = 0.0, pend_share = 0.0;
+  for (int i = 0; i < n_calls; i++) {
+    if (pend && lag >= 0 && i >= pend_ready) {
+      pend = false;
+      const bool was_on_box = W.on_box;
+      mi355::boxwatch_snapshot(W, pend_share, pend_probe);
+      if (was_on_box && !W.on_box) { launches_since = 0; acc = 0.0; }
+    }
+    const bool box = mi355::boxwatch_next(W, !pend);
+    box_out[i] = box ? 1 : 0;
+    if (!box) continue;
+    acc += share[i];
+    launches_since++;
+    if (!pend && launches_since >= (W.probing ? 1u : mi355::kBoxWatchSnapEvery)) {
+      pend = true; pend_probe = W.probing; pend_share = acc / launches_since; pend_ready = i + 1 + lag;
+      launches_since = 0; acc = 0.0;
+    }
+  }
+  return MI355_OK;
+}
diff --git a/gst-plugins-rs_amd/csrc/colorlut_box.hpp b/gst-plugins-rs_amd/csrc/colorlut_box.hpp
--- /dev/null
+++ b/gst-plugins-rs_amd/csrc/colorlut_box.hpp
@@ -0,0 +1,38 @@
+#pragma once
+#include <hip/hip_runtime.h>
+#include <cstddef>
+#include <cstdint>
+#include "boxwatch.hpp"
+
+struct mi355_ctx;
+
+namespace mi355 {
+
+constexpr unsigned kBoxCapBricks = 64;
+constexpr unsigned kBoxTileW4 = 64, kBoxTileRows = 64;
+
+constexpr unsigned box_bricks(const unsigned lo[3], const unsigned hi[3]) {
+  unsigned n = 1;
+  for (int c = 0; c < 3; c++) n *= (((hi[c] | 3u) - (lo[c] & ~3u)) + 1u) >> 2;
+  return n;
+}
+
+bool box_applicable(unsigned w4, unsigned sw4, unsigned dw4, size_t rows);
+int launch_box_table(mi355_ctx *ctx, const uint32_t *table, const uint8_t *d_src, uint8_t *d_dst, unsigned w4, unsigned sw4, unsigned dw4, size_t rows, bool small);
+bool box_multi_applicable(unsigned w4, size_t frame_rows, int n_frames);
+int launch_box_table_multi(mi355_ctx *ctx, hipStream_t stream, const uint32_t *table, uint8_t *const *srcs, uint8_t *const *dsts, int n_frames, unsigned w4,
+                           size_t frame_rows, bool small);
+struct BoxWatchState {
+  BoxWatch w;
+  unsigned *d_counters = nullptr, *h_counters = nullptr;
+  hipEvent_t ev = nullptr;
+  bool pending = false, probe_snapshot = false, stale = false;
+  unsigned long long waves_since = 0, waves_snapshot = 0;
+  unsigned launches_since = 0;
+};
+bool box_watch_choose(mi355_ctx *ctx);
+int launch_box_table_watched(mi355_ctx *ctx, const uint32_t *table, const uint8_t *d_src, uint8_t *d_dst, unsigned w4, unsigned sw4, unsigned dw4, size_t rows);
+int box_read_counters(mi355_ctx *ctx, unsigned long long out[2], bool reset);
+void box_release(mi355_ctx *ctx);
+
+}
diff --git a/gst-plugins-rs_amd/csrc/colorlut_kernels.hip b/gst-plugins-rs_amd/csrc/colorlut_kernels.hip
--- a/gst-plugins-rs_amd/csrc/colorlut_kernels.hip
+++ b/gst-plugins-rs_amd/csrc/colorlut_kernels.hip
@@ -1513,7 +1513,7 @@
   return MI355_OK;
 }
 
-enum TableKernel { kTableGather = 0, kTableWindow = 1, kTableEither = 2 };
+enum TableKernel { kTableGather = 0, kTableWindow = 1, kTableEither = 2, kTableBox = 3, kTableBoxWatch = 4 };
 template <class Compute, class Ensure, class Table>
 static int auto_launch(mi355_ctx *ctx, AutoPick &A, size_t n_vec, Compute &&compute, Ensure &&ensure, Table &&table);
 static int launch_table_gather(mi355_ctx *ctx, const uint32_t *t, const uint8_t *d_src, uint8_t *d_dst, const Rgba8Geom &geo, int width, size_t rows, int morton);
@@ -1528,7 +1528,21 @@
 
 static int launch_table_raw(mi355_ctx *ctx, const uint32_t *t, const uint8_t *d_src, uint8_t *d_dst, const Rgba8Geom &geo, int width, size_t rows, int morton,
                             TableKernel sub, int *last_sub) {
-  const bool window_ok = morton && sub != kTableGather && width % 4 == 0 && window_applicable(ctx, (unsigned)width / 4, geo.dw4, rows);
+  if (sub == kTableBox && morton && width % 4 == 0 && box_applicable((unsigned)width / 4, geo.sw4, geo.dw4, rows)) {
+    if (last_sub) *last_sub = 2;
+    ctx->lut.last_kernel = "colorlut_box_kernel";
+    return launch_box_table(ctx, t, d_src, d_dst, (unsigned)width / 4, geo.sw4, geo.dw4, rows, ctx->lut_variant == 11);
+  }
+  if (sub == kTableBoxWatch) {
+    if (morton && width % 4 == 0 && window_applicable(ctx, (unsigned)width / 4, geo.dw4, rows) && box_applicable((unsigned)width / 4, geo.sw4, geo.dw4, rows) &&
+        !recently_written(ctx->device, d_src, (size_t)geo.sw4 * 16 * rows) && box_watch_choose(ctx)) {
+      if (last_sub) *last_sub = 2;
+      ctx->lut.last_kernel = "colorlut_box_kernel";
+      return launch_box_table_watched(ctx, t, d_src, d_dst, (unsigned)width / 4, geo.sw4, geo.dw4, rows);
+    }
+    sub = kTableEither;
+  }
+  const bool window_ok = morton && sub != kTableGather && sub != kTableBox && width % 4 == 0 && window_applicable(ctx, (unsigned)width / 4, geo.dw4, rows);
   const size_t src_bytes = (size_t)geo.sw4 * 16 * rows;
   const bool window = window_ok && (sub == kTableWindow || !recently_written(ctx->device, d_src, src_bytes));
   if (last_sub) *last_sub = window ? 1 : 0;
@@ -1609,8 +1623,8 @@
 }
 
 constexpr size_t kAutoMinVec = 16384;
-static bool table_variant(int v) { return v == 4 || v == 5 || v == 8 || v == 9; }
-static TableKernel table_variant_kernel(int v) { return v == 8 ? kTableWindow : (v == 9 ? kTableEither : kTableGather); }
+static bool table_variant(int v) { return v == 4 || v == 5 || v == 8 || v == 9 || v == 10 || v == 11; }
+static TableKernel table_variant_kernel(int v) { return v == 8 ? kTableWindow : (v == 9 ? kTableEither : (v == 10 || v == 11 ? kTableBox : kTableGather)); }
 
 int launch_colorlut(mi355_ctx *ctx, const uint8_t *d_src, size_t src_pitch, int src_stride, uint8_t *d_dst,
                     size_t dst_pitch, int dst_stride, int n_frames, int width, int height, int format) {
@@ -1654,7 +1668,7 @@
     L.pick[1].learn = 2;
   }
   return auto_launch(ctx, L.pick[1], n_vec, compute, [&]() { return table_ensure(ctx, 1, 1, &hs); },
-                     [&]() { return launch_table(ctx, 1, d_src, d_dst, geo, width, (size_t)n_frames * height, 1, &hs, kTableEither); });
+                     [&]() { return launch_table(ctx, 1, d_src, d_dst, geo, width, (size_t)n_frames * height, 1, &hs, kTableBoxWatch); });
 }
 
 int colorlut_multi_table(mi355_ctx *ctx, const uint32_t **table_out) {
@@ -1685,6 +1699,10 @@
     d.p[f] = dsts[f];
   }
   const unsigned w4 = (unsigned)width / 4;
+  if ((ctx->lut_variant == 10 || ctx->lut_variant == 11) && box_multi_applicable(w4, (size_t)height, n_frames)) {
+    ctx->lut.last_kernel = "colorlut_box_kernel";
+    return launch_box_table_multi(ctx, stream, table, srcs, dsts, n_frames, w4, (size_t)height, ctx->lut_variant == 11);
+  }
   if (from_hbm && ctx->lut_variant == 0 && window_multi_applicable(ctx, w4, (size_t)height, n_frames)) {
     ctx->lut.last_kernel = "colorlut_window_kernel";
     return launch_window_table_multi(ctx, stream, table, srcs, dsts, n_frames, w4, (size_t)height);
@@ -1744,7 +1762,7 @@
   if (ctx->hsv_table_mode == 2) {
     int rc = hsv_table_ensure(ctx, fmt, hs);
     T.last_table = true;
-    return rc ? rc : launch_table_raw(ctx, T.d_table, d_data, d_data, geo, width, rows, 1, kTableEither, nullptr);
+    return rc ? rc : launch_table_raw(ctx, T.d_table, d_data, d_data, geo, width, rows, 1, ctx->lut_variant == 10 || ctx->lut_variant == 11 ? kTableBox : kTableEither, nullptr);
   }
   if (n_vec < kAutoMinVec) return compute();
   if (same_hs(hs, T.seen_hs) && fmt.bgr == T.seen_bgr) { if (T.seen_stable < kStableCalls) T.seen_stable++; }
diff --git a/gst-plugins-rs_amd/csrc/ctx.hip b/gst-plugins-rs_amd/csrc/ctx.hip
--- a/gst-plugins-rs_amd/csrc/ctx.hip
+++ b/gst-plugins-rs_amd/csrc/ctx.hip
@@ -177,6 +177,7 @@
   lut_release(ctx);
   hsv_table_release(ctx);
   window_release(ctx);
+  box_release(ctx);
   loudnorm_release(ctx);
   loudnorm_batch_release(ctx);
   dssim_release(ctx);
@@ -223,7 +224,7 @@
   REQUIRE_CTX(ctx);
   if (flag == MI355_FLAG_FORCE_GENERIC) { ctx->force_generic = value != 0; return MI355_OK; }
   if (flag == MI355_FLAG_LUT_STAGGER && value >= 0 && value <= 4096) { ctx->lut_stagger = value; return MI355_OK; }
-  if (flag == MI355_FLAG_LUT_VARIANT && value >= 0 && value <= 9) { ctx->lut_variant = value; return MI355_OK; }
+  if (flag == MI355_FLAG_LUT_VARIANT && value >= 0 && value <= 11) { ctx->lut_variant = value; return MI355_OK; }
   if (flag == MI355_FLAG_BRICK_TILES_PER_RUN && value >= 0 && value <= 4096) { ctx->brick_tiles_per_run = value; return MI355_OK; }
   if (flag == MI355_FLAG_BRICK_FOLD_AXIS && value >= 0 && value <= 2) { ctx->brick_fold_axis = value; return MI355_OK; }
   if (flag == MI355_FLAG_DSSIM_TRANSLUCENT && (value == 0 || value == 1)) { ctx->dssim_translucent = value; return MI355_OK; }
@@ -443,7 +444,7 @@
   const AutoPick &A = fused == 2 ? ctx->hsv_table.pick : ctx->lut.pick[fused ? 1 : 0];
   if (table_in_use)
     *table_in_use = fused == 2 ? (ctx->hsv_table.last_table ? 1 : 0)
-                               : (ctx->lut_variant == 4 || ctx->lut_variant == 5 || ctx->lut_variant == 8 || ctx->lut_variant == 9 || (ctx->lut_variant == 0 && A.t_table > 0.0 && A.table));
+                               : (ctx->lut_variant == 4 || ctx->lut_variant == 5 || ctx->lut_variant == 8 || ctx->lut_variant == 9 || ctx->lut_variant == 10 || ctx->lut_variant == 11 || (ctx->lut_variant == 0 && A.t_table > 0.0 && A.table));
   if (ms_per_mpx_compute) *ms_per_mpx_compute = A.t_compute * 250000.0;
   if (ms_per_mpx_table) *ms_per_mpx_table = A.t_table * 250000.0;
   return MI355_OK;
@@ -474,6 +475,17 @@
   int rc = window_read_counters(ctx, c, reset != 0);
   if (rc) return rc;
   for (int i = 0; i < 3; i++) counters[i] = c[i];
+  return MI355_OK;
+}
+
+int mi355_colorlut_box_stats(mi355_ctx *ctx, uint64_t counters[2], int reset) {
+  REQUIRE_CTX(ctx);
+  BIND_DEVICE(ctx);
+  if (!counters) return set_error(ctx, MI355_ERR_INVALID_ARG, "null counters");
+  unsigned long long c[2] = {0, 0};
+  int rc = box_read_counters(ctx, c, reset != 0);
+  if (rc) return rc;
+  for (int i = 0; i < 2; i++) counters[i] = c[i];
   return MI355_OK;
 }
 
diff --git a/gst-plugins-rs_amd/csrc/group.hip b/gst-plugins-rs_amd/csrc/group.hip
--- a/gst-plugins-rs_amd/csrc/group.hip
+++ b/gst-plugins-rs_amd/csrc/group.hip
@@ -1002,7 +1002,7 @@
   }
   const uint8_t *one[1] = {d_src};
   d.batchable = settled && format == MI355_FMT_RGBA && (fused || d_src != d_dst) && hsvfilter_multi_applicable(one, 1, width, height, stride, fmt) && width % 4 == 0 &&
-                width >= 128 && (uintptr_t)d_dst % 16 == 0 && ctx->lut_variant == 0 && ctx->hsv_table_mode != 2 && (!fused || ctx->lut.is3d);
+                width >= 128 && (uintptr_t)d_dst % 16 == 0 && (ctx->lut_variant == 0 || ctx->lut_variant == 10 || ctx->lut_variant == 11) && ctx->hsv_table_mode != 2 && (!fused || ctx->lut.is3d);
   if (d.batchable && (fused ? colorlut_multi_fused_table(ctx, settings, &d.table) : colorlut_multi_table(ctx, &d.table)) != MI355_OK) {
     (void)hipGetLastError();
     d.batchable = false;
diff --git a/gst-plugins-rs_amd/csrc/internal.hpp b/gst-plugins-rs_amd/csrc/internal.hpp
--- a/gst-plugins-rs_amd/csrc/internal.hpp
+++ b/gst-plugins-rs_amd/csrc/internal.hpp
@@ -10,6 +10,7 @@
 #include "autopick.hpp"
 #include "colorlut_brick.hpp"
 #include "colorlut_window.hpp"
+#include "colorlut_box.hpp"
 
 namespace mi355 {
 
@@ -113,6 +114,9 @@
   int window_order = 1;
   bool window_stats_on = false;
   unsigned long long *d_window_counters = nullptr;
+  unsigned *d_box_counters = nullptr;
+  mi355::BoxWatchState box_watch;
+  unsigned long long box_waves = 0;
   int blockhash_any_size = 0;
   int hsv_nt = 0;
   mi355_hsv_settings group_fused_hs{};
diff --git a/gst-plugins-rs_amd/mi355fx/__init__.py b/gst-plugins-rs_amd/mi355fx/__init__.py
--- a/gst-plugins-rs_amd/mi355fx/__init__.py
+++ b/gst-plugins-rs_amd/mi355fx/__init__.py
@@ -210,6 +210,8 @@
         "mi355_colorlut_last_kernel": (C.c_char_p, [vp]),
         "mi355_colorlut_brick_stats": (i, [vp, C.POINTER(C.c_uint64), C.POINTER(C.c_double), C.POINTER(C.c_int), i]),
         "mi355_colorlut_window_stats": (i, [vp, C.POINTER(C.c_uint64), i]),
+        "mi355_colorlut_box_stats": (i, [vp, C.POINTER(C.c_uint64), i]),
+        "mi355_selftest_boxwatch": (i, [i, C.POINTER(C.c_double), i, C.POINTER(C.c_int)]),
         "mi355_selftest_brickwatch": (i, [i, C.POINTER(C.c_double), C.POINTER(C.c_double), C.POINTER(C.c_double), C.POINTER(C.c_double), i, C.POINTER(C.c_int)]),
         "mi355_colorlut_frame": (i, [vp, u8p, i, u8p, i, i, i, i]),
         "mi355_colorlut_frames_device": (i, [vp, u8p, sz, i, u8p, sz, i, i, i, i, i]),
@@ -1194,6 +1196,11 @@
         self._ck(self.L.mi355_colorlut_window_stats(self.h, c, int(reset)))
         return int(c[0]), int(c[1]), int(c[2])
 
+    def colorlut_box_stats(self, reset=False):
+        c = (C.c_uint64 * 2)()
+        self._ck(self.L.mi355_colorlut_box_stats(self.h, c, int(reset)))
+        return int(c[0]), int(c[1])
+
     def colorlut_frame(self, src, src_stride, dst, dst_stride, width, height, fmt="RGBA"):
         self._ck(self.L.mi355_colorlut_frame(self.h, _ptr(src), src_stride, _ptr(dst), dst_stride, width, height, FMT[fmt]))
         return dst
diff --git a/include/mi355fx.h b/include/mi355fx.h
--- a/include/mi355fx.h
+++ b/include/mi355fx.h
@@ -112,6 +112,8 @@
 const char *mi355_colorlut_last_kernel(mi355_ctx *ctx);
 int mi355_colorlut_brick_stats(mi355_ctx *ctx, uint64_t counters[2], double *last_miss_fraction, int *level, int reset);
 int mi355_colorlut_window_stats(mi355_ctx *ctx, uint64_t counters[3], int reset);
+int mi355_colorlut_box_stats(mi355_ctx *ctx, uint64_t counters[2], int reset);
+int mi355_selftest_boxwatch(int n_calls, const double *share, int lag, int *box_out);
 int mi355_selftest_brickwatch(int n_calls, const double *miss0, const double *slow0, const double *miss1, const double *slow1, int lag,
                               int *level_out);
 int mi355_selftest_autopick(int n_calls, const uint64_t *n_vec, const double *ms_compute, const double *ms_table, int lag,
```

Measured after the change: 45140. No clear change (-0.0%).
